# ESMS-Group-Public/FoKL-GPy

Measured on AMD Instinct MI355X. Metric: candidate-terms/sec (basis build + Gibbs + BIC), higher is better.
Workload: dtype f64

## Files before the change

### fokl_gpy_amd/_capi.py

```python
import ctypes
import os

import numpy as np

_HERE = os.path.dirname(os.path.abspath(__file__))
LIB_PATH = os.environ.get('FOKL_HIP_LIBRARY', os.path.join(_HERE, 'libfokl_hip.so'))

UNIQUE_ID_BYTES = 128
K_BASIS, K_GRAM, K_RESID, K_PREDICT, K_RESID_MF, K_GRAM_MFMA, K_GRAM_REDUCE = 0, 1, 2, 3, 4, 5, 6
K_INTEGRATE, K_BAND = 7, 8
K_OPTIMIZE = 9
K_OPTIMIZE_SYSTEM = 10
K_POPULATION = 11
K_RESAMPLE = 12
K_SCORE = 13
K_INFER = 14
K_DESIGN = 15
INTEGRATE_MAX_STATES = 4
RESID_TERMS_MAX_FACTORS = 32
RESID_TERMS_MAX_ORDER = 8
RESID_TERMS_LAYOUTS = ((8, 1), (16, 1), (8, 2), (4, 4), (2, 8), (8, 4), (16, 2), (4, 8))
SLOT_ONES, SLOT_Y, SLOT_FIRST_FREE = 0, 1, 2
PREDICT_NONE, PREDICT_VALU_LDS, PREDICT_VALU_GLOBAL, PREDICT_MFMA = 0, 1, 2, 3
POPULATION_COEFFICIENTS = ('none', 'registers', 'table')
# ... 1396 lines not shown
        a = self._area[3 * self.p1 + self.p1 * self.p1 + 2:]
        return dict(sweeps=int(a[0]), rotations=int(a[1]), seconds=float(a[2]), not_converged=bool(a[3]))

    def release(self):
        if not self._released and self.engine._h:
            self._released = True
            _check(self.engine._lib.fokl_dspectral_release(self.engine._h, self.ticket))


class DeviceSpectralEngine:

    def __init__(self, device=0):
        self._lib = load()
        self._h = None
        h = c_vp(0)
        _check(self._lib.fokl_dspectral_create(int(device), ctypes.byref(h)))
        self._h = h
        self.device = int(device)
        self.max_columns = int(self._lib.fokl_dspectral_max_columns())

    def close(self):
        if self._h:
            self._lib.fokl_dspectral_destroy(self._h)
            self._h = None

    __del__ = close

    def set_signs(self, canonical=True):
        _check(self._lib.fokl_dspectral_set_signs(self._h, 1 if canonical else 0))

    def submit(self, gram, idx, launch=True):
        gram = np.ascontiguousarray(gram, dtype=np.float64)
        idx = np.ascontiguousarray(idx, dtype=np.int32)
        ticket, result = c_i64(0), c_vp(0)
        _check(self._lib.fokl_dspectral_submit(self._h, _ptr(gram), int(gram.shape[0]), _ptr(idx), int(idx.size),
                                               int(gram.shape[0]) - 1, 1 if launch else 0, ctypes.byref(ticket),
                                               ctypes.byref(result)))
        return DeviceSpectralJob(self, ticket.value, result.value, idx.size)

    def flush(self):
        _check(self._lib.fokl_dspectral_flush(self._h))

    def stats(self):
        submitted, launches = c_i64(0), c_i64(0)
        _check(self._lib.fokl_dspectral_stats(self._h, ctypes.byref(submitted), ctypes.byref(launches)))
        return dict(submitted=submitted.value, launches=launches.value)


def gibbs_chain_device(engine, lamb, qty, b, btau, dtd, sigsqd0, tausqd0, tape, stat_first=0):
    job = engine.submit(lamb, qty, b, btau, dtd, sigsqd0, tausqd0, tape, stat_first, follow=False)
    try:
        mean_w, flag = job.wait()
        return job.fetch_w(), np.array(mean_w), bool(flag[0])
    finally:
        job.release()



_OPS_SIGS = (('reserve_slots', [c_vp, c_int]),
             ('build_terms', [c_vp, c_vp, c_int, c_vp]),
             ('gram', [c_vp, c_vp, c_int, c_vp, c_int, c_vp, c_int, c_int]),
             ('gram_launch', [c_vp, c_vp, c_int, c_vp, c_int, c_int]),
             ('gram_fetch', [c_vp, c_vp, c_i64]),
             ('gram_ready', [c_vp]),
             ('bic_resid', [c_vp, c_vp, c_int, c_vp, c_vp, c_int]),
             ('bic_resid_launch', [c_vp, c_vp, c_int, c_vp]),
             ('bic_resid_fetch', [c_vp, c_vp, c_int]),
             ('bic_resid_terms_launch', [c_vp, c_vp, c_int, c_vp]))
_OPS_TYPES = {name: ctypes.CFUNCTYPE(c_int, *args) for name, args in _OPS_SIGS}


class _BackendOps(ctypes.Structure):
    _fields_ = [('ctx', c_vp)] + [(name, c_vp) for name, _ in _OPS_SIGS] + [('kernel_id', c_i32)]


class _RunParams(ctypes.Structure):
    _fields_ = [(name, c_i32) for name in (
        'm', 'n_phis', 'way3', 'tolerance', 'gimmie', 'draws', 'half0', 'lookahead', 'lookahead_native', 'foresight',
        'speculate_across', 'forecast_early', 'forecast_polls', 'matrix_free', 'update_from', 'update_depth',
        'update_lookahead', 'head_start', 'slot_capacity')]


RUN_STATS = ('terms_physical', 'substages', 'forecasts_used', 'forecasts_early', 'resid_matrix_free', 't_resid',
             'phase_prepare', 'phase_model', 'phase_statistics', 'phase_tests', 'phase_wrap_up')


def backend_ops(backend, kernel_id):
    lib = load()
    ops = _BackendOps()
    ops.kernel_id = int(kernel_id)
    ctx = getattr(backend, 'ctx', None)
    if isinstance(ctx, DeviceContext):
        ops.ctx = ctx._h
        for name, _ in _OPS_SIGS:
            setattr(ops, name, ctypes.cast(getattr(lib, 'fokl_' + name), c_vp).value)
        return ops, (ctx,)
    pending, raised = {}, []

    def arr(ptr, count, ctype, dtype):
        return np.array(np.ctypeslib.as_array(ctypes.cast(ptr, ctypes.POINTER(ctype * count)).contents), dtype=dtype)

    def guard(fn):
        def call(*args):
            try:
                fn(*args)
                return 0
            except BaseException as exc:
                raised.append(exc)
                return -3
        return call

    def out(ptr, values):
        values = np.ascontiguousarray(values, dtype=np.float64).reshape(-1)
        ctypes.memmove(ptr, values.ctypes.data, values.nbytes)

    def reserve_slots(_c, n):
        backend.reserve_slots(int(n))

    def build_terms(_c, terms, T, slots):
        sl = arr(slots, T, ctypes.c_int32, np.int32)
        m = pending['m']
        backend.build_terms(arr(terms, T * m, ctypes.c_int32, np.int32).reshape(T, m), [int(v) for v in sl])

    def gram(_c, rows, nr, cols, nc, dst, _path, allreduce):
        out(dst, backend.gram([int(v) for v in arr(rows, nr, ctypes.c_int32, np.int32)],
                              [int(v) for v in arr(cols, nc, ctypes.c_int32, np.int32)], bool(allreduce)))

    def gram_launch(_c, rows, nr, cols, nc, allreduce):
        pending['gram'] = backend.gram([int(v) for v in arr(rows, nr, ctypes.c_int32, np.int32)],
                                       [int(v) for v in arr(cols, nc, ctypes.c_int32, np.int32)], bool(allreduce))

    def gram_fetch(_c, dst, count):
        block = pending.pop('gram')
        assert block.size == count
        out(dst, block)

    def bic_resid(_c, slots, nc, betahat, dst, allreduce):
        out(dst, backend.bic_resid([int(v) for v in arr(slots, nc, ctypes.c_int32, np.int32)],
                                   arr(betahat, nc, ctypes.c_double, np.float64), bool(allreduce)))

    def bic_resid_launch(_c, slots, nc, betahat):
        pending['resid'] = backend.bic_resid([int(v) for v in arr(slots, nc, ctypes.c_int32, np.int32)],
                                             arr(betahat, nc, ctypes.c_double, np.float64), False)

    def bic_resid_fetch(_c, dst, _allreduce):
        out(dst, pending.pop('resid'))

    table = dict(reserve_slots=reserve_slots, build_terms=build_terms, gram=gram, gram_launch=gram_launch,
                 gram_fetch=gram_fetch, bic_resid=bic_resid, bic_resid_launch=bic_resid_launch,
                 bic_resid_fetch=bic_resid_fetch)
    keep = [pending, raised]
    for name, fn in table.items():
        cb = _OPS_TYPES[name](guard(fn))
        keep.append(cb)
        setattr(ops, name, ctypes.cast(cb, c_vp).value)
    return ops, tuple(keep)


class NativeRun:

    def __init__(self, backend, kernel_id, **params):
        self._lib = load()
        self._h = None
        self._ops, self._keep = backend_ops(backend, kernel_id)
        if isinstance(self._keep[0], dict):
            self._keep[0]['m'] = int(params['m'])
        self._prm = _RunParams(**{k: int(v) for k, v in params.items()})
# ... 349 lines not shown
    def design_select(self, slots, C0, CMC0=None, picks=1, replicates=False, refresh_every=64, keep=False, grid_cap=0):
        s = np.ascontiguousarray(slots, dtype=np.int32)
        nc = s.shape[0]
        C0 = np.ascontiguousarray(C0, dtype=np.float64)
        if C0.shape != (nc, nc):
            raise ValueError("design_select: C0 must be [columns, columns] of the slot list")
        if CMC0 is not None:
            CMC0 = np.ascontiguousarray(CMC0, dtype=np.float64)
            if CMC0.shape != (nc, nc):
                raise ValueError("design_select: CMC0 must be [columns, columns] of the slot list")
        picks = int(picks)
        rows = max(picks, 0)
        index = np.empty(rows, dtype=np.int64)
        gain, vstar, x = np.empty(rows), np.empty(rows), np.empty((rows, nc))
        v = np.empty(self.n, dtype=np.float64) if keep else None
        w = np.empty(self.n, dtype=np.float64) if keep and CMC0 is not None else None
        self._ck(self._lib.fokl_design_select(self._h, _ptr(s), nc, _ptr(C0), _ptr(CMC0), picks, int(bool(replicates)),
                                              int(refresh_every), int(grid_cap), _ptr(index), _ptr(gain), _ptr(vstar), _ptr(x),
                                              _ptr(v), _ptr(w)))
        return dict(index=index, gain=gain, vstar=vstar, x=x, v=v, w=w)

    def design_report(self):
        out = np.zeros(12, dtype=np.int64)
        self._ck(self._lib.fokl_design_report(self._h, _ptr(out)))
        v = [int(x) for x in out]
        return dict(instance=DESIGN_INSTANCES[v[0]], grid=v[1], step_grid=v[2], row_tiles=v[3], lds_bytes=v[4], picks=v[5],
                    refreshes=v[6], launches=v[7], kernel_us=v[8], quadform_us=v[9], step_us=v[10], pivot_us=v[11])

    def infer_inputs(self, mtx_u, betas, h, table, lo, hi, prior_mean, prior_prec, y, known_prod, starts, burnin, draws,
                     thin, jump_every, seed, draw_ids=None, rows=True, term_cap=0):
        f64 = lambda a: np.ascontiguousarray(a, dtype=np.float64)
        mtx_u = np.ascontiguousarray(mtx_u, dtype=np.int32)
        betas, h, table, lo, hi, prior_mean, prior_prec, y, known_prod, starts = (
            f64(a) for a in (betas, h, table, lo, hi, prior_mean, prior_prec, y, known_prod, starts))
        if mtx_u.ndim != 2 or betas.ndim != 2 or table.ndim != 2 or y.ndim != 1 or starts.ndim != 2 or lo.ndim != 1:
            raise ValueError("infer_inputs: array shapes disagree")
        n_terms, d = mtx_u.shape
        E, K = betas.shape[0], y.shape[0]
        if betas.shape[1] != n_terms + 1 or h.shape != (E,) or known_prod.shape != (K, n_terms + 1) or \
                starts.shape != (INFER_WALKERS, d) or any(a.shape != (d,) for a in (lo, hi, prior_mean, prior_prec)):
            raise ValueError("infer_inputs: array shapes disagree")
        ids = None
        if draw_ids is not None:
            ids = np.ascontiguousarray(draw_ids, dtype=np.uint32)
            if ids.shape != (E,):
                raise ValueError("infer_inputs: one draw id per row of betas")
        kept = -(-int(draws) // int(thin)) if int(thin) >= 1 and int(draws) >= 1 else 0
        x = np.empty((E, kept, INFER_WALKERS, d), dtype=np.float64) if rows else None
        lp = np.empty((E, kept, INFER_WALKERS), dtype=np.float64) if rows else None
        sums = np.empty((E, INFER_WALKERS, 2, 2, d), dtype=np.float64)
        accepted = np.empty((E, INFER_WALKERS, 2), dtype=np.int32)
        evaluations = np.empty(E, dtype=np.int64)
        self._ck(self._lib.fokl_infer_inputs(
            self._h, int(d), int(n_terms), _ptr(mtx_u), int(E), _ptr(betas), _ptr(h), _ptr(ids), _ptr(table),
            int(table.shape[0]), int(table.shape[1]), _ptr(lo), _ptr(hi), _ptr(prior_mean), _ptr(prior_prec), int(K), _ptr(y),
            _ptr(known_prod), _ptr(starts), int(burnin), int(draws), int(thin), int(jump_every), int(seed) & 0xFFFFFFFF,
            int(term_cap), _ptr(x), _ptr(lp), _ptr(sums), _ptr(accepted), _ptr(evaluations)))
        return x, lp, sums, accepted, evaluations

    def infer_report(self):
        out = np.zeros(9, dtype=np.int64)
        self._ck(self._lib.fokl_infer_report(self._h, _ptr(out)))
        v = [int(x) for x in out]
        return dict(mapping=INFER_MAPPINGS[v[0]], lds_rows=v[1], grid=v[2], launches=v[3], kernel_us=v[4], iterations=v[5],
                    evaluations=v[6], draws_per_launch=v[7], lds_bytes=v[8])

    def _fit_report(self, which, count):
        out = np.zeros(count, dtype=np.int64)
        self._ck(self._lib.fokl_fit_report(self._h, which, _ptr(out), count))
        return [int(v) for v in out]

    def gram_report(self):
        keys = ('kernel', 'nt8', 'half', 'loaders', 'lds_buffers', 'ks', 'depth', 'rows_per_chunk', 'groups', 'ct', 'nt',
                'pieces', 'lds_bytes', 'S', 'chunks_per_workgroup', 'nr_pad', 'nc_pad', 'slabs', 'reduce_epb', 'row_tiles',
                'col_tiles', 'lanes')
        ran = dict(zip(keys, self._fit_report(0, len(keys))))
        ran['kernel'], ran['half'] = GRAM_KERNELS[ran['kernel']], bool(ran['half'])
        return ran

    def resid_report(self):
        v = self._fit_report(1, 9)
        return dict(kernel=RESID_KERNELS[v[0]], columns=v[1], batches=v[2], grid=v[3], row_tiles=v[4], layout=(v[5], v[6]),
                    order_class=v[7], inputs=v[8])

    def basis_report(self):
        v = self._fit_report(2, 23)
        keys = ('kernel', 'splines', 'lanes', 'factors', 'slabs', 'grid', 'row_tiles')

        def one(rec):
            d = dict(zip(keys, rec))
            d['kernel'], d['splines'] = BASIS_KERNELS[d['kernel']], bool(d['splines'])
            return d
        return dict(launches=v[0], lds_table=v[1], first=one(v[2:9]), last=one(v[9:16]), last_lds=one(v[16:23]))

    def gp_integrate_ensemble(self, n_members, n_states, n_other, n_steps, betas, per_member, mtx, rows, cols, sources,
                              n_src, forcing, norms, table, n_basis, width, h, y0, cut=None, want_members=False):
        mean = np.empty((n_states, n_steps + 1), dtype=np.float64)
        bounds = np.empty((n_states, n_steps + 1, 2), dtype=np.float64) if cut is not None else None
        members = np.empty((n_members, n_states, n_steps + 1), dtype=np.float64) if want_members else None
        self._ck(self._lib.fokl_gp_integrate_ensemble(
            self._h, int(n_members), int(n_states), int(n_other), int(n_steps), betas, _ptr(per_member), mtx, _ptr(rows),
            _ptr(cols), sources, _ptr(n_src), _ptr(forcing), _ptr(norms), _ptr(table), int(n_basis), int(width), float(h),
            _ptr(y0), int(y0.ndim == 2), int(cut or 0), _ptr(mean), _ptr(bounds), _ptr(members)))
        return mean, bounds, members

    def simulate_ensemble(self, p):
        K, E, P = int(p['K']), int(p['E']), int(p['n_steps']) + 1
        mean = np.empty((K, P), dtype=np.float64)
        bounds = np.empty((K, P, 2), dtype=np.float64) if p['want_bounds'] else None
        members = np.empty((E, K, P), dtype=np.float64) if p['want_members'] else None
        first = np.empty(E, dtype=np.int32)
        i32 = lambda a: np.ascontiguousarray(a, dtype=np.int32)
        f64 = lambda a: np.ascontiguousarray(a, dtype=np.float64)
        forcing, norm_src, norm_lo, norm_span = f64(p['forcing']), i32(p['norm_src']), f64(p['norm_lo']), f64(p['norm_span'])
        fac_norm, fac_kind, fac_row, fac_degree = (i32(p[key]) for key in ('fac_norm', 'fac_kind', 'fac_row', 'fac_degree'))
        spline, bern, entries = f64(p['spline_table']), f64(p['bern_table']), i32(p['entries']).reshape(-1, 4)
        begin, count, constant = i32(p['entry_begin']), i32(p['entry_count']), i32(p['constant'])
        coef, y0, box = f64(p['coef']), f64(p['y0']), f64(p['box'])
        if coef.ndim != 2 or coef.shape[1] != E or y0.shape != (K, E) or box.shape != (K, 2) or begin.shape != (K,) or \
                count.shape != (K,) or constant.shape != (K,) or forcing.ndim != 2 or forcing.shape[0] != P - 1 or \
                not (norm_src.shape == norm_lo.shape == norm_span.shape) or \
                not (fac_norm.shape == fac_kind.shape == fac_row.shape == fac_degree.shape) or \
                spline.shape[1:] != (499, 4) or bern.ndim != 2 or bern.shape[1] != 21:
            raise ValueError("simulate_ensemble: array shapes disagree")
        self._ck(self._lib.fokl_simulate_ensemble(
            self._h, E, K, P - 1, float(p['h']), forcing.shape[1], _ptr(forcing), int(p['n_norm_forcing']), norm_src.shape[0],
            _ptr(norm_src), _ptr(norm_lo), _ptr(norm_span), int(p['n_forcing_factors']), fac_norm.shape[0], _ptr(fac_norm),
            _ptr(fac_kind), _ptr(fac_row), _ptr(fac_degree), spline.shape[0], _ptr(spline), bern.shape[0], _ptr(bern),
            entries.shape[0], _ptr(entries), _ptr(begin), _ptr(count), _ptr(constant), coef.shape[0], _ptr(coef), _ptr(y0),
            _ptr(box), int(p['cut']) if p['want_bounds'] else 0, _ptr(mean), _ptr(bounds), _ptr(members), _ptr(first)))
        return mean, bounds, members, first

    def simulate_report(self):
        out = np.zeros(8, dtype=np.int64)
        self._ck(self._lib.fokl_simulate_report(self._h, _ptr(out)))
        keys = ('NS', 'members', 'workgroups', 'lds_bytes', 'launches', 'spline_factors', 'bernoulli_factors',
                'steps_per_launch')
        return dict(zip(keys, (int(v) for v in out)))

    def assimilate_ensemble(self, p):
        K, E, P = int(p['K']), int(p['E']), int(p['n_steps']) + 1
        i32 = lambda a: np.ascontiguousarray(a, dtype=np.int32)
        f64 = lambda a: np.ascontiguousarray(a, dtype=np.float64)
        forcing, norm_src, norm_lo, norm_span = f64(p['forcing']), i32(p['norm_src']), f64(p['norm_lo']), f64(p['norm_span'])
        fac_norm, fac_kind, fac_row, fac_degree = (i32(p[key]) for key in ('fac_norm', 'fac_kind', 'fac_row', 'fac_degree'))
        spline, bern, entries = f64(p['spline_table']), f64(p['bern_table']), i32(p['entries']).reshape(-1, 4)
        begin, count, constant = i32(p['entry_begin']), i32(p['entry_count']), i32(p['constant'])
        coef, y0, box = f64(np.asarray(p['coef']).T), f64(p['y0']), f64(p['box'])
        ids = np.ascontiguousarray(p['draw_ids'], dtype=np.uint32)
        obs_state, obs_sd, obs_row = i32(p['obs_state']), f64(p['obs_sd']), i32(p['obs_row'])
        data, obs_const, q, y0_sd = f64(p['data']), f64(p['obs_const']), f64(p['process_q']), f64(p['y0_sd'])
        n_obs = data.shape[0] if data.ndim == 2 else -1
        if coef.ndim != 2 or coef.shape[0] != E or y0.shape != (K, E) or box.shape != (K, 2) or begin.shape != (K,) or \
                count.shape != (K,) or constant.shape != (K,) or forcing.ndim != 2 or forcing.shape[0] != P - 1 or \
                not (norm_src.shape == norm_lo.shape == norm_span.shape) or \
                not (fac_norm.shape == fac_kind.shape == fac_row.shape == fac_degree.shape) or \
                spline.shape[1:] != (499, 4) or bern.ndim != 2 or bern.shape[1] != 21 or ids.shape != (E,) or \
                obs_state.ndim != 1 or obs_sd.shape != obs_state.shape or data.ndim != 2 or \
                data.shape[1] != obs_state.shape[0] or obs_row.shape != (P,) or obs_const.shape != (n_obs,) or \
                q.shape != (K,) or y0_sd.shape != (K,):
            raise ValueError("assimilate_ensemble: array shapes disagree")
        stats = np.empty((E, n_obs, 2 * K + 3), dtype=np.float64)
        keep = bool(p['want_particles'])
        particles = np.empty((E, n_obs, ASSIMILATE_PARTICLES, K), dtype=np.float64) if keep else None
        weights = np.empty((E, n_obs, ASSIMILATE_PARTICLES), dtype=np.float64) if keep else None
        first, collapsed = np.empty(E, dtype=np.int32), np.empty(E, dtype=np.int32)
# ... 396 lines not shown
```

### fokl_gpy_amd/csrc/fokl_gram_dev.inc

```

namespace fokl {


constexpr int GM_THREADS = 256;
constexpr int GM_R = 32;
constexpr int GM_PITCH = GM_R + 2;

template <int TI, int TJ, bool ISPLIT>
__global__ __launch_bounds__(GM_THREADS) void gram_mfma_kernel(double *const *__restrict__ slot_ptr,
                                                               const int *__restrict__ row_slots, int nr,
                                                               const int *__restrict__ col_slots, int nc, int64_t n,
                                                               double *__restrict__ slab, int nr_pad, int nc_pad,
                                                               const double *__restrict__ zero_col)
{
    static_assert(!ISPLIT || TI == 4, "i-split needs one i-tile per wavefront");
    constexpr int BI = 16 * TI;
    constexpr int BJ = ISPLIT ? 16 * TJ : 64 * TJ;
    constexpr int NCOL = BI + BJ;
    constexpr int PASSES = (NCOL + 15) / 16;
    constexpr int MI = ISPLIT ? 1 : TI;
    __shared__ __attribute__((aligned(16))) double tile[NCOL * GM_PITCH];

    const int tid = threadIdx.x, wave = tid / WAVE, lane = tid % WAVE;
    const int i0 = blockIdx.z * BI, j0 = blockIdx.y * BJ;
// ... 302 lines not shown

template <int NT>
static gram_tiles_fn tiles_kernel_n(int passes, int depth, int ks)
{
    if (passes <= 4) return tiles_kernel_np<NT, 4>(depth, ks);
    if (passes <= 8) return tiles_kernel_np<NT, 8>(depth, ks);
    return tiles_kernel_np<NT, 16>(depth, ks);
}

static gram_tiles_fn tiles_kernel(int nt, int passes, int depth, int ks)
{
    switch (nt) {
        case 1: return tiles_kernel_n<1>(passes, depth, ks);
        case 2: return tiles_kernel_n<2>(passes, depth, ks);
        case 3: return tiles_kernel_n<3>(passes, depth, ks);
        case 4: return tiles_kernel_n<4>(passes, depth, ks);
        case 5: return gram_tiles_kernel<5, 16, 1, 1>;
        case 6: return gram_tiles_kernel<6, 16, 1, 1>;
        case 7: return gram_tiles_kernel<7, 16, 1, 1>;
        case 8: return gram_tiles_kernel<8, 16, 1, 1>;
        case 9: return gram_tiles_kernel<9, 16, 1, 1>;
        default: return gram_tiles_kernel<10, 16, 1, 1>;
    }
}

typedef void (*gram_tiles4_fn)(double *const *, const int *, int, const GramGroup *, int, int64_t, double *, int, int,
                               const double *, const double *);

template <int NT>
static gram_tiles4_fn tiles4s_kernel_n(int passes)
{
    if (passes <= 2) return gram_tiles4s_kernel<NT, 2>;
    if (passes <= 4) return gram_tiles4s_kernel<NT, 4>;
    if (passes <= 6) return gram_tiles4s_kernel<NT, 6>;
    return gram_tiles4s_kernel<NT, 8>;
}

static gram_tiles4_fn tiles4s_kernel(int nt, int passes)
{
    switch (nt) {
        case 1: return tiles4s_kernel_n<1>(passes);
        case 2: return tiles4s_kernel_n<2>(passes);
        case 3: return tiles4s_kernel_n<3>(passes);
        default: return tiles4s_kernel_n<4>(passes);
    }
}


static gram_dma_fn tiles_dma_kernel_ab(int nt8, bool half, int nbuf, int loaders)
{
    if (nbuf == 3) return loaders == 0 ? tiles_dma_kernel_b<3, 0>(nt8, half) : nullptr;
    if (nbuf == 2 && loaders == 2) return tiles_dma_kernel_b<2, 2>(nt8, half);
    return tiles_dma_kernel(nt8, half, nbuf, loaders);
}

static int launch_gram_panel(fokl_ctx *ctx, const GramCall &c, GramLaunch &run)
{
    const int *d_rows, *d_cols;
    int rc = push_slot_lists(ctx, c, d_rows, d_cols);
    if (rc) return rc;
    const int nr = c.nr, nc = c.nc;
    gram_mfma_fn mfma_fn = nullptr;
    int BI, BJ;
    const int j_tiles = (nc + 15) / 16;
    if (nr > 32) {
        const int panels = (j_tiles + 11) / 12;
        const int tj = (j_tiles + panels - 1) / panels;
        mfma_fn = isplit_kernel(tj);
        BI = 64;
        BJ = 16 * tj;
    } else {
        const int ti = nr > 16 ? 2 : 1;
        const int per_wave = (j_tiles + 3) / 4;
        const int panels = (per_wave + 2) / 3;
        const int tj = (per_wave + panels - 1) / panels;
        mfma_fn = jsplit_kernel(ti, tj);
        BI = 16 * ti;
        BJ = 64 * tj;
    }
    const int gz = (nr + BI - 1) / BI, gy = (nc + BJ - 1) / BJ;
    run.nr_pad = gz * BI;
    run.nc_pad = gy * BJ;
    const int64_t n_chunks = (ctx->n + GM_R - 1) / GM_R;
    const int per_cu = blocks_per_cu(mfma_fn, GM_THREADS, 0);
    const int target = std::max(1, (per_cu * cu_count(ctx)) / (gz * gy));
    rc = size_slabs(ctx, run, (int)std::max<int64_t>(1, std::min<int64_t>(n_chunks, target)), 1, n_chunks);
    if (rc) return rc;
    run.rep[0] = FOKL_GRAM_PANEL, run.rep[5] = run.rep[6] = 1, run.rep[7] = GM_R, run.rep[8] = gy * gz;
    run.rep[21] = GM_THREADS;
    TimedRegion timed(ctx, c.slot, c.bytes, c.flops);
    hipLaunchKernelGGL(mfma_fn, dim3(run.S, gy, gz), dim3(GM_THREADS), 0, ctx->stream, ctx->d_slot_ptr, d_rows, nr, d_cols,
                       nc, ctx->n, ctx->d_slab, run.nr_pad, run.nc_pad, ctx->d_zero);
    return FOKL_OK;
}

static int launch_gram_tiles4(fokl_ctx *ctx, const GramCall &c, GramLaunch &run, int wgs_cap)
{
    const GramPlan &pl = run.plan;
    const int P = pl.ct <= 2 ? 2 : pl.ct <= 4 ? 4 : pl.ct <= 6 ? 6 : 8;
    gram_tiles4_fn fn = tiles4s_kernel(pl.nt, pl.ct);
    const size_t lds = (size_t)P * 16 * G4_PITCH * sizeof(double);
    int rc = raise_lds_limit(ctx, reinterpret_cast<const void *>(fn), lds);
    if (rc) return rc;
    const int64_t n_chunks = (ctx->n + 31) / 32;
    const int per_cu = std::min(wgs_cap, blocks_per_cu(fn, G4S_THREADS, lds));
    const int target = std::max(1, (per_cu * cu_count(ctx)) / (int)pl.groups.size());
    rc = size_slabs(ctx, run, (int)std::max<int64_t>(1, std::min<int64_t>(n_chunks, target)), 1, n_chunks);
    if (rc) return rc;
    run.rep[0] = FOKL_GRAM_TILES4, run.rep[1] = pl.nt, run.rep[7] = 32, run.rep[12] = (int64_t)lds, run.rep[21] = G4S_THREADS;
    TimedRegion timed(ctx, c.slot, c.bytes, c.flops);
    hipLaunchKernelGGL(fn, dim3(run.S, (unsigned)pl.groups.size()), dim3(G4S_THREADS), lds, ctx->stream, ctx->d_slot_ptr,
                       run.d_icols, pl.nci, run.d_groups, pl.ct, ctx->n, ctx->d_slab, run.nr_pad, run.nc_pad, ctx->d_zero,
                       run.grid_base);
    return FOKL_OK;
}

static int launch_gram_dev(fokl_ctx *ctx, const GramCall &c, const LaunchKnobs &k, int path, GramLaunch &run, bool &taken)
{
    const GramPlan &pl = run.plan;
    taken = true;
    if (path == 3) return launch_gram_panel(ctx, c, run);
    if (pl.kind == 1) return launch_gram_tiles4(ctx, c, run, k.wgs);
    if (pl.ks == 1 && k.dma != 2 && !(k.dma == 1 && c.slot == FOKL_K_GRAM_MFMA)) {
        gram_tiles_fn fn = tiles_kernel(pl.nt, pl.ct << pl.rb_shift, pl.depth, 1);
        const size_t lds = (size_t)pl.ct * 16 * ((32 << pl.rb_shift) + 2) * sizeof(double);
        return launch_gram_tiles(ctx, c, run, fn, k.wgs, blocks_per_cu(fn, GT_THREADS, lds), cu_count(ctx));
    }
    if (pl.ks > 1 && (pl.rb_shift != 0 || pl.depth != 1)) {
        const int passes = pl.ct << pl.rb_shift;
        return launch_gram_tiles(ctx, c, run, tiles_kernel(pl.nt, passes, pl.depth, pl.ks), k.wgs, passes > 8 && pl.depth == 2 ? 2 : 3);
    }
    const size_t pieces = (pl.ct * 16 * 34 * 8 + 1023) / 1024;
    const int nbuf = k.bufs == 3 && 3 * pieces * 1024 <= 160 * 1024 ? 3 : 2;
    if (pl.ks == 1 && (nbuf == 3 || k.loaders == 2))
        return launch_gram_dma(ctx, c, run, tiles_dma_kernel_ab, k.wgs, nbuf, nbuf == 2 ? k.loaders : 0);
    taken = false;
    return FOKL_OK;
}
```

### fokl_gpy_amd/csrc/fokl_hip.hip

```cpp
#include <hip/hip_runtime.h>

#include <algorithm>
#include <climits>
#include <cmath>
#include <cstdint>
#include <cstdio>
#include <cstdlib>
#include <cstring>
#include <map>
#include <mutex>
#include <string>
#include <utility>
#include <vector>

#include "../../include/fokl_hip_internal.h"
#include "fokl_kernels.hip.h"

using namespace fokl;


static std::mutex g_err_mutex;
static std::string g_err;

void fokl_set_global_error(const std::string &msg)
{
    std::lock_guard<std::mutex> lock(g_err_mutex);
    g_err = msg;
}

struct TimingSlot {
    double ms = 0.0;
    int64_t launches = 0;
    double bytes = 0.0;
    double flops = 0.0;
    double ideal_ms = 0.0;
};

struct PendingEvent {
    int kernel_id;
    hipEvent_t start, stop;
};

struct fokl_ctx {
    int device = 0;
    int cus = 0;
    hipStream_t stream = nullptr;
    std::string err;

    bool have_data = false;
    int64_t n = 0, ld = 0;
    int m = 0, kernel = 0, n_basis = 0, width = 0;
    double *d_x = nullptr;
    double *d_zero = nullptr;
    double *d_staged = nullptr;
    int64_t staged_n = 0;
    int staged_m = 0;
    double *d_phis = nullptr;
    std::vector<double> h_phis;
    size_t phis_doubles = 0;

    static constexpr int CHUNK_SLOTS = 16;
    std::vector<double *> chunks;
    std::vector<double *> slot_ptr;
    double **d_slot_ptr = nullptr;
    int table_cap = 0;

    char *d_args = nullptr;
    char *h_args = nullptr;
    size_t args_cap = 0;
    double *d_slab = nullptr;
    size_t slab_doubles = 0;
    double *d_out = nullptr;
    double *h_out = nullptr;
    size_t out_doubles = 0;
    hipEvent_t args_free = nullptr;
    bool resid_pending = false;
    double *d_rout = nullptr;
    double *h_rout = nullptr;
    double *d_gout = nullptr;
    double *h_gout = nullptr;
    size_t gout_doubles = 0;
    size_t gram_pending = 0;
    hipEvent_t gram_done = nullptr;
    hipEvent_t resid_done = nullptr;
    int64_t predict_report[6] = {0, 0, 0, 0, 0, 0};
    int64_t population_report[FOKL_POPULATION_REPORT_LEN] = {};
    int64_t resample_report[FOKL_RESAMPLE_REPORT_LEN] = {};
    int64_t score_report[FOKL_SCORE_REPORT_LEN] = {};
    int64_t infer_report[FOKL_INFER_REPORT_LEN] = {};
    int64_t design_report[FOKL_DESIGN_REPORT_LEN] = {};
    int64_t simulate_report[FOKL_SIMULATE_REPORT_LEN] = {};
    int64_t assimilate_report[FOKL_ASSIMILATE_REPORT_LEN] = {};
    int64_t control_report[FOKL_CONTROL_REPORT_LEN] = {};
    int64_t control_pooled_report[FOKL_CONTROL_POOLED_REPORT_LEN] = {};
    int64_t control_cvar_report[FOKL_CONTROL_CVAR_REPORT_LEN] = {};
    int64_t gram_report[FOKL_GRAM_REPORT_LEN] = {};
    int64_t resid_report[FOKL_RESID_REPORT_LEN] = {};
    int64_t basis_report[FOKL_BASIS_REPORT_LEN] = {};

    bool timing = false;
    TimingSlot tslot[FOKL_K_COUNT];
    std::vector<PendingEvent> pending;
    std::vector<hipEvent_t> event_pool;

    void *comm = nullptr;
    int rank = 0, world = 1;
    double *d_comm = nullptr;
    size_t comm_doubles = 0;

    int64_t optimize_report[FOKL_OPTIMIZE_REPORT_LEN] = {};
    int64_t system_optimize_report[FOKL_OPTIMIZE_REPORT_LEN] = {};
};

static int fail(fokl_ctx *ctx, int code, const std::string &msg)
{
    if (ctx) ctx->err = msg;
    fokl_set_global_error(msg);
    return code;
}

#define HIP_TRY(ctx, call)                                                                                     \
    do {                                                                                                       \
        hipError_t e__ = (call);                                                                               \
        if (e__ != hipSuccess)                                                                                 \
            return fail(ctx, FOKL_ERR_HIP, std::string(#call) + ": " + hipGetErrorString(e__));                \
    } while (0)

struct DeviceBuffers {
    std::vector<void *> owned;
    ~DeviceBuffers()
    {
        for (void *p : owned) (void)hipFree(p);
    }
    template <typename T>
    hipError_t get(T **out, size_t count)
    {
        void *p = nullptr;
        hipError_t e = hipMalloc(&p, std::max<size_t>(count, 1) * sizeof(T));
        if (e == hipSuccess) owned.push_back(p);
        *out = static_cast<T *>(p);
        return e;
    }
    template <typename T>
    hipError_t upload(T **out, const void *host, size_t count)
    {
        hipError_t e = get(out, count);
        if (e == hipSuccess && count) e = hipMemcpy(*out, host, count * sizeof(T), hipMemcpyHostToDevice);
        return e;
    }
};


static hipEvent_t take_event(fokl_ctx *ctx)
{
    if (!ctx->event_pool.empty()) {
        hipEvent_t e = ctx->event_pool.back();
        ctx->event_pool.pop_back();
        return e;
    }
    hipEvent_t e = nullptr;
    if (hipEventCreate(&e) != hipSuccess) return nullptr;
    return e;
}

struct TimedRegion {
    fokl_ctx *ctx;
    int id;
    hipEvent_t start = nullptr, stop = nullptr;
    TimedRegion(fokl_ctx *c, int kernel_id, double bytes, double flops) : ctx(c), id(kernel_id)
    {
        if (!ctx->timing) return;
        ctx->tslot[id].launches += 1;
        ctx->tslot[id].bytes += bytes;
        ctx->tslot[id].flops += flops;
        ctx->tslot[id].ideal_ms += 1e3 * std::max(bytes / FOKL_PEAK_HBM_BYTES_PER_S, flops / FOKL_PEAK_F64_FLOPS);
        start = take_event(ctx);
        stop = take_event(ctx);
        if (start && stop) (void)hipEventRecord(start, ctx->stream);
    }
    ~TimedRegion()
    {
        if (!ctx->timing || !start || !stop) return;
        (void)hipEventRecord(stop, ctx->stream);
        ctx->pending.push_back({id, start, stop});
    }
};

static void drain_events(fokl_ctx *ctx)
{
    for (auto &p : ctx->pending) {
        float ms = 0.f;
        if (hipEventSynchronize(p.stop) == hipSuccess && hipEventElapsedTime(&ms, p.start, p.stop) == hipSuccess)
            ctx->tslot[p.kernel_id].ms += ms;
        ctx->event_pool.push_back(p.start);
        ctx->event_pool.push_back(p.stop);
    }
    ctx->pending.clear();
}


static int ensure_args(fokl_ctx *ctx, size_t bytes)
{
    if (bytes <= ctx->args_cap) return FOKL_OK;
    size_t cap = std::max<size_t>(bytes * 2, 1 << 16);
    HIP_TRY(ctx, hipStreamSynchronize(ctx->stream));
    if (ctx->d_args) HIP_TRY(ctx, hipFree(ctx->d_args));
    if (ctx->h_args) HIP_TRY(ctx, hipHostFree(ctx->h_args));
    ctx->d_args = nullptr;
    ctx->h_args = nullptr;
    ctx->args_cap = 0;
    HIP_TRY(ctx, hipMalloc((void **)&ctx->d_args, cap));
    HIP_TRY(ctx, hipHostMalloc((void **)&ctx->h_args, cap, hipHostMallocDefault));
    ctx->args_cap = cap;
    return FOKL_OK;
}

static int ensure_slab(fokl_ctx *ctx, size_t doubles)
{
    if (doubles <= ctx->slab_doubles) return FOKL_OK;
    size_t cap = std::max<size_t>(doubles + doubles / 2, 1 << 16);
    HIP_TRY(ctx, hipStreamSynchronize(ctx->stream));
    if (ctx->d_slab) HIP_TRY(ctx, hipFree(ctx->d_slab));
    ctx->d_slab = nullptr;
    ctx->slab_doubles = 0;
    HIP_TRY(ctx, hipMalloc((void **)&ctx->d_slab, cap * sizeof(double)));
    ctx->slab_doubles = cap;
    return FOKL_OK;
}

static int ensure_out(fokl_ctx *ctx, size_t doubles)
{
    if (doubles <= ctx->out_doubles) return FOKL_OK;
    size_t cap = std::max<size_t>(doubles * 2, 1 << 12);
    HIP_TRY(ctx, hipStreamSynchronize(ctx->stream));
    if (ctx->d_out) HIP_TRY(ctx, hipFree(ctx->d_out));
    if (ctx->h_out) HIP_TRY(ctx, hipHostFree(ctx->h_out));
    ctx->d_out = nullptr;
    ctx->h_out = nullptr;
    ctx->out_doubles = 0;
    HIP_TRY(ctx, hipMalloc((void **)&ctx->d_out, cap * sizeof(double)));
    HIP_TRY(ctx, hipHostMalloc((void **)&ctx->h_out, cap * sizeof(double), hipHostMallocDefault));
    ctx->out_doubles = cap;
    return FOKL_OK;
}

static int ensure_rout(fokl_ctx *ctx)
{
    if (ctx->d_rout) return FOKL_OK;
    HIP_TRY(ctx, hipMalloc((void **)&ctx->d_rout, 2 * sizeof(double)));
    HIP_TRY(ctx, hipHostMalloc((void **)&ctx->h_rout, 2 * sizeof(double), hipHostMallocDefault));
    return FOKL_OK;
}

static int ensure_gout(fokl_ctx *ctx, size_t doubles)
{
    if (doubles <= ctx->gout_doubles) return FOKL_OK;
    size_t cap = std::max<size_t>(doubles * 2, 1 << 12);
    HIP_TRY(ctx, hipStreamSynchronize(ctx->stream));
    if (ctx->d_gout) HIP_TRY(ctx, hipFree(ctx->d_gout));
    if (ctx->h_gout) HIP_TRY(ctx, hipHostFree(ctx->h_gout));
    ctx->d_gout = nullptr;
    ctx->h_gout = nullptr;
    ctx->gout_doubles = 0;
    HIP_TRY(ctx, hipMalloc((void **)&ctx->d_gout, cap * sizeof(double)));
    HIP_TRY(ctx, hipHostMalloc((void **)&ctx->h_gout, cap * sizeof(double), hipHostMallocDefault));
    ctx->gout_doubles = cap;
    return FOKL_OK;
}

static int begin_args(fokl_ctx *ctx, size_t bytes)
{
    int rc = ensure_args(ctx, bytes);
    if (rc) return rc;
    HIP_TRY(ctx, hipEventSynchronize(ctx->args_free));
    return FOKL_OK;
}

static int push_args(fokl_ctx *ctx, size_t bytes)
{
    HIP_TRY(ctx, hipMemcpyAsync(ctx->d_args, ctx->h_args, bytes, hipMemcpyHostToDevice, ctx->stream));
    HIP_TRY(ctx, hipEventRecord(ctx->args_free, ctx->stream));
    return FOKL_OK;
}

static void free_slots(fokl_ctx *ctx)
{
    for (double *c : ctx->chunks) (void)hipFree(c);
    ctx->chunks.clear();
    ctx->slot_ptr.clear();
}

static int check_slots(fokl_ctx *ctx, const int32_t *slots, int count, const char *who)
{
    if (!slots && count > 0) return fail(ctx, FOKL_ERR_ARG, std::string(who) + ": null slot list");
    const int cap = (int)ctx->slot_ptr.size();
    for (int i = 0; i < count; ++i)
        if (slots[i] < 0 || slots[i] >= cap)
            return fail(ctx, FOKL_ERR_ARG, std::string(who) + ": slot " + std::to_string(slots[i]) +
                                               " outside [0, " + std::to_string(cap) + ")");
    return FOKL_OK;
}


extern "C" int fokl_version(void) { return 100; }

extern "C" int fokl_device_count(int *count)
{
    if (!count) return fail(nullptr, FOKL_ERR_ARG, "fokl_device_count: null pointer");
    int n = 0;
    hipError_t e = hipGetDeviceCount(&n);
    if (e != hipSuccess) {
        *count = 0;
        return fail(nullptr, FOKL_ERR_HIP, std::string("hipGetDeviceCount: ") + hipGetErrorString(e));
    }
    *count = n;
    return FOKL_OK;
}

extern "C" const char *fokl_last_error(const fokl_ctx *ctx)
{
    if (ctx) return ctx->err.c_str();
    std::lock_guard<std::mutex> lock(g_err_mutex);
    static thread_local std::string copy;
    copy = g_err;
    return copy.c_str();
}

extern "C" int fokl_ctx_create(int device, fokl_ctx **out)
{
    if (!out) return fail(nullptr, FOKL_ERR_ARG, "fokl_ctx_create: null output pointer");
    *out = nullptr;
    int n = 0;
    hipError_t e = hipGetDeviceCount(&n);
    if (e != hipSuccess || n <= 0)
        return fail(nullptr, FOKL_ERR_HIP, "fokl_ctx_create: no HIP device available (" +
                                               std::string(hipGetErrorString(e)) + ")");
    if (device < 0 || device >= n)
        return fail(nullptr, FOKL_ERR_ARG, "fokl_ctx_create: device index out of range");
    fokl_ctx *ctx = new fokl_ctx();
    ctx->device = device;
    if (const char *mode = std::getenv("FOKL_SYNC"))
        if (std::strcmp(mode, "blocking") == 0) {
            (void)hipSetDeviceFlags(hipDeviceScheduleBlockingSync);
            (void)hipGetLastError();
        }
    HIP_TRY(nullptr, hipSetDevice(device));
    hipDeviceProp_t prop;
    HIP_TRY(nullptr, hipGetDeviceProperties(&prop, device));
    if (std::string(prop.gcnArchName).rfind("gfx950", 0) != 0) {
        std::string arch = prop.gcnArchName;
        delete ctx;
        return fail(nullptr, FOKL_ERR_HIP, "fokl_ctx_create: device is " + arch + ", this library is built for gfx950 only");
    }
    const int total_cus = prop.multiProcessorCount;
    ctx->cus = total_cus;
    const hipError_t made = hipStreamCreateWithFlags(&ctx->stream, hipStreamNonBlocking);
    if (made != hipSuccess ||
        hipEventCreateWithFlags(&ctx->args_free, hipEventDisableTiming) != hipSuccess ||
        hipEventCreateWithFlags(&ctx->gram_done, hipEventDisableTiming) != hipSuccess ||
        hipEventCreateWithFlags(&ctx->resid_done, hipEventDisableTiming) != hipSuccess) {
        delete ctx;
        return fail(nullptr, FOKL_ERR_HIP, "fokl_ctx_create: cannot create stream / event");
    }
    (void)hipEventRecord(ctx->args_free, ctx->stream);
    *out = ctx;
    return FOKL_OK;
}

extern "C" int fokl_comm_destroy(fokl_ctx *ctx);

extern "C" void fokl_ctx_destroy(fokl_ctx *ctx)
{
    if (!ctx) return;
    (void)hipSetDevice(ctx->device);
    if (ctx->stream) (void)hipStreamSynchronize(ctx->stream);
    (void)fokl_comm_destroy(ctx);
    drain_events(ctx);
    for (hipEvent_t e : ctx->event_pool) (void)hipEventDestroy(e);
    free_slots(ctx);
    if (ctx->d_slot_ptr) (void)hipFree(ctx->d_slot_ptr);
    if (ctx->d_x) (void)hipFree(ctx->d_x);
    if (ctx->d_phis) (void)hipFree(ctx->d_phis);
    if (ctx->d_zero) (void)hipFree(ctx->d_zero);
    if (ctx->d_staged) (void)hipFree(ctx->d_staged);
    if (ctx->d_args) (void)hipFree(ctx->d_args);
    if (ctx->h_args) (void)hipHostFree(ctx->h_args);
    if (ctx->d_slab) (void)hipFree(ctx->d_slab);
    if (ctx->d_out) (void)hipFree(ctx->d_out);
    if (ctx->h_out) (void)hipHostFree(ctx->h_out);
    if (ctx->d_gout) (void)hipFree(ctx->d_gout);
    if (ctx->h_gout) (void)hipHostFree(ctx->h_gout);
    if (ctx->d_rout) (void)hipFree(ctx->d_rout);
    if (ctx->h_rout) (void)hipHostFree(ctx->h_rout);
    if (ctx->d_comm) (void)hipFree(ctx->d_comm);
    if (ctx->args_free) (void)hipEventDestroy(ctx->args_free);
    if (ctx->gram_done) (void)hipEventDestroy(ctx->gram_done);
    if (ctx->resid_done) (void)hipEventDestroy(ctx->resid_done);
    if (ctx->stream) (void)hipStreamDestroy(ctx->stream);
    delete ctx;
}

extern "C" int fokl_sync(fokl_ctx *ctx)
{
    if (!ctx) return fail(nullptr, FOKL_ERR_ARG, "fokl_sync: null context");
    HIP_TRY(ctx, hipStreamSynchronize(ctx->stream));
    drain_events(ctx);
    return FOKL_OK;
}

extern "C" int fokl_slot_capacity(const fokl_ctx *ctx) { return ctx ? (int)ctx->slot_ptr.size() : 0; }
extern "C" int64_t fokl_rows(const fokl_ctx *ctx) { return ctx ? ctx->n : 0; }


extern "C" int fokl_reserve_slots(fokl_ctx *ctx, int n_slots)
{
    if (!ctx) return fail(nullptr, FOKL_ERR_ARG, "fokl_reserve_slots: null context");
    if (!ctx->have_data) return fail(ctx, FOKL_ERR_STATE, "fokl_reserve_slots: call fokl_upload first");
    HIP_TRY(ctx, hipSetDevice(ctx->device));
    bool grew = false;
    while ((int)ctx->slot_ptr.size() < n_slots) {
        double *chunk = nullptr;
        const size_t bytes = (size_t)fokl_ctx::CHUNK_SLOTS * ctx->ld * sizeof(double);
        HIP_TRY(ctx, hipMalloc((void **)&chunk, bytes));
        ctx->chunks.push_back(chunk);
        for (int i = 0; i < fokl_ctx::CHUNK_SLOTS; ++i) ctx->slot_ptr.push_back(chunk + (size_t)i * ctx->ld);
        grew = true;
    }
    if (grew) {
        const int cap = (int)ctx->slot_ptr.size();
        if (cap > ctx->table_cap) {
            HIP_TRY(ctx, hipStreamSynchronize(ctx->stream));
            if (ctx->d_slot_ptr) HIP_TRY(ctx, hipFree(ctx->d_slot_ptr));
            ctx->d_slot_ptr = nullptr;
            ctx->table_cap = 0;
            const int new_cap = std::max(cap * 2, 256);
            HIP_TRY(ctx, hipMalloc((void **)&ctx->d_slot_ptr, (size_t)new_cap * sizeof(double *)));
            ctx->table_cap = new_cap;
        }
        HIP_TRY(ctx, hipStreamSynchronize(ctx->stream));
        HIP_TRY(ctx, hipMemcpy(ctx->d_slot_ptr, ctx->slot_ptr.data(), (size_t)cap * sizeof(double *),
                               hipMemcpyHostToDevice));
    }
    return FOKL_OK;
}


static int upload_dataset(fokl_ctx *ctx, const double *x, const double *y, int64_t n, int m, int kernel, const double *phis,
                          int n_basis, int width, const double *lows, const double *spans, const char *who)
{
    if (!ctx) return fail(nullptr, FOKL_ERR_ARG, std::string(who) + ": null context");
    if (!y || !phis) return fail(ctx, FOKL_ERR_ARG, std::string(who) + ": null pointer");
    if (n <= 0 || m <= 0 || m > 4096) return fail(ctx, FOKL_ERR_ARG, std::string(who) + ": need n > 0 and 0 < m <= 4096");
    if (kernel != FOKL_KERNEL_SPLINES && kernel != FOKL_KERNEL_BERNOULLI)
        return fail(ctx, FOKL_ERR_ARG, std::string(who) + ": unknown kernel id");
    if (n_basis <= 0 || width <= 0) return fail(ctx, FOKL_ERR_ARG, std::string(who) + ": empty coefficient table");
    if (kernel == FOKL_KERNEL_BERNOULLI && width < n_basis + 1)
        return fail(ctx, FOKL_ERR_ARG, std::string(who) + ": Bernoulli table needs width >= n_basis + 1");
    HIP_TRY(ctx, hipSetDevice(ctx->device));
    HIP_TRY(ctx, hipStreamSynchronize(ctx->stream));
    drain_events(ctx);

    free_slots(ctx);
    if (ctx->d_x) HIP_TRY(ctx, hipFree(ctx->d_x));
    if (ctx->d_phis) HIP_TRY(ctx, hipFree(ctx->d_phis));
    if (ctx->d_zero) HIP_TRY(ctx, hipFree(ctx->d_zero));
    ctx->d_x = nullptr;
    ctx->d_phis = nullptr;
    ctx->d_zero = nullptr;
    ctx->have_data = false;

    ctx->n = n;
    ctx->m = m;
    ctx->ld = (n + 63) / 64 * 64;
    ctx->kernel = kernel;
    ctx->n_basis = n_basis;
    ctx->width = width;
    ctx->phis_doubles = (kernel == FOKL_KERNEL_SPLINES) ? (size_t)n_basis * 4 * width : (size_t)n_basis * width;

// ... 41 lines not shown

extern "C" int fokl_stage_inputs(fokl_ctx *ctx, const double *x, int64_t n, int m, double *lows_out, double *highs_out)
{
    if (!ctx) return fail(nullptr, FOKL_ERR_ARG, "fokl_stage_inputs: null context");
    if (!x || !lows_out || !highs_out) return fail(ctx, FOKL_ERR_ARG, "fokl_stage_inputs: null pointer");
    if (n <= 0 || m <= 0 || m > 4096) return fail(ctx, FOKL_ERR_ARG, "fokl_stage_inputs: need n > 0 and 0 < m <= 4096");
    HIP_TRY(ctx, hipSetDevice(ctx->device));
    if (ctx->d_staged) HIP_TRY(ctx, hipFree(ctx->d_staged));
    ctx->d_staged = nullptr;
    HIP_TRY(ctx, hipMalloc((void **)&ctx->d_staged, (size_t)n * m * sizeof(double)));
    ctx->staged_n = n;
    ctx->staged_m = m;
    HIP_TRY(ctx, hipMemcpy(ctx->d_staged, x, (size_t)n * m * sizeof(double), hipMemcpyHostToDevice));
    const int64_t total = n * (int64_t)m;
    int64_t lanes = std::min<int64_t>((int64_t)1024 * 256, (total + 7) / 8);
    lanes = std::max<int64_t>(m, lanes / m * m);
    const int blocks = (int)((lanes + 255) / 256);
    double *d_part = nullptr;
    HIP_TRY(ctx, hipMalloc((void **)&d_part, (size_t)(2 * lanes + 2 * m) * sizeof(double)));
    hipLaunchKernelGGL(column_bounds_kernel, dim3(blocks), dim3(256), 0, ctx->stream, ctx->d_staged, total, m, lanes, d_part);
    hipLaunchKernelGGL(column_bounds_finish_kernel, dim3(m), dim3(256), 0, ctx->stream, d_part, lanes, m, d_part + 2 * lanes);
    HIP_TRY(ctx, hipGetLastError());
    std::vector<double> h((size_t)2 * m);
    HIP_TRY(ctx, hipMemcpyAsync(h.data(), d_part + 2 * lanes, (size_t)2 * m * sizeof(double), hipMemcpyDeviceToHost, ctx->stream));
    HIP_TRY(ctx, hipStreamSynchronize(ctx->stream));
    HIP_TRY(ctx, hipFree(d_part));
    for (int k = 0; k < m; ++k) {
        lows_out[k] = h[(size_t)k];
        highs_out[k] = h[(size_t)m + k];
    }
    return FOKL_OK;
}

extern "C" int fokl_upload_staged(fokl_ctx *ctx, const double *y, int64_t n, int m, int kernel, const double *phis,
                                  int n_basis, int width, const double *lows, const double *spans)
{
    if (!ctx) return fail(nullptr, FOKL_ERR_ARG, "fokl_upload_staged: null context");
    if (!lows || !spans) return fail(ctx, FOKL_ERR_ARG, "fokl_upload_staged: null pointer");
    if (!ctx->d_staged || ctx->staged_n != n || ctx->staged_m != m)
        return fail(ctx, FOKL_ERR_STATE, "fokl_upload_staged: no staged inputs of this shape (fokl_stage_inputs first)");
    return upload_dataset(ctx, nullptr, y, n, m, kernel, phis, n_basis, width, lows, spans, "fokl_upload_staged");
}

extern "C" int fokl_download_inputs(fokl_ctx *ctx, double *x_out)
{
    if (!ctx) return fail(nullptr, FOKL_ERR_ARG, "fokl_download_inputs: null context");
    if (!x_out) return fail(ctx, FOKL_ERR_ARG, "fokl_download_inputs: null pointer");
    if (!ctx->have_data) return fail(ctx, FOKL_ERR_STATE, "fokl_download_inputs: call fokl_upload first");
    HIP_TRY(ctx, hipSetDevice(ctx->device));
    double *d_rows = nullptr;
    HIP_TRY(ctx, hipMalloc((void **)&d_rows, (size_t)ctx->n * ctx->m * sizeof(double)));
    const int blocks = (int)std::min<int64_t>((ctx->n + 255) / 256, 4096);
    hipLaunchKernelGGL(rows_from_columns_kernel, dim3(blocks), dim3(256), 0, ctx->stream, ctx->d_x, ctx->n, ctx->m, ctx->ld, d_rows);
    HIP_TRY(ctx, hipGetLastError());
    HIP_TRY(ctx, hipMemcpyAsync(x_out, d_rows, (size_t)ctx->n * ctx->m * sizeof(double), hipMemcpyDeviceToHost, ctx->stream));
    HIP_TRY(ctx, hipStreamSynchronize(ctx->stream));
    HIP_TRY(ctx, hipFree(d_rows));
    return FOKL_OK;
}


static int cu_count(fokl_ctx *ctx) { return ctx->cus > 0 ? ctx->cus : 256; }

static int env_int(const char *name, int fallback)
{
    const char *v = std::getenv(name);
    return v && *v ? std::atoi(v) : fallback;
}

struct LaunchKnobs {
    int path = 2, mfma4 = 0, dma = 2, half = 1, bufs = 2, loaders = 4, rb = 1, depth = 1, wgs = 3;
    int k1_wgs = INT_MAX;
    int tiles4_nt = 0, tiles4_ct = 0;
    bool half_slots() const { return mfma4 != 2 && dma == 2 && half != 0; }
};
#ifdef FOKL_DEV_KERNELS
static LaunchKnobs launch_knobs();
#else
static LaunchKnobs launch_knobs() { return LaunchKnobs(); }
#endif

static constexpr size_t K1_LDS_BUDGET = 144 * 1024;

static int launch_basis(fokl_ctx *ctx, const int32_t *terms, const int32_t *slots, int t_begin, int t_end,
                        const DerivSpec &deriv)
{
    const int m = ctx->m;
    const bool splines = ctx->kernel == FOKL_KERNEL_SPLINES;
    std::map<std::pair<int, int>, int> fac_id;
    for (int j = t_begin; j < t_end; ++j)
        for (int k = 0; k < m; ++k) {
            const int o = terms[(size_t)j * m + k];
            if (o != 0) fac_id.emplace(std::make_pair(k, o), 0);
        }
    int U = 0;
    for (auto &kv : fac_id) kv.second = U++;
    const int T = t_end - t_begin;

    std::vector<int> slab_orders;
    if (splines) {
        for (auto &kv : fac_id) {
            const int o = kv.first.second;
            if (std::find(slab_orders.begin(), slab_orders.end(), o) == slab_orders.end() &&
                (int)slab_orders.size() < K1_MAX_LDS_SLABS)
                slab_orders.push_back(o);
        }
    }
    const int NS = (int)slab_orders.size();
    size_t slab_doubles = splines ? (((size_t)NS * 4 * ctx->width + 1) & ~(size_t)1) : 0;
    int threads = K1_THREADS;
    {
        int best_waves = -1;
        for (int t : {256, 128, 64}) {
            const size_t need = slab_doubles * sizeof(double) + (size_t)std::max(U, 1) * t * sizeof(d2);
            const int blocks = (int)std::min<size_t>(16, (160 * 1024) / std::max<size_t>(need, 1));
            const int waves = std::min(32, blocks * (t / 64));
            if (waves > best_waves) {
                best_waves = waves;
                threads = t;
            }
        }
        if (const char *env = getenv("FOKL_K1_THREADS")) {
            const int t = atoi(env);
            if (t == 64 || t == 128 || t == 256) threads = t;
        }
    }
    const bool reg_table = U <= K1_REG_FACTORS;
    if (reg_table) threads = K1_THREADS;
    size_t lds_bytes = slab_doubles * sizeof(double) +
                       (reg_table ? 0 : (size_t)std::max(U, 1) * threads * sizeof(d2));

    size_t n_fac_entries = 0;
    for (int j = t_begin; j < t_end; ++j)
        for (int k = 0; k < m; ++k) n_fac_entries += terms[(size_t)j * m + k] != 0;

    const size_t n_ints = (size_t)3 * U + K1_MAX_LDS_SLABS + (T + 1) + n_fac_entries + T;
    const size_t plan_bytes = sizeof(BasisPlan);
    const size_t bytes = plan_bytes + n_ints * sizeof(int);
    int rc = begin_args(ctx, bytes);
    if (rc) return rc;
    BasisPlan *plan = reinterpret_cast<BasisPlan *>(ctx->h_args);
    plan->n_fac = U;
    plan->n_terms = T;
    plan->n_slabs = NS;
    plan->pad = 0;
    int *arr = reinterpret_cast<int *>(ctx->h_args + plan_bytes);
    int *fac_input = arr, *fac_order = arr + U, *fac_slab = arr + 2 * U, *slab_order = arr + 3 * U;
    int *term_off = slab_order + K1_MAX_LDS_SLABS, *term_fac = term_off + (T + 1);
    int *term_slot = term_fac + n_fac_entries;
    for (auto &kv : fac_id) {
        const int u = kv.second;
        fac_input[u] = kv.first.first;
        fac_order[u] = kv.first.second;
        int s = -1;
        for (int q = 0; q < NS; ++q)
            if (slab_orders[q] == kv.first.second) s = q;
        fac_slab[u] = s;
    }
    for (int q = 0; q < K1_MAX_LDS_SLABS; ++q) slab_order[q] = q < NS ? slab_orders[q] : 1;
    int off = 0;
    for (int j = t_begin; j < t_end; ++j) {
        term_off[j - t_begin] = off;
        for (int k = 0; k < m; ++k) {
            const int o = terms[(size_t)j * m + k];
            if (o != 0) term_fac[off++] = fac_id[std::make_pair(k, o)];
        }
        term_slot[j - t_begin] = slots[j];
    }
    term_off[T] = off;
    rc = push_args(ctx, bytes);
    if (rc) return rc;

    const int64_t tile_rows = (int64_t)threads * K1_ROWS_PER_THREAD;
    const int64_t n_tiles = (ctx->n + tile_rows - 1) / tile_rows;
    int per_cu = (int)std::max<size_t>(1, std::min<size_t>(reg_table ? 5 : 16, (160 * 1024) / std::max<size_t>(lds_bytes, 1)));
    per_cu = std::min(per_cu, launch_knobs().k1_wgs);
    const int grid = (int)std::min<int64_t>(n_tiles, (int64_t)cu_count(ctx) * per_cu);
    const BasisPlan *d_plan = reinterpret_cast<const BasisPlan *>(ctx->d_args);
    const int *d_arr = reinterpret_cast<const int *>(ctx->d_args + plan_bytes);

    int m_used = 0;
    {
        int last = -1;
        for (auto &kv : fac_id)
            if (kv.first.first != last) {
                last = kv.first.first;
                ++m_used;
            }
    }
    const double alg_bytes = 8.0 * (double)ctx->n * (double)(m_used + T);
    TimedRegion timed(ctx, FOKL_K_BASIS, alg_bytes, 0.0);
    typedef void (*basis_fn)(const double *, int64_t, int64_t, const double *, int, const BasisPlan *, const int *,
                             double *const *, DerivSpec);
    basis_fn fn = splines ? (reg_table ? basis_build_reg_kernel<true> : basis_build_kernel<true>)
                          : (reg_table ? basis_build_reg_kernel<false> : basis_build_kernel<false>);
    if (lds_bytes > 64 * 1024)
        HIP_TRY(ctx, hipFuncSetAttribute(reinterpret_cast<const void *>(fn), hipFuncAttributeMaxDynamicSharedMemorySize,
                                         (int)K1_LDS_BUDGET + 4096));
    hipLaunchKernelGGL(fn, dim3(grid), dim3(threads), lds_bytes, ctx->stream, ctx->d_x, ctx->ld, ctx->n, ctx->d_phis,
                       ctx->width, d_plan, d_arr, ctx->d_slot_ptr, deriv);
    HIP_TRY(ctx, hipGetLastError());
    {
        const int64_t rec[7] = {reg_table ? FOKL_BASIS_REG_TABLE : FOKL_BASIS_LDS_TABLE, splines ? 1 : 0, threads, U, NS,
                                grid, n_tiles};
        int64_t *rep = ctx->basis_report;
        if (rep[0]++ == 0) std::memcpy(rep + 2, rec, sizeof rec);
        std::memcpy(rep + 9, rec, sizeof rec);
        if (!reg_table) {
            rep[1] += 1;
            std::memcpy(rep + 16, rec, sizeof rec);
        }
    }
    return FOKL_OK;
}

static int build_terms_impl(fokl_ctx *ctx, const int32_t *terms, int T, const int32_t *slots, const DerivSpec &deriv);

extern "C" int fokl_build_terms(fokl_ctx *ctx, const int32_t *terms, int T, const int32_t *slots)
{
    const DerivSpec plain = {-1, 0, 1.0, 0};
    return build_terms_impl(ctx, terms, T, slots, plain);
}

extern "C" int fokl_build_terms_deriv(fokl_ctx *ctx, const int32_t *terms, int T, const int32_t *slots, int wrt_input,
                                      int order, double divisor)
{
    if (!ctx) return fail(nullptr, FOKL_ERR_ARG, "fokl_build_terms_deriv: null context");
    if (!ctx->have_data) return fail(ctx, FOKL_ERR_STATE, "fokl_build_terms_deriv: call fokl_upload first");
    if (wrt_input < 0 || wrt_input >= ctx->m || (order != 1 && order != 2) || !(divisor != 0.0))
        return fail(ctx, FOKL_ERR_ARG, "fokl_build_terms_deriv: need 0 <= wrt_input < m, order 1 or 2, divisor != 0");
    for (int j = 0; j < T; ++j)
        if (terms && terms[(size_t)j * ctx->m + wrt_input] == 0)
            return fail(ctx, FOKL_ERR_ARG, "fokl_build_terms_deriv: a term does not contain the differentiated input "
                                           "(its derivative is the zero column; leave it out)");
    const DerivSpec spec = {wrt_input, order, divisor, 1};
    return build_terms_impl(ctx, terms, T, slots, spec);
}

static int build_terms_impl(fokl_ctx *ctx, const int32_t *terms, int T, const int32_t *slots, const DerivSpec &deriv)
{
    if (!ctx) return fail(nullptr, FOKL_ERR_ARG, "fokl_build_terms: null context");
    std::memset(ctx->basis_report, 0, sizeof ctx->basis_report);
    if (!ctx->have_data) return fail(ctx, FOKL_ERR_STATE, "fokl_build_terms: call fokl_upload first");
    if (T < 0 || (T > 0 && (!terms || !slots))) return fail(ctx, FOKL_ERR_ARG, "fokl_build_terms: null pointer");
    if (T == 0) return FOKL_OK;
    HIP_TRY(ctx, hipSetDevice(ctx->device));
    int rc = check_slots(ctx, slots, T, "fokl_build_terms");
    if (rc) return rc;
    const int m = ctx->m;
    for (int j = 0; j < T; ++j) {
        if (slots[j] < FOKL_SLOT_FIRST_FREE)
            return fail(ctx, FOKL_ERR_ARG, "fokl_build_terms: slots 0 and 1 are reserved (ones, y)");
        int nz = 0;
        for (int k = 0; k < m; ++k) {
            const int o = terms[(size_t)j * m + k];
            if (o < 0 || o > ctx->n_basis)
                return fail(ctx, FOKL_ERR_ARG, "fokl_build_terms: basis order " + std::to_string(o) +
                                                   " outside [0, " + std::to_string(ctx->n_basis) + "]");
            nz += o != 0;
        }
        if (nz == 0) return fail(ctx, FOKL_ERR_ARG, "fokl_build_terms: term with no input (all-zero row)");
    }
    const bool splines = ctx->kernel == FOKL_KERNEL_SPLINES;
    const size_t slab_bytes = splines ? (size_t)K1_MAX_LDS_SLABS * 4 * ctx->width * sizeof(double) + 16 : 0;
    const int lds_fac = (int)((K1_LDS_BUDGET - slab_bytes) / (K1_THREADS * sizeof(d2)));
    int max_fac = K1_REG_FACTORS;
    for (int j = 0; j < T; ++j) {
        int nz = 0;
        for (int k = 0; k < m; ++k) nz += terms[(size_t)j * m + k] != 0;
        if (nz > lds_fac) return fail(ctx, FOKL_ERR_ARG, "fokl_build_terms: a single term has more factors than fit in LDS");
        if (nz > max_fac) max_fac = nz;
    }
    int begin = 0;
    while (begin < T) {
        std::map<std::pair<int, int>, int> seen;
        int end = begin;
        while (end < T) {
            std::vector<std::pair<int, int>> add;
            for (int k = 0; k < m; ++k) {
                const int o = terms[(size_t)end * m + k];
                if (o != 0 && !seen.count({k, o})) add.push_back({k, o});
            }
            if ((int)(seen.size() + add.size()) > max_fac) break;
            for (auto &p : add) seen[p] = 1;
            ++end;
        }
        if (end == begin) rc = fail(ctx, FOKL_ERR_ARG, "fokl_build_terms: a single term has more factors than fit in LDS");
        if (!rc) rc = launch_basis(ctx, terms, slots, begin, end, deriv);
        if (rc) {
            std::memset(ctx->basis_report, 0, sizeof ctx->basis_report);
            return rc;
        }
        begin = end;
    }
    return FOKL_OK;
}


extern "C" int fokl_comm_allreduce_sum_f64(fokl_ctx *ctx, double *buf, int count);
static int comm_allreduce_device(fokl_ctx *ctx, double *d_buf, size_t count);

static int reduce_elements_per_block(int total)
{
    int epb = 1;
    while (epb < 16 && epb * 64 < total) epb *= 2;
    while (epb < 64 && (total + epb - 1) / epb > 4096) epb *= 2;
    return epb;
}

template <typename F>
static int blocks_per_cu(F fn, int threads, size_t dyn_lds)
{
    int nb = 0;
    if (hipOccupancyMaxActiveBlocksPerMultiprocessor(&nb, fn, threads, dyn_lds) != hipSuccess || nb < 1) nb = 1;
    return std::min(nb, 8);
}


struct GramPlan {
    int nci = 0, it = 0, jt = 0;
    int nt = 1, ct = 1, ks = 1, rb_shift = 0, depth = 1;
    int kind = 0, waves = 4;
    bool half = false;
    std::vector<int32_t> icols;
    std::vector<int32_t> perm;
    std::vector<GramGroup> groups;
};

static void plan_gram(const int32_t *row_slots, int nr, const int32_t *col_slots, int nc, int kind, const LaunchKnobs &knobs,
                      GramPlan &pl)
{
    pl.kind = kind;
    pl.waves = 4;
    const int nt_max = kind == 1 ? knobs.tiles4_nt : GT_MAX_NT;
    const int ct_max = kind == 1 ? knobs.tiles4_ct : GT_MAX_CT;
    pl.icols.assign(row_slots, row_slots + nr);
    pl.perm.resize(nc);
    {
        std::map<int32_t, int> where;
        for (int i = 0; i < nr; ++i) where.emplace(row_slots[i], i);
        for (int j = 0; j < nc; ++j) {
            auto f = where.find(col_slots[j]);
            if (f != where.end()) {
                pl.perm[j] = f->second;
            } else {
                pl.perm[j] = (int)pl.icols.size();
                where.emplace(col_slots[j], (int)pl.icols.size());
                pl.icols.push_back(col_slots[j]);
            }
        }
    }
    pl.nci = (int)pl.icols.size();
    pl.it = (nr + 15) / 16;
    pl.jt = (pl.nci + 15) / 16;

    struct Cut {
        std::vector<std::pair<int, int>> tiles;
        std::vector<int> staged;
    };
    std::vector<Cut> cuts;
    const int max_tiles = pl.waves * nt_max;
    for (int b0 = 0; b0 < pl.it; b0 += 4) {
        const int i_hi = std::min(pl.it, b0 + 4);
        std::vector<std::pair<int, int>> seq;
        for (int jt = b0; jt < pl.jt; ++jt)
            for (int it = b0; it < std::min(i_hi, jt + 1); ++it) seq.emplace_back(it, jt);
        const int T = (int)seq.size();
        for (int G = std::max(1, (T + max_tiles - 1) / max_tiles);; ++G) {
            std::vector<Cut> trial;
            bool fits = true;
            int at = 0;
            for (int gi = 0; gi < G && fits; ++gi) {
                const int size = T / G + (gi < T % G ? 1 : 0);
                Cut c;
                c.tiles.assign(seq.begin() + at, seq.begin() + at + size);
                at += size;
                for (auto &t : c.tiles) {
                    c.staged.push_back(t.first);
                    c.staged.push_back(t.second);
                }
                std::sort(c.staged.begin(), c.staged.end());
                c.staged.erase(std::unique(c.staged.begin(), c.staged.end()), c.staged.end());
                fits = (int)c.staged.size() <= ct_max && size <= max_tiles;
                if (size > 0) trial.push_back(std::move(c));
            }
            if (fits) {
                for (auto &c : trial) cuts.push_back(std::move(c));
                break;
            }
        }
    }

    int most_tiles = 1, most_staged = 1;
    for (auto &c : cuts) {
        most_tiles = std::max(most_tiles, (int)c.tiles.size());
        most_staged = std::max(most_staged, (int)c.staged.size());
    }
    pl.ks = kind != 0 ? 1 : most_tiles == 1 ? 4 : most_tiles == 2 ? 2 : 1;
// ... 82 lines not shown
static int no_instance(fokl_ctx *ctx, const char *kernel, const GramPlan &pl)
{
    return fail(ctx, FOKL_ERR_ARG, std::string("fokl_gram: this library holds no ") + kernel + " for nt " + std::to_string(pl.nt) +
                                       ", ct " + std::to_string(pl.ct << pl.rb_shift) + ", depth " + std::to_string(pl.depth));
}

static gram_tiles_fn ksplit_kernel(const GramPlan &pl)
{
    if (pl.nt != 1 || pl.ct > 4 || pl.rb_shift != 0 || pl.depth != 1) return nullptr;
    return pl.ks == 4 ? gram_tiles_kernel<1, 4, 1, 4> : pl.ks == 2 ? gram_tiles_kernel<1, 4, 1, 2> : nullptr;
}

typedef void (*gram_dma_fn)(const GramGroup *, int, int, int64_t, double *, int, int, const double *, uint32_t);
typedef gram_dma_fn (*gram_dma_picker)(int nt8, bool half, int nbuf, int loaders);

template <int NBUF, int LW>
static gram_dma_fn tiles_dma_kernel_b(int nt8, bool half)
{
    static const gram_dma_fn plain[5] = {gram_tiles_dma_kernel<1, NBUF, false, LW>, gram_tiles_dma_kernel<2, NBUF, false, LW>,
                                         gram_tiles_dma_kernel<3, NBUF, false, LW>, gram_tiles_dma_kernel<4, NBUF, false, LW>,
                                         gram_tiles_dma_kernel<5, NBUF, false, LW>};
    static const gram_dma_fn slots[4] = {gram_tiles_dma_kernel<1, NBUF, true, LW>, gram_tiles_dma_kernel<2, NBUF, true, LW>,
                                         gram_tiles_dma_kernel<3, NBUF, true, LW>, gram_tiles_dma_kernel<4, NBUF, true, LW>};
    return nt8 < 1 || nt8 > (half ? 4 : 5) ? nullptr : half ? slots[nt8 - 1] : plain[nt8 - 1];
}

static gram_dma_fn tiles_dma_kernel(int nt8, bool half, int nbuf, int loaders)
{
    if (nbuf != 2) return nullptr;
    return loaders == 4 ? tiles_dma_kernel_b<2, 4>(nt8, half) : loaders == 0 ? tiles_dma_kernel_b<2, 0>(nt8, half) : nullptr;
}

extern "C" int fokl_gram_plan(const int32_t *row_slots, int nr, const int32_t *col_slots, int nc, int kind, int32_t *info,
                              int32_t *icols, int32_t *perm, int32_t *staged, int32_t *tiles, int cap_groups)
{
    if (!row_slots || !col_slots || !info || nr <= 0 || nc <= 0 || kind < 0 || kind > 1)
        return fail(nullptr, FOKL_ERR_ARG, "fokl_gram_plan: bad argument");
    const LaunchKnobs knobs = launch_knobs();
    if (kind == 1 && !knobs.tiles4_nt)
        return fail(nullptr, FOKL_ERR_ARG, "fokl_gram_plan: kind 1 (4x4x4 tile lists) needs a development build");
    GramPlan pl;
    plan_gram(row_slots, nr, col_slots, nc, kind, knobs, pl);
    const int32_t head[10] = {pl.nci, pl.it, pl.jt, (int32_t)pl.groups.size(), pl.nt, pl.ct, pl.rb_shift, pl.ks, pl.depth,
                              pl.waves};
    std::memcpy(info, head, sizeof(head));
    if ((int)pl.groups.size() > cap_groups) return FOKL_OK;
    if (icols) std::memcpy(icols, pl.icols.data(), pl.icols.size() * sizeof(int32_t));
    if (perm) std::memcpy(perm, pl.perm.data(), pl.perm.size() * sizeof(int32_t));
    for (size_t gi = 0; gi < pl.groups.size(); ++gi) {
        const GramGroup &g = pl.groups[gi];
        if (staged) std::memcpy(staged + gi * GT_MAX_CT, g.ct, sizeof(g.ct));
        if (tiles)
            for (int w = 0; w < GT_MAX_WAVES; ++w)
                for (int k = 0; k < GT_MAX_NT; ++k) {
                    int32_t *t = tiles + ((gi * GT_MAX_WAVES + w) * GT_MAX_NT + k) * 4;
                    t[0] = g.a[w][k] | (pl.half && k < 2 && g.oi[w][k] != 0xFFFF ? 256 : 0);
                    t[1] = g.b[w][k];
                    t[2] = g.oi[w][k] == 0xFFFF ? -1 : g.oi[w][k];
                    t[3] = g.oj[w][k] == 0xFFFF ? -1 : g.oj[w][k];
                }
    }
    return FOKL_OK;
}


struct GramCall {
    const int32_t *row_slots, *col_slots;
    int nr, nc;
    int slot;
    double bytes, flops;
};

struct GramLaunch {
    GramPlan plan;
    const int *d_icols = nullptr;
    const GramGroup *d_groups = nullptr;
    const double *grid_base = nullptr;
    const int *d_perm = nullptr;
    int S = 0, slabs = 0;
    int nr_pad = 0, nc_pad = 0;
    int64_t rep[FOKL_GRAM_REPORT_LEN] = {};
};

static std::mutex lds_limit_mutex;
static std::map<const void *, size_t> lds_limit_set;

static int raise_lds_limit(fokl_ctx *ctx, const void *fn, size_t lds)
{
    std::lock_guard<std::mutex> lock(lds_limit_mutex);
    size_t &have = lds_limit_set[fn];
    if (have < lds) {
        HIP_TRY(ctx, hipFuncSetAttribute(fn, hipFuncAttributeMaxDynamicSharedMemorySize, 160 * 1024));
        have = 160 * 1024;
    }
    return FOKL_OK;
}

static int pinned_row_cut(int wgs_cap, int by_registers, size_t lds, size_t groups, int64_t n_chunks, int cus = 256)
{
    const int lds_fit = (int)std::max<size_t>(1, (size_t)(160 * 1024) / std::max<size_t>(lds, 1));
    const int target = std::max(1, (std::min({wgs_cap, by_registers, lds_fit}) * cus) / (int)groups);
    return (int)std::max<int64_t>(1, std::min<int64_t>(n_chunks, target));
}

static int size_slabs(fokl_ctx *ctx, GramLaunch &run, int S, int ks, int64_t n_chunks)
{
    run.S = S;
    run.slabs = S * ks;
    run.rep[14] = (n_chunks + S - 1) / S;
    return ensure_slab(ctx, (size_t)run.slabs * run.nr_pad * run.nc_pad);
}

static int push_slot_lists(fokl_ctx *ctx, const GramCall &c, const int *&d_rows, const int *&d_cols)
{
    const size_t arg_bytes = (size_t)(c.nr + c.nc) * sizeof(int);
    int rc = begin_args(ctx, arg_bytes);
    if (rc) return rc;
    int *h = reinterpret_cast<int *>(ctx->h_args);
    std::memcpy(h, c.row_slots, (size_t)c.nr * sizeof(int));
    std::memcpy(h + c.nr, c.col_slots, (size_t)c.nc * sizeof(int));
    d_rows = reinterpret_cast<const int *>(ctx->d_args);
    d_cols = d_rows + c.nr;
    return push_args(ctx, arg_bytes);
}

static int launch_gram_valu(fokl_ctx *ctx, const GramCall &c, GramLaunch &run)
{
    const int *d_rows, *d_cols;
    int rc = push_slot_lists(ctx, c, d_rows, d_cols);
    if (rc) return rc;
    const int gz = (c.nr + GV_TI - 1) / GV_TI, gy = (c.nc + GV_TJ - 1) / GV_TJ;
    run.nr_pad = gz * GV_TI;
    run.nc_pad = gy * GV_TJ;
    const int64_t n_row_blocks = (ctx->n + GV_THREADS * 2 - 1) / (GV_THREADS * 2);
    const int target = std::max(1, (8 * cu_count(ctx)) / (gz * gy));
    rc = size_slabs(ctx, run, (int)std::max<int64_t>(1, std::min<int64_t>(n_row_blocks, target)), 1, n_row_blocks);
    if (rc) return rc;
    run.rep[0] = FOKL_GRAM_VALU, run.rep[5] = run.rep[6] = 1, run.rep[7] = GV_THREADS * 2, run.rep[8] = gy * gz;
    run.rep[21] = GV_THREADS;
    TimedRegion timed(ctx, c.slot, c.bytes, c.flops);
    hipLaunchKernelGGL(gram_valu_kernel, dim3(run.S, gy, gz), dim3(GV_THREADS), 0, ctx->stream, ctx->d_slot_ptr, d_rows, c.nr,
                       d_cols, c.nc, ctx->n, ctx->d_slab, run.nr_pad, run.nc_pad);
    return FOKL_OK;
}

static int stage_gram_tiles(fokl_ctx *ctx, const GramCall &c, int kind, const LaunchKnobs &knobs, GramLaunch &run)
{
    GramPlan &pl = run.plan;
    plan_gram(c.row_slots, c.nr, c.col_slots, c.nc, kind, knobs, pl);
    const uintptr_t lo = reinterpret_cast<uintptr_t>(run.grid_base);
    const uint32_t zero_units = (uint32_t)((reinterpret_cast<uintptr_t>(ctx->d_zero) - lo) >> 8) | 0x80000000u;
    for (GramGroup &g : pl.groups)
        for (int p = 0; p < GT_MAX_CT; ++p)
            for (int k = 0; k < 16; ++k) {
                const int col = g.ct[p] >= 0 ? 16 * g.ct[p] + k : -1;
                g.col_units[p][k] = col >= 0 && col < pl.nci
                                        ? (uint32_t)((reinterpret_cast<uintptr_t>(ctx->slot_ptr[pl.icols[col]]) - lo) >> 8)
                                        : zero_units;
            }
    const size_t ints = (size_t)pl.nci + (size_t)c.nc;
    const size_t group_off = (ints * sizeof(int32_t) + 15) / 16 * 16;
    const size_t arg_bytes = group_off + pl.groups.size() * sizeof(GramGroup);
    int rc = begin_args(ctx, arg_bytes);
    if (rc) return rc;
    std::memcpy(ctx->h_args, pl.icols.data(), (size_t)pl.nci * sizeof(int32_t));
    std::memcpy(ctx->h_args + (size_t)pl.nci * sizeof(int32_t), pl.perm.data(), (size_t)c.nc * sizeof(int32_t));
    std::memcpy(ctx->h_args + group_off, pl.groups.data(), pl.groups.size() * sizeof(GramGroup));
    run.d_icols = reinterpret_cast<const int *>(ctx->d_args);
    run.d_perm = run.d_icols + pl.nci;
    run.d_groups = reinterpret_cast<const GramGroup *>(ctx->d_args + group_off);
    run.nr_pad = 16 * pl.it;
    run.nc_pad = 16 * pl.jt;
    run.rep[2] = pl.half ? 1 : 0, run.rep[5] = pl.ks, run.rep[6] = pl.depth, run.rep[8] = (int64_t)pl.groups.size();
    run.rep[9] = pl.ct, run.rep[10] = pl.nt, run.rep[19] = pl.it, run.rep[20] = pl.jt;
    return push_args(ctx, arg_bytes);
}

static int launch_gram_tiles(fokl_ctx *ctx, const GramCall &c, GramLaunch &run, gram_tiles_fn fn, int wgs_cap,
                             int by_registers = 3, int cut_cus = 256)
{
    const GramPlan &pl = run.plan;
    if (!fn) return no_instance(ctx, "gram_tiles_kernel", pl);
    const int R = 32 << pl.rb_shift;
    const size_t lds = (size_t)pl.ct * 16 * (R + 2) * sizeof(double);
    int rc = raise_lds_limit(ctx, reinterpret_cast<const void *>(fn), lds);
    if (rc) return rc;
    const int64_t n_chunks = (ctx->n + R - 1) / R;
    rc = size_slabs(ctx, run, pinned_row_cut(wgs_cap, by_registers, lds, pl.groups.size(), n_chunks, cut_cus), pl.ks, n_chunks);
    if (rc) return rc;
    run.rep[0] = FOKL_GRAM_TILES, run.rep[1] = pl.nt, run.rep[7] = R, run.rep[12] = (int64_t)lds, run.rep[21] = GT_THREADS;
    TimedRegion timed(ctx, c.slot, c.bytes, c.flops);
    hipLaunchKernelGGL(fn, dim3(run.S, (unsigned)pl.groups.size()), dim3(GT_THREADS), lds, ctx->stream, ctx->d_slot_ptr,
                       run.d_icols, pl.nci, run.d_groups, pl.ct, pl.rb_shift, ctx->n, ctx->d_slab, run.nr_pad, run.nc_pad,
                       ctx->d_zero, run.grid_base);
    return FOKL_OK;
}

static int launch_gram_dma(fokl_ctx *ctx, const GramCall &c, GramLaunch &run, gram_dma_picker pick, int wgs_cap, int nbuf,
                           int loaders)
{
    const GramPlan &pl = run.plan;
    const int nt8 = (pl.nt + 1) / 2, pieces = (pl.ct * 16 * 34 * 8 + 1023) / 1024;
    const size_t lds = (size_t)nbuf * pieces * 1024;
    gram_dma_fn fn = pick(nt8, pl.half, nbuf, 0);
    if (!fn) return no_instance(ctx, "gram_tiles_dma_kernel", pl);
    int rc = raise_lds_limit(ctx, reinterpret_cast<const void *>(fn), lds);
    if (rc) return rc;
    const int by_registers = nt8 == 1 ? 3 : 2;
    if (loaders) {
        gram_dma_fn with = pick(nt8, pl.half, nbuf, loaders);
        if (!with) return no_instance(ctx, "gram_tiles_dma_kernel with loader wavefronts", pl);
        rc = raise_lds_limit(ctx, reinterpret_cast<const void *>(with), lds);
        if (rc) return rc;
        const int per_cu = std::min({wgs_cap, blocks_per_cu(fn, GD_THREADS, lds), by_registers});
        if (blocks_per_cu(with, GD_THREADS + 64 * loaders, lds) >= per_cu)
            fn = with;
        else
            loaders = 0;
    }
    const int64_t n_chunks = (ctx->n + 31) / 32;
    rc = size_slabs(ctx, run, pinned_row_cut(wgs_cap, by_registers, lds, pl.groups.size(), n_chunks), 1, n_chunks);
    if (rc) return rc;
    const uint32_t zero_units =
        (uint32_t)((reinterpret_cast<uintptr_t>(ctx->d_zero) - reinterpret_cast<uintptr_t>(run.grid_base)) >> 8);
    run.rep[0] = FOKL_GRAM_DMA, run.rep[1] = nt8, run.rep[3] = loaders, run.rep[4] = nbuf, run.rep[7] = 32, run.rep[11] = pieces;
    run.rep[12] = (int64_t)lds, run.rep[21] = GD_THREADS + 64 * loaders;
    TimedRegion timed(ctx, c.slot, c.bytes, c.flops);
    hipLaunchKernelGGL(fn, dim3(run.S, (unsigned)pl.groups.size()), dim3(GD_THREADS + 64 * loaders), lds, ctx->stream,
                       run.d_groups, pl.ct, pieces, ctx->n, ctx->d_slab, run.nr_pad, run.nc_pad, run.grid_base, zero_units);
    return FOKL_OK;
}

#ifdef FOKL_DEV_KERNELS
#include "fokl_gram_dev.inc"
#endif

static int launch_gram(fokl_ctx *ctx, const GramCall &c, const LaunchKnobs &knobs, int path, GramLaunch &run)
{
    if (path == 1) return launch_gram_valu(ctx, c, run);
    if (path == 2) {
        const int rc = stage_gram_tiles(ctx, c, knobs.mfma4 == 2 ? 1 : 0, knobs, run);
        if (rc) return rc;
    }
#ifdef FOKL_DEV_KERNELS
    bool taken = false;
    const int rc = launch_gram_dev(ctx, c, knobs, path, run, taken);
    if (taken) return rc;
#endif
    if (path == 3) return fail(ctx, FOKL_ERR_ARG, "fokl_gram: path 3 (round-1 panel kernel) needs a development build");
    if (run.plan.ks > 1) return launch_gram_tiles(ctx, c, run, ksplit_kernel(run.plan), knobs.wgs);
    return launch_gram_dma(ctx, c, run, tiles_dma_kernel, knobs.wgs, 2, knobs.loaders);
}

static int gram_enqueue(fokl_ctx *ctx, const int32_t *row_slots, int nr, const int32_t *col_slots, int nc, int path,
                        int allreduce, bool aside)
{
    std::memset(ctx->gram_report, 0, sizeof ctx->gram_report);
    if (!ctx->have_data) return fail(ctx, FOKL_ERR_STATE, "fokl_gram: call fokl_upload first");
    if (nr <= 0 || nc <= 0) return fail(ctx, FOKL_ERR_ARG, "fokl_gram: empty block");
    if (path < 0 || path > 3) return fail(ctx, FOKL_ERR_ARG, "fokl_gram: path must be 0, 1, 2 or 3");
    HIP_TRY(ctx, hipSetDevice(ctx->device));
    int rc = check_slots(ctx, row_slots, nr, "fokl_gram");
    if (rc) return rc;
    rc = check_slots(ctx, col_slots, nc, "fokl_gram");
    if (rc) return rc;

    const LaunchKnobs knobs = launch_knobs();
    if (path == 0) path = (int64_t)nr * nc > 64 ? knobs.path : 1;
    if (path < 1 || path > 3) path = 2;
    const double *grid_base = path == 2 ? slot_grid_base(ctx) : nullptr;
    if (path == 2 && !grid_base) path = 3;
    rc = aside ? ensure_gout(ctx, (size_t)nr * nc) : ensure_out(ctx, (size_t)nr * nc);
    if (rc) return rc;
    double *d_dst = aside ? ctx->d_gout : ctx->d_out;
    double *h_dst = aside ? ctx->h_gout : ctx->h_out;

    std::vector<int32_t> uniq(row_slots, row_slots + nr);
    uniq.insert(uniq.end(), col_slots, col_slots + nc);
    std::sort(uniq.begin(), uniq.end());
    const double distinct = (double)(std::unique(uniq.begin(), uniq.end()) - uniq.begin());
    GramCall call = {row_slots, col_slots, nr, nc, FOKL_K_GRAM, 8.0 * (double)ctx->n * distinct,
                     2.0 * (double)ctx->n * (double)nr * (double)nc};
    if (call.flops / FOKL_PEAK_F64_FLOPS > call.bytes / FOKL_PEAK_HBM_BYTES_PER_S) call.slot = FOKL_K_GRAM_MFMA;
    if (const char *trace = std::getenv("FOKL_GRAM_TRACE")) {
        if (FILE *fh = std::fopen(trace, "a")) {
            std::fprintf(fh, "%d %d %d %s\n", nr, nc, (int)distinct, call.slot == FOKL_K_GRAM_MFMA ? "gram_mfma" : "gram");
            std::fclose(fh);
        }
    }

    GramLaunch run;
    run.grid_base = grid_base;
    rc = launch_gram(ctx, call, knobs, path, run);
    if (rc) return rc;
    HIP_TRY(ctx, hipGetLastError());

    const int total = nr * nc, epb = reduce_elements_per_block(total);
    {
        TimedRegion timed(ctx, FOKL_K_GRAM_REDUCE, 8.0 * ((double)run.slabs + 1.0) * total, 0.0);
        if (run.d_perm)
            hipLaunchKernelGGL(reduce_slabs_sym_kernel, dim3((total + epb - 1) / epb), dim3(RD_THREADS), 0, ctx->stream,
                               ctx->d_slab, run.slabs, nr, nc, run.nr_pad, run.nc_pad, epb, run.d_perm, d_dst);
        else
            hipLaunchKernelGGL(reduce_slabs_kernel, dim3((total + epb - 1) / epb), dim3(RD_THREADS), 0, ctx->stream,
                               ctx->d_slab, run.slabs, nr, nc, run.nr_pad, run.nc_pad, epb, d_dst);
    }
    HIP_TRY(ctx, hipGetLastError());
    if (allreduce && ctx->comm) {
        rc = comm_allreduce_device(ctx, d_dst, (size_t)nr * nc);
        if (rc) return rc;
    }
    HIP_TRY(ctx, hipMemcpyAsync(h_dst, d_dst, (size_t)nr * nc * sizeof(double), hipMemcpyDeviceToHost, ctx->stream));
    run.rep[13] = run.S, run.rep[15] = run.nr_pad, run.rep[16] = run.nc_pad, run.rep[17] = run.slabs, run.rep[18] = epb;
    std::memcpy(ctx->gram_report, run.rep, sizeof run.rep);
    return FOKL_OK;
}

extern "C" int fokl_gram(fokl_ctx *ctx, const int32_t *row_slots, int nr, const int32_t *col_slots, int nc,
                         double *out, int path, int allreduce)
{
    if (!ctx) return fail(nullptr, FOKL_ERR_ARG, "fokl_gram: null context");
    if (!out) return fail(ctx, FOKL_ERR_ARG, "fokl_gram: null output");
    int rc = gram_enqueue(ctx, row_slots, nr, col_slots, nc, path, allreduce, false);
    if (rc) return rc;
    HIP_TRY(ctx, hipStreamSynchronize(ctx->stream));
    std::memcpy(out, ctx->h_out, (size_t)nr * nc * sizeof(double));
    return FOKL_OK;
}

extern "C" int fokl_gram_launch(fokl_ctx *ctx, const int32_t *row_slots, int nr, const int32_t *col_slots, int nc,
                                int allreduce)
{
    if (!ctx) return fail(nullptr, FOKL_ERR_ARG, "fokl_gram_launch: null context");
    ctx->gram_pending = 0;
    int rc = gram_enqueue(ctx, row_slots, nr, col_slots, nc, 0, allreduce, true);
    if (rc) return rc;
    HIP_TRY(ctx, hipEventRecord(ctx->gram_done, ctx->stream));
    ctx->gram_pending = (size_t)nr * nc;
    return FOKL_OK;
}

extern "C" int fokl_gram_ready(fokl_ctx *ctx)
{
    if (!ctx) return fail(nullptr, FOKL_ERR_ARG, "fokl_gram_ready: null context");
    if (!ctx->gram_pending) return fail(ctx, FOKL_ERR_STATE, "fokl_gram_ready: nothing launched");
    const hipError_t st = hipEventQuery(ctx->gram_done);
    if (st == hipSuccess) return 1;
    if (st == hipErrorNotReady) return 0;
    return fail(ctx, FOKL_ERR_HIP, std::string("hipEventQuery: ") + hipGetErrorString(st));
}

extern "C" int fokl_gram_fetch(fokl_ctx *ctx, double *out, int64_t count)
{
    if (!ctx || !out) return fail(ctx, FOKL_ERR_ARG, "fokl_gram_fetch: null pointer");
    if (!ctx->gram_pending) return fail(ctx, FOKL_ERR_STATE, "fokl_gram_fetch: nothing launched");
    if (count != (int64_t)ctx->gram_pending)
        return fail(ctx, FOKL_ERR_ARG, "fokl_gram_fetch: the launched block has a different size");
    HIP_TRY(ctx, hipSetDevice(ctx->device));
    HIP_TRY(ctx, hipEventSynchronize(ctx->gram_done));
    std::memcpy(out, ctx->h_gout, ctx->gram_pending * sizeof(double));
    ctx->gram_pending = 0;
    return FOKL_OK;
}


extern "C" int fokl_bic_resid_launch(fokl_ctx *ctx, const int32_t *slots, int nc, const double *betahat)
{
    if (!ctx) return fail(nullptr, FOKL_ERR_ARG, "fokl_bic_resid_launch: null context");
    std::memset(ctx->resid_report, 0, sizeof ctx->resid_report);
    if (!ctx->have_data) return fail(ctx, FOKL_ERR_STATE, "fokl_bic_resid_launch: call fokl_upload first");
    if (nc <= 0 || !betahat) return fail(ctx, FOKL_ERR_ARG, "fokl_bic_resid_launch: empty model or null pointer");
    if (ctx->resid_pending) return fail(ctx, FOKL_ERR_STATE, "fokl_bic_resid_launch: previous launch not fetched");
    HIP_TRY(ctx, hipSetDevice(ctx->device));
    int rc = check_slots(ctx, slots, nc, "fokl_bic_resid_launch");
    if (rc) return rc;

    const size_t beta_off = ((size_t)nc * sizeof(int) + 7) & ~(size_t)7;
    const size_t arg_bytes = beta_off + (size_t)nc * sizeof(double);
    rc = begin_args(ctx, arg_bytes);
    if (rc) return rc;
    std::memcpy(ctx->h_args, slots, (size_t)nc * sizeof(int));
    std::memcpy(ctx->h_args + beta_off, betahat, (size_t)nc * sizeof(double));
    rc = push_args(ctx, arg_bytes);
    if (rc) return rc;

    const int64_t n_row_blocks = (ctx->n + RS_THREADS * 2 - 1) / (RS_THREADS * 2);
    const int S = (int)std::max<int64_t>(1, std::min<int64_t>(n_row_blocks, (int64_t)cu_count(ctx) * 8));
    rc = ensure_slab(ctx, (size_t)S * 2);
    if (rc) return rc;
    rc = ensure_rout(ctx);
    if (rc) return rc;
    {
        {
            TimedRegion timed(ctx, FOKL_K_RESID, 8.0 * (double)ctx->n * (double)(nc + 1), 2.0 * (double)ctx->n * nc);
            hipLaunchKernelGGL(resid_kernel, dim3(S), dim3(RS_THREADS), 0, ctx->stream, ctx->d_slot_ptr,
                               reinterpret_cast<const int *>(ctx->d_args),
                               nc, reinterpret_cast<const double *>(ctx->d_args + beta_off),
                               ctx->slot_ptr[FOKL_SLOT_Y], ctx->n, ctx->d_slab);
        }
        HIP_TRY(ctx, hipGetLastError());
        hipLaunchKernelGGL(reduce_slabs_kernel, dim3(1), dim3(RD_THREADS), 0, ctx->stream, ctx->d_slab, S, 1, 2, 1, 2,
                           2, ctx->d_rout);
        HIP_TRY(ctx, hipGetLastError());
    }
    HIP_TRY(ctx, hipMemcpyAsync(ctx->h_rout, ctx->d_rout, 2 * sizeof(double), hipMemcpyDeviceToHost, ctx->stream));
    HIP_TRY(ctx, hipEventRecord(ctx->resid_done, ctx->stream));
    ctx->resid_pending = true;
    {
        const int64_t rep[FOKL_RESID_REPORT_LEN] = {FOKL_RESID_COLUMNS, nc, (nc + RS_BATCH - 1) / RS_BATCH, S, n_row_blocks};
        std::memcpy(ctx->resid_report, rep, sizeof rep);
    }
    return FOKL_OK;
}

typedef void (*resid_quad_fn)(const double *, int64_t, int64_t, const double *, int, const ResidQuadTable *, const double *,
                              double *);

struct ResidQuadLayout {
    int gm, km;
    resid_quad_fn bernoulli2, bernoulli4, bernoulli8, splines;
};
#define FOKL_RQ_LAYOUT(GM, KM)                                                                          \
    {GM, KM, resid_quadratic_kernel<false, GM, KM, 2>, resid_quadratic_kernel<false, GM, KM, 4>,        \
     resid_quadratic_kernel<false, GM, KM, RT_MAX_ORDER>, resid_quadratic_kernel<true, GM, KM, 2>}
static const ResidQuadLayout kResidQuadLayouts[] = {FOKL_RQ_LAYOUT(8, 1), FOKL_RQ_LAYOUT(16, 1), FOKL_RQ_LAYOUT(8, 2),
                                                    FOKL_RQ_LAYOUT(4, 4), FOKL_RQ_LAYOUT(2, 8), FOKL_RQ_LAYOUT(8, 4),
                                                    FOKL_RQ_LAYOUT(16, 2), FOKL_RQ_LAYOUT(4, 8)};
#undef FOKL_RQ_LAYOUT

extern "C" int fokl_bic_resid_terms_launch(fokl_ctx *ctx, const int32_t *terms, int n_terms, const double *betahat)
{
    if (!ctx) return fail(nullptr, FOKL_ERR_ARG, "fokl_bic_resid_terms_launch: null context");
    std::memset(ctx->resid_report, 0, sizeof ctx->resid_report);
    if (!ctx->have_data) return fail(ctx, FOKL_ERR_STATE, "fokl_bic_resid_terms_launch: call fokl_upload first");
    if (n_terms < 0 || !betahat || (n_terms > 0 && !terms))
        return fail(ctx, FOKL_ERR_ARG, "fokl_bic_resid_terms_launch: null pointer");
    if (ctx->resid_pending) return fail(ctx, FOKL_ERR_STATE, "fokl_bic_resid_terms_launch: previous launch not fetched");
    HIP_TRY(ctx, hipSetDevice(ctx->device));
    const int m = ctx->m;
    const bool splines = ctx->kernel == FOKL_KERNEL_SPLINES;

    std::map<int, std::vector<int>> orders_of;
    for (int j = 0; j < n_terms; ++j) {
        int nz = 0;
        for (int k = 0; k < m; ++k) {
            const int o = terms[(size_t)j * m + k];
            if (o < 0 || o > ctx->n_basis)
                return fail(ctx, FOKL_ERR_ARG, "fokl_bic_resid_terms_launch: basis order " + std::to_string(o) +
                                                   " outside [0, " + std::to_string(ctx->n_basis) + "]");
            if (o != 0) {
                if (!splines && o > RT_MAX_ORDER)
                    return fail(ctx, FOKL_ERR_ARG, "fokl_bic_resid_terms_launch: Bernoulli order " + std::to_string(o) +
                                                       " beyond " + std::to_string(RT_MAX_ORDER) +
                                                       " (FOKL_RESID_TERMS_MAX_ORDER)");
                std::vector<int> &os = orders_of[k];
                auto at = std::lower_bound(os.begin(), os.end(), o);
                if (at == os.end() || *at != o) os.insert(at, o);
                ++nz;
            }
        }
        if (nz == 0) return fail(ctx, FOKL_ERR_ARG, "fokl_bic_resid_terms_launch: term with no input (all-zero row)");
        if (nz > 2)
            return fail(ctx, FOKL_ERR_ARG, "fokl_bic_resid_terms_launch: a term has more than two factors (the stored-column "
                                           "pass, fokl_bic_resid_launch, takes such models)");
    }
    const int G = (int)orders_of.size();
    int K = 1, top_order = 1;
    for (const auto &kv : orders_of) {
        K = std::max(K, (int)kv.second.size());
        top_order = std::max(top_order, kv.second.back());
    }
    const ResidQuadLayout *layout = nullptr;
    for (const ResidQuadLayout &l : kResidQuadLayouts)
        if (G <= l.gm && K <= l.km) {
            layout = &l;
            break;
        }
    if (!layout)
        return fail(ctx, FOKL_ERR_ARG, "fokl_bic_resid_terms_launch: " + std::to_string(G) + " inputs with up to " +
                                           std::to_string(K) + " orders each fit none of the factor layouts (8 x 1, 16 x 1, "
                                           "8 x 2, 4 x 4, 2 x 8, 8 x 4, 16 x 2, 4 x 8: FOKL_RESID_TERMS_MAX_FACTORS slots)");
    const int GM = layout->gm, KM = layout->km, UM = GM * KM;

    int rc = begin_args(ctx, sizeof(ResidQuadTable));
    if (rc) return rc;
    ResidQuadTable *tab = reinterpret_cast<ResidQuadTable *>(ctx->h_args);
    std::memset(tab, 0, sizeof(ResidQuadTable));
    tab->n_groups = G;
    std::map<std::pair<int, int>, int> slot_of;
    double flops_per_row = 5.0;
    {
        int g = 0;
        for (const auto &kv : orders_of) {
            tab->input[g] = kv.first;
            tab->omax[g] = kv.second.back();
            flops_per_row += 8.0 * std::max(0, kv.second.back() - 1);
            for (size_t k = 0; k < kv.second.size(); ++k) {
                const int o = kv.second[k], u = g * KM + (int)k;
                slot_of[std::make_pair(kv.first, o)] = u;
                if (!splines)
                    for (int q = 0; q <= o; ++q) tab->coef[u][q] = ctx->h_phis[(size_t)(o - 1) * ctx->width + q];
                tab->coef[u][9] = (double)o;
                flops_per_row += splines ? 14.0 : 2.0 * o;
            }
            ++g;
        }
    }
    tab->c0 = betahat[0];
    for (int j = 0; j < n_terms; ++j) {
        int fa = -1, fb = -1;
        for (int k = 0; k < m; ++k) {
            const int o = terms[(size_t)j * m + k];
            if (o != 0) (fa < 0 ? fa : fb) = slot_of[std::make_pair(k, o)];
        }
        if (fb < 0)
            tab->lin[fa] += betahat[j + 1];
        else
            tab->quad[resid_quad_index(fa, fb, UM, KM)] += betahat[j + 1];
    }
    flops_per_row += 2.0 * 2.0 * (UM + UM * (UM - 1) / 2 - GM * (KM * (KM - 1) / 2));
    rc = push_args(ctx, sizeof(ResidQuadTable));
    if (rc) return rc;

    const int64_t n_row_blocks = (ctx->n + RS_THREADS * 2 - 1) / (RS_THREADS * 2);
    const int S = (int)std::max<int64_t>(1, std::min<int64_t>(n_row_blocks, (int64_t)cu_count(ctx) * 8));
    rc = ensure_slab(ctx, (size_t)S * 2);
    if (rc) return rc;
    rc = ensure_rout(ctx);
    if (rc) return rc;
    resid_quad_fn fn = splines ? layout->splines : top_order <= 2 ? layout->bernoulli2 : top_order <= 4 ? layout->bernoulli4 : layout->bernoulli8;
    {
        {
            TimedRegion timed(ctx, FOKL_K_RESID_MF, 8.0 * (double)ctx->n * (double)(G + 1),
                              (double)ctx->n * flops_per_row);
            hipLaunchKernelGGL(fn, dim3(S), dim3(RS_THREADS), 0, ctx->stream, ctx->d_x, ctx->ld, ctx->n, ctx->d_phis,
                               ctx->width, reinterpret_cast<const ResidQuadTable *>(ctx->d_args), ctx->slot_ptr[FOKL_SLOT_Y],
                               ctx->d_slab);
        }
        HIP_TRY(ctx, hipGetLastError());
        hipLaunchKernelGGL(reduce_slabs_kernel, dim3(1), dim3(RD_THREADS), 0, ctx->stream, ctx->d_slab, S, 1, 2, 1, 2,
                           2, ctx->d_rout);
        HIP_TRY(ctx, hipGetLastError());
    }
    HIP_TRY(ctx, hipMemcpyAsync(ctx->h_rout, ctx->d_rout, 2 * sizeof(double), hipMemcpyDeviceToHost, ctx->stream));
    HIP_TRY(ctx, hipEventRecord(ctx->resid_done, ctx->stream));
    ctx->resid_pending = true;
    {
        const int64_t rep[FOKL_RESID_REPORT_LEN] = {FOKL_RESID_MATRIX_FREE, n_terms, 0, S, n_row_blocks, GM, KM,
                                                    splines ? 0 : top_order <= 2 ? 2 : top_order <= 4 ? 4 : RT_MAX_ORDER, G};
        std::memcpy(ctx->resid_report, rep, sizeof rep);
    }
    return FOKL_OK;
}

extern "C" int fokl_bic_resid_fetch(fokl_ctx *ctx, double *out, int allreduce)
{
    if (!ctx || !out) return fail(ctx, FOKL_ERR_ARG, "fokl_bic_resid_fetch: null pointer");
    if (!ctx->resid_pending) return fail(ctx, FOKL_ERR_STATE, "fokl_bic_resid_fetch: nothing was launched");
    HIP_TRY(ctx, hipSetDevice(ctx->device));
    ctx->resid_pending = false;
    if (allreduce && ctx->comm) {
        int rc = comm_allreduce_device(ctx, ctx->d_rout, 2);
        if (rc) return rc;
        HIP_TRY(ctx, hipMemcpyAsync(ctx->h_rout, ctx->d_rout, 2 * sizeof(double), hipMemcpyDeviceToHost, ctx->stream));
        HIP_TRY(ctx, hipEventRecord(ctx->resid_done, ctx->stream));
    }
    HIP_TRY(ctx, hipEventSynchronize(ctx->resid_done));
    out[0] = ctx->h_rout[0];
    out[1] = ctx->h_rout[1];
    return FOKL_OK;
}

extern "C" int fokl_bic_resid(fokl_ctx *ctx, const int32_t *slots, int nc, const double *betahat, double *out,
                              int allreduce)
{
    if (!out) return fail(ctx, FOKL_ERR_ARG, "fokl_bic_resid: null output");
    int rc = fokl_bic_resid_launch(ctx, slots, nc, betahat);
    if (rc) return rc;
    return fokl_bic_resid_fetch(ctx, out, allreduce);
}

extern "C" int fokl_fit_report(const fokl_ctx *ctx, int which, int64_t *out, int count)
{
    if (!ctx || !out || count < 0) return fail(nullptr, FOKL_ERR_ARG, "fokl_fit_report: null argument");
    const int64_t *src = which == FOKL_REPORT_GRAM ? ctx->gram_report : which == FOKL_REPORT_RESID ? ctx->resid_report
                         : which == FOKL_REPORT_BASIS ? ctx->basis_report : nullptr;
    const int len = which == FOKL_REPORT_GRAM ? FOKL_GRAM_REPORT_LEN : which == FOKL_REPORT_RESID ? FOKL_RESID_REPORT_LEN
                                                                                                  : FOKL_BASIS_REPORT_LEN;
    if (!src) return fail(nullptr, FOKL_ERR_ARG, "fokl_fit_report: which must be FOKL_REPORT_GRAM, _RESID or _BASIS");
    std::memcpy(out, src, (size_t)std::min(count, len) * sizeof(int64_t));
    return FOKL_OK;
}


extern "C" int fokl_read_slot(fokl_ctx *ctx, int slot, int64_t row0, int64_t nrows, double *host)
{
    if (!ctx) return fail(nullptr, FOKL_ERR_ARG, "fokl_read_slot: null context");
    if (!ctx->have_data) return fail(ctx, FOKL_ERR_STATE, "fokl_read_slot: call fokl_upload first");
    int32_t s = slot;
    int rc = check_slots(ctx, &s, 1, "fokl_read_slot");
    if (rc) return rc;
    if (row0 < 0 || nrows < 0 || row0 + nrows > ctx->n || (nrows > 0 && !host))
        return fail(ctx, FOKL_ERR_ARG, "fokl_read_slot: row range outside the dataset");
    HIP_TRY(ctx, hipSetDevice(ctx->device));
    HIP_TRY(ctx, hipStreamSynchronize(ctx->stream));
    HIP_TRY(ctx, hipMemcpy(host, ctx->slot_ptr[slot] + row0, (size_t)nrows * sizeof(double), hipMemcpyDeviceToHost));
    return FOKL_OK;
}

extern "C" int fokl_write_slot(fokl_ctx *ctx, int slot, int64_t row0, int64_t nrows, const double *host)
{
    if (!ctx) return fail(nullptr, FOKL_ERR_ARG, "fokl_write_slot: null context");
    if (!ctx->have_data) return fail(ctx, FOKL_ERR_STATE, "fokl_write_slot: call fokl_upload first");
    int32_t s = slot;
    int rc = check_slots(ctx, &s, 1, "fokl_write_slot");
    if (rc) return rc;
    if (row0 < 0 || nrows < 0 || row0 + nrows > ctx->n || (nrows > 0 && !host))
        return fail(ctx, FOKL_ERR_ARG, "fokl_write_slot: row range outside the dataset");
    HIP_TRY(ctx, hipSetDevice(ctx->device));
    HIP_TRY(ctx, hipStreamSynchronize(ctx->stream));
    HIP_TRY(ctx, hipMemcpy(ctx->slot_ptr[slot] + row0, host, (size_t)nrows * sizeof(double), hipMemcpyHostToDevice));
    return FOKL_OK;
}


extern "C" int fokl_timing_enable(fokl_ctx *ctx, int on)
{
    if (!ctx) return fail(nullptr, FOKL_ERR_ARG, "fokl_timing_enable: null context");
    ctx->timing = on != 0;
    return FOKL_OK;
}

extern "C" int fokl_timing_reset(fokl_ctx *ctx)
{
    if (!ctx) return fail(nullptr, FOKL_ERR_ARG, "fokl_timing_reset: null context");
    (void)hipStreamSynchronize(ctx->stream);
    drain_events(ctx);
    for (auto &t : ctx->tslot) t = TimingSlot();
    return FOKL_OK;
}

extern "C" int fokl_timing_get(fokl_ctx *ctx, int kernel_id, double *total_ms, int64_t *launches, double *bytes,
                               double *flops, double *ideal_ms)
{
    if (!ctx) return fail(nullptr, FOKL_ERR_ARG, "fokl_timing_get: null context");
    if (kernel_id < 0 || kernel_id >= FOKL_K_COUNT) return fail(ctx, FOKL_ERR_ARG, "fokl_timing_get: bad kernel id");
    HIP_TRY(ctx, hipStreamSynchronize(ctx->stream));
    drain_events(ctx);
    if (total_ms) *total_ms = ctx->tslot[kernel_id].ms;
    if (launches) *launches = ctx->tslot[kernel_id].launches;
    if (bytes) *bytes = ctx->tslot[kernel_id].bytes;
    if (flops) *flops = ctx->tslot[kernel_id].flops;
    if (ideal_ms) *ideal_ms = ctx->tslot[kernel_id].ideal_ms;
    return FOKL_OK;
}

#include "fokl_comm.inc"
#include "fokl_chain_device.inc"
#include "fokl_spectral_device.inc"
#include "fokl_predict.inc"
#include "fokl_population.inc"
#include "fokl_integrate_device.inc"
#include "fokl_simulate_device.inc"
#include "fokl_assimilate_device.inc"
#include "fokl_control_device.inc"
#include "fokl_control_pooled_device.inc"
#include "fokl_control_cvar_device.inc"
#include "fokl_probe.inc"
#include "fokl_dgemm_device.inc"
#include "fokl_optimize_core.inc"
#include "fokl_optimize_device.inc"
#include "fokl_optimize_system_device.inc"
#include "fokl_infer_device.inc"
#include "fokl_embedded_device.inc"
#include "fokl_resample_device.inc"
#include "fokl_score_device.inc"
#include "fokl_design_device.inc"

#if defined(FOKL_GT_STAMP) || defined(FOKL_GD_STAMP)
extern "C" int fokl_debug_stamps_read(unsigned long long *out, int count)
{
    return hipMemcpyFromSymbol(out, HIP_SYMBOL(fokl::fokl_debug_stamps), sizeof(unsigned long long) * count) == hipSuccess ? 0 : -1;
}

extern "C" int fokl_debug_stamps_clear()
{
    static const unsigned long long zeros[8192] = {};
    return hipMemcpyToSymbol(HIP_SYMBOL(fokl::fokl_debug_stamps), zeros, sizeof(zeros)) == hipSuccess ? 0 : -1;
}
#endif
```

### fokl_gpy_amd/csrc/fokl_kernels.hip.h

```cpp
#pragma once
#include <hip/hip_runtime.h>
#include <stdint.h>

namespace fokl {

constexpr int WAVE = 64;
constexpr int K1_THREADS = 256;
constexpr int K1_ROWS_PER_THREAD = 2;
constexpr int K1_MAX_LDS_SLABS = 4;

typedef double d2 __attribute__((ext_vector_type(2)));
typedef double d4 __attribute__((ext_vector_type(4)));

typedef __attribute__((address_space(1))) const d2 *global_cd2_ptr;
typedef __attribute__((address_space(1))) d2 *global_d2_ptr;
typedef __attribute__((address_space(1))) double *global_d_ptr;
typedef __attribute__((address_space(1))) const double *global_cd_ptr;

__device__ __forceinline__ d2 load_d2(const double *p) { return *(global_cd2_ptr)(p); }
#ifndef FOKL_STREAM_NT
#define FOKL_STREAM_NT 1
#endif
__device__ __forceinline__ d2 load_d2_stream(const double *p)
{
// ... 50 lines not shown

__device__ __forceinline__ double bernoulli_basis_d1(const double *__restrict__ c, int order, double x)
{
    double s = 0.0;
    double ph = 1.0, pl = 0.0;
    for (int k = 2; k <= order; ++k) {
        dd_mul_d(ph, pl, x);
        s = s + ((double)k * c[k]) * ph;
    }
    return c[1] + s;
}

__device__ __forceinline__ double bernoulli_basis_d2(const double *__restrict__ c, int order, double x)
{
    double s = 0.0;
    double ph = 1.0, pl = 0.0;
    for (int k = 2; k <= order; ++k) {
        if (k > 2) dd_mul_d(ph, pl, x);
        s = s + ((double)((k - 1) * k) * c[k]) * ph;
    }
    return s;
}

__device__ __forceinline__ double cubic_basis_d1(double c1, double c2, double c3, double t)
{
    double r = c1 + (2.0 * c2) * t;
    return r + (3.0 * c3) * (t * t);
}

__device__ __forceinline__ double cubic_basis_d2(double c2, double c3, double t) { return 2.0 * c2 + (6.0 * c3) * t; }

__device__ __forceinline__ void spline_locate(double x, int width, bool twice_normalised, int &piece, double &t)
{
    double xl = x * (double)width;
    int p = (int)ceil(xl);
    if (p == 0) p = 1;
    p -= 1;
    if (twice_normalised) {
        const double r = 1.0 / (double)width;
        t = (x - (double)p * r) / r;
    } else {
        t = xl - (double)p;
    }
    piece = min(max(p, 0), width - 1);
}

struct DerivSpec {
    int input;
    int order;
    double div;
    int twice_normalised;
};

template <bool SPLINES, typename SlabPtr>
__device__ __forceinline__ void evaluate_factor(SlabPtr sl, const double *__restrict__ bern, int order,
                                                int width, d2 x, int p0, int p1, double t0, double t1, int deriv,
                                                double div, double &vx, double &vy)
{
    if (SPLINES) {
        if (deriv == 0) {
            vx = cubic_basis(sl[p0], sl[width + p0], sl[2 * width + p0], sl[3 * width + p0], t0);
            vy = cubic_basis(sl[p1], sl[width + p1], sl[2 * width + p1], sl[3 * width + p1], t1);
        } else if (deriv == 1) {
            vx = cubic_basis_d1(sl[width + p0], sl[2 * width + p0], sl[3 * width + p0], t0) / div;
            vy = cubic_basis_d1(sl[width + p1], sl[2 * width + p1], sl[3 * width + p1], t1) / div;
        } else {
            vx = cubic_basis_d2(sl[2 * width + p0], sl[3 * width + p0], t0) / div;
            vy = cubic_basis_d2(sl[2 * width + p1], sl[3 * width + p1], t1) / div;
        }
    } else {
        if (deriv == 0) {
            vx = bernoulli_basis(bern, order, x.x);
            vy = bernoulli_basis(bern, order, x.y);
        } else if (deriv == 1) {
            vx = bernoulli_basis_d1(bern, order, x.x) / div;
            vy = bernoulli_basis_d1(bern, order, x.y) / div;
        } else {
            vx = bernoulli_basis_d2(bern, order, x.x) / div;
            vy = bernoulli_basis_d2(bern, order, x.y) / div;
        }
    }
}

template <bool SPLINES>
__global__ __launch_bounds__(K1_THREADS) void basis_build_kernel(
    const double *__restrict__ xT, int64_t ld, int64_t n, const double *__restrict__ phis, int width,
    const BasisPlan *__restrict__ plan, const int *__restrict__ arr, double *const *__restrict__ slot_ptr,
    DerivSpec deriv)
{
    __builtin_amdgcn_s_setprio(3);
    extern __shared__ __attribute__((aligned(16))) double lds[];
    const int U = plan->n_fac, T = plan->n_terms, NS = plan->n_slabs;
    const int *fac_input = arr;
    const int *fac_order = arr + U;
    const int *fac_slab = arr + 2 * U;
    const int *slab_order = arr + 3 * U;
    const int *term_off = arr + 3 * U + K1_MAX_LDS_SLABS;
    const int *term_fac = term_off + (T + 1);
    const int *term_slot = term_fac + term_off[T];

    const int tid = threadIdx.x;
    const int nthr = blockDim.x;
    double *slabs = lds;
    const int slab_doubles = SPLINES ? ((NS * 4 * width + 1) & ~1) : 0;
    d2 *fac = reinterpret_cast<d2 *>(lds + slab_doubles);

    if (SPLINES) {
        for (int s = 0; s < NS; ++s) {
            const double *src = phis + (size_t)(slab_order[s] - 1) * 4 * width;
            for (int i = tid; i < 4 * width; i += nthr) slabs[s * 4 * width + i] = src[i];
        }
        __syncthreads();
    }

    const int tile_rows = nthr * K1_ROWS_PER_THREAD;
    const int64_t n_tiles = (n + tile_rows - 1) / tile_rows;
    for (int64_t tile = blockIdx.x; tile < n_tiles; tile += gridDim.x) {
        const int64_t r0 = tile * tile_rows + (int64_t)tid * K1_ROWS_PER_THREAD;
        const bool in0 = r0 < n, in1 = r0 + 1 < n;

        int cur_input = -1;
        d2 x = {0.0, 0.0};
        int p0 = 0, p1 = 0;
        double t0 = 0.0, t1 = 0.0;
        for (int u = 0; u < U; ++u) {
            const int k = fac_input[u], order = fac_order[u];
            if (k != cur_input) {
                cur_input = k;
                if (in0) x = *reinterpret_cast<const d2 *>(xT + (size_t)k * ld + r0);
                if (SPLINES) {
                    spline_locate(x.x, width, deriv.twice_normalised != 0, p0, t0);
                    spline_locate(x.y, width, deriv.twice_normalised != 0, p1, t1);
                }
            }
            d2 v;
            {
                const int s = SPLINES ? fac_slab[u] : -1;
                const double *bern = SPLINES ? nullptr : phis + (size_t)(order - 1) * width;
                const int dv = k == deriv.input ? deriv.order : 0;
                double vx, vy;
                if (SPLINES && s < 0)
                    evaluate_factor<SPLINES>((global_cd_ptr)(phis + (size_t)(order - 1) * 4 * width), bern, order, width,
                                             x, p0, p1, t0, t1, dv, deriv.div, vx, vy);
                else
                    evaluate_factor<SPLINES>((const double *)(slabs + (SPLINES ? s : 0) * 4 * width), bern, order, width,
                                             x, p0, p1, t0, t1, dv, deriv.div, vx, vy);
                v.x = vx;
                v.y = vy;
            }
            fac[u * nthr + tid] = v;
        }

        for (int j = 0; j < T; ++j) {
            const int b = term_off[j], e = term_off[j + 1];
            d2 phi = fac[term_fac[b] * nthr + tid];
            for (int f = b + 1; f < e; ++f) {
                const d2 g = fac[term_fac[f] * nthr + tid];
                phi.x = phi.x * g.x;
                phi.y = phi.y * g.y;
            }
            double *col = slot_ptr[term_slot[j]];
            if (in1) {
                store_d2(col + r0, phi);
            } else if (in0) {
                store_d1(col + r0, phi.x);
            }
        }
    }
}

constexpr int K1_REG_FACTORS = 16;

template <bool SPLINES>
__global__ __launch_bounds__(K1_THREADS) void basis_build_reg_kernel(
    const double *__restrict__ xT, int64_t ld, int64_t n, const double *__restrict__ phis, int width,
    const BasisPlan *__restrict__ plan, const int *__restrict__ arr, double *const *__restrict__ slot_ptr,
    DerivSpec deriv)
{
    __builtin_amdgcn_s_setprio(3);
    extern __shared__ __attribute__((aligned(16))) double lds[];
    const int U = plan->n_fac, T = plan->n_terms, NS = plan->n_slabs;
    const int *fac_input = arr;
    const int *fac_order = arr + U;
    const int *fac_slab = arr + 2 * U;
    const int *slab_order = arr + 3 * U;
    const int *term_off = arr + 3 * U + K1_MAX_LDS_SLABS;
    const int *term_fac = term_off + (T + 1);
    const int *term_slot = term_fac + term_off[T];

    const int tid = threadIdx.x;
    const int nthr = blockDim.x;
    double *slabs = lds;
    if (SPLINES) {
        for (int s = 0; s < NS; ++s) {
            const double *src = phis + (size_t)(slab_order[s] - 1) * 4 * width;
            for (int i = tid; i < 4 * width; i += nthr) slabs[s * 4 * width + i] = src[i];
        }
        __syncthreads();
    }

    const int tile_rows = nthr * K1_ROWS_PER_THREAD;
    const int64_t n_tiles = (n + tile_rows - 1) / tile_rows;
    for (int64_t tile = blockIdx.x; tile < n_tiles; tile += gridDim.x) {
        const int64_t r0 = tile * tile_rows + (int64_t)tid * K1_ROWS_PER_THREAD;
        const bool in0 = r0 < n, in1 = r0 + 1 < n;
        double fx[K1_REG_FACTORS], fy[K1_REG_FACTORS];

        int cur_input = -1;
        d2 x = {0.0, 0.0};
        int p0 = 0, p1 = 0;
        double t0 = 0.0, t1 = 0.0;
        for (int u = 0; u < U; ++u) {
            const int k = fac_input[u], order = fac_order[u];
            if (k != cur_input) {
                cur_input = k;
                if (in0) x = *reinterpret_cast<const d2 *>(xT + (size_t)k * ld + r0);
                if (SPLINES) {
                    spline_locate(x.x, width, deriv.twice_normalised != 0, p0, t0);
                    spline_locate(x.y, width, deriv.twice_normalised != 0, p1, t1);
                }
            }
            double vx, vy;
            {
                const int s = SPLINES ? fac_slab[u] : -1;
                const double *bern = SPLINES ? nullptr : phis + (size_t)(order - 1) * width;
                const int dv = k == deriv.input ? deriv.order : 0;
                if (SPLINES && s < 0)
                    evaluate_factor<SPLINES>((global_cd_ptr)(phis + (size_t)(order - 1) * 4 * width), bern, order, width,
                                             x, p0, p1, t0, t1, dv, deriv.div, vx, vy);
                else
                    evaluate_factor<SPLINES>((const double *)(slabs + (SPLINES ? s : 0) * 4 * width), bern, order, width,
                                             x, p0, p1, t0, t1, dv, deriv.div, vx, vy);
            }
            fx[u] = vx;
            fy[u] = vy;
        }

        for (int j = 0; j < T; ++j) {
            const int b = term_off[j], e = term_off[j + 1];
            const int a0 = term_fac[b];
            d2 phi = {fx[a0], fy[a0]};
            for (int f = b + 1; f < e; ++f) {
                const int g = term_fac[f];
                phi.x = phi.x * fx[g];
                phi.y = phi.y * fy[g];
            }
            double *col = slot_ptr[term_slot[j]];
            if (in1) {
                store_d2(col + r0, phi);
            } else if (in0) {
                store_d1(col + r0, phi.x);
            }
        }
    }
}


__global__ void transpose_inputs_kernel(const double *__restrict__ x, const double *__restrict__ y, int64_t n, int m,
                                        int64_t ld, double *__restrict__ xT, double *__restrict__ ones,
                                        double *__restrict__ ycol, const double *__restrict__ bounds)
{
    for (int64_t i = (int64_t)blockIdx.x * blockDim.x + threadIdx.x; i < ld; i += (int64_t)gridDim.x * blockDim.x) {
        const bool in = i < n;
        for (int k = 0; k < m; ++k) {
            double v = in ? x[(size_t)i * m + k] : 0.0;
            if (bounds && in) v = (v - bounds[k]) / bounds[m + k];
            xT[(size_t)k * ld + i] = v;
        }
        ones[i] = in ? 1.0 : 0.0;
        ycol[i] = in ? y[i] : 0.0;
    }
}

__global__ void rows_from_columns_kernel(const double *__restrict__ xT, int64_t n, int m, int64_t ld, double *__restrict__ rows)
{
    for (int64_t i = (int64_t)blockIdx.x * blockDim.x + threadIdx.x; i < n; i += (int64_t)gridDim.x * blockDim.x)
        for (int k = 0; k < m; ++k) rows[(size_t)i * m + k] = xT[(size_t)k * ld + i];
}

__device__ __forceinline__ double nan_min(double a, double b) { return (b < a || b != b) ? b : a; }
__device__ __forceinline__ double nan_max(double a, double b) { return (b > a || b != b) ? b : a; }

__global__ void column_bounds_kernel(const double *__restrict__ x, int64_t total, int m, int64_t lanes, double *__restrict__ part)
{
    const int64_t t = (int64_t)blockIdx.x * blockDim.x + threadIdx.x;
    if (t >= lanes) return;
    double lo = x[t < total ? t : t % m], hi = lo;
    for (int64_t at = t + lanes; at < total; at += lanes) {
        const double v = x[at];
        lo = nan_min(lo, v);
        hi = nan_max(hi, v);
    }
    part[t] = lo;
    part[lanes + t] = hi;
}

__global__ void column_bounds_finish_kernel(const double *__restrict__ part, int64_t lanes, int m, double *__restrict__ out)
{
    __shared__ double lo_s[256], hi_s[256];
    const int k = blockIdx.x, tid = threadIdx.x;
    double lo = part[k], hi = part[lanes + k];
    for (int64_t t = k + (int64_t)tid * m; t < lanes; t += (int64_t)256 * m) {
        lo = nan_min(lo, part[t]);
        hi = nan_max(hi, part[lanes + t]);
    }
    lo_s[tid] = lo;
    hi_s[tid] = hi;
    __syncthreads();
    for (int w = 128; w > 0; w >>= 1) {
        if (tid < w) {
            lo_s[tid] = nan_min(lo_s[tid], lo_s[tid + w]);
            hi_s[tid] = nan_max(hi_s[tid], hi_s[tid + w]);
        }
        __syncthreads();
    }
    if (tid == 0) {
        out[k] = lo_s[0];
        out[m + k] = hi_s[0];
    }
}


__device__ __forceinline__ double wave_sum(double v)
{
#pragma unroll
    for (int off = WAVE / 2; off > 0; off >>= 1) v += __shfl_down(v, off, WAVE);
    return v;
}


constexpr int GV_THREADS = 256;
constexpr int GV_TI = 4, GV_TJ = 4;

__global__ __launch_bounds__(GV_THREADS) void gram_valu_kernel(double *const *__restrict__ slot_ptr,
                                                               const int *__restrict__ row_slots, int nr,
                                                               const int *__restrict__ col_slots, int nc, int64_t n,
                                                               double *__restrict__ slab, int nr_pad, int nc_pad)
// ... 544 lines not shown
        fokl_debug_stamps[2 * blockIdx.x] = __builtin_amdgcn_s_memtime() - stamp_c0;
        fokl_debug_stamps[2 * blockIdx.x + 1] = __builtin_amdgcn_s_memrealtime() - stamp_r0;
    }
#endif
#ifdef FOKL_GD_STAMP
    if (lane == 0 && (wave == 0 || wave == 7) && blockIdx.y == 0 && blockIdx.x < 512) {
        unsigned long long *st = fokl_debug_stamps + 8 * blockIdx.x + (wave == 7 ? 4 : 0);
        st[0] = ph_issue;
        st[1] = ph_mult;
        st[2] = ph_wait;
        st[3] = ph_bar;
    }
#endif
    double *out = slab + (size_t)blockIdx.x * nr_pad * nc_pad;
    asm volatile("" ::: "memory");
    if (half_real) {
        const int oi = g.oi[row][first], oj = g.oj[row][first];
#pragma unroll
        for (int q = 0; q < 2; ++q) out[(size_t)(16 * oi + 4 * q + fk) * nc_pad + 16 * oj + fm] = hacc[q];
    }
#pragma unroll
    for (int k = 0; k < NT; ++k) {
        const int j = E0 + 2 * k + first;
        if (j < GT_MAX_NT) {
            const int oi = g.oi[row][j], oj = g.oj[row][j];
            if (oi != 0xFFFF) {
#pragma unroll
                for (int v = 0; v < 4; ++v) out[(size_t)(16 * oi + fk + 4 * v) * nc_pad + 16 * oj + fm] = acc[k][v];
            }
        }
    }
}

__global__ __launch_bounds__(RD_THREADS) void reduce_slabs_sym_kernel(const double *__restrict__ slab, int S, int nr,
                                                                      int nc, int nr_pad, int nc_pad, int epb,
                                                                      const int *__restrict__ perm,
                                                                      double *__restrict__ out)
{
    __shared__ double part_sum[RD_THREADS];
    const int parts = RD_THREADS / epb;
    const int el = threadIdx.x % epb, part = threadIdx.x / epb;
    const int e = blockIdx.x * epb + el;
    const int total = nr * nc;
    double acc = 0.0;
    if (e < total) {
        int i = e / nc, c = perm[e % nc];
        if ((c >> 4) < (i >> 4)) {
            const int t = i;
            i = c;
            c = t;
        }
        const size_t plane = (size_t)nr_pad * nc_pad;
        const double *p = slab + (size_t)i * nc_pad + c;
        double a[8] = {0.0, 0.0, 0.0, 0.0, 0.0, 0.0, 0.0, 0.0};
        int k = part;
        for (; k + 7 * parts < S; k += 8 * parts) {
            double v[8];
#pragma unroll
            for (int u = 0; u < 8; ++u) v[u] = p[(size_t)(k + u * parts) * plane];
#pragma unroll
            for (int u = 0; u < 8; ++u) a[u] += v[u];
        }
        for (int u = 0; k < S; k += parts, ++u) a[u & 7] += p[(size_t)k * plane];
        acc = ((a[0] + a[1]) + (a[2] + a[3])) + ((a[4] + a[5]) + (a[6] + a[7]));
    }
    part_sum[threadIdx.x] = acc;
    __syncthreads();
    if (part == 0 && e < total) {
        double s = part_sum[el];
        for (int q = 1; q < parts; ++q) s += part_sum[q * epb + el];
        out[e] = s;
    }
}


constexpr int RS_THREADS = 256;
constexpr int RS_BATCH = 256;

struct ResidCol {
    const double *ptr;
    double beta;
};

__global__ __launch_bounds__(RS_THREADS) void resid_kernel(double *const *__restrict__ slot_ptr,
                                                           const int *__restrict__ slots, int nc,
                                                           const double *__restrict__ beta,
                                                           const double *__restrict__ y, int64_t n,
                                                           double *__restrict__ slab)
{
    __builtin_amdgcn_s_setprio(3);
    __shared__ __attribute__((aligned(16))) ResidCol cols[RS_BATCH];
    __shared__ double red[RS_THREADS / WAVE][2];
    const int tid = threadIdx.x;
    double s1 = 0.0, s2 = 0.0;
    const int64_t n_tiles = (n + RS_THREADS * 2 - 1) / (RS_THREADS * 2);
    const bool single_batch = nc <= RS_BATCH;
    if (single_batch) {
        for (int j = tid; j < nc; j += RS_THREADS) cols[j] = ResidCol{slot_ptr[slots[j]], beta[j]};
        __syncthreads();
    }
    for (int64_t tile = blockIdx.x; tile < n_tiles; tile += gridDim.x) {
        const int64_t r = (tile * RS_THREADS + tid) * 2;
        const bool in0 = r < n, in1 = r + 1 < n;
        d2 fit = {0.0, 0.0};
        for (int c0 = 0; c0 < nc; c0 += RS_BATCH) {
            const int cnt = min(RS_BATCH, nc - c0);
            if (!single_batch) {
                __syncthreads();
                for (int j = tid; j < cnt; j += RS_THREADS) cols[j] = ResidCol{slot_ptr[slots[c0 + j]], beta[c0 + j]};
                __syncthreads();
            }
            if (in0) {
#pragma unroll 8
                for (int j = 0; j < cnt; ++j) {
                    const ResidCol c = cols[j];
                    const d2 xv = load_d2_stream(c.ptr + r);
                    fit.x = __builtin_fma(c.beta, xv.x, fit.x);
                    fit.y = __builtin_fma(c.beta, xv.y, fit.y);
                }
            }
        }
        if (in0) {
            const d2 yv = *reinterpret_cast<const d2 *>(y + r);
            const double r0 = yv.x - fit.x;
            const double r1 = in1 ? yv.y - fit.y : 0.0;
            s1 += r0 + r1;
            s2 += r0 * r0 + r1 * r1;
        }
    }
    const int wave = tid / WAVE, lane = tid % WAVE;
    s1 = wave_sum(s1);
    s2 = wave_sum(s2);
    if (lane == 0) {
        red[wave][0] = s1;
        red[wave][1] = s2;
    }
    __syncthreads();
    if (tid < 2) {
        double s = red[0][tid];
#pragma unroll
        for (int w = 1; w < RS_THREADS / WAVE; ++w) s += red[w][tid];
        slab[(size_t)blockIdx.x * 2 + tid] = s;
    }
}



constexpr int RT_MAX_ORDER = 8;
constexpr int RT_COEF_STRIDE = 10;
constexpr int RQ_MAX_SLOTS = 32;

struct ResidQuadTable {
    int32_t n_groups;
    int32_t pad;
    int32_t input[RQ_MAX_SLOTS];
    int32_t omax[RQ_MAX_SLOTS];
    double c0;
    double coef[RQ_MAX_SLOTS][RT_COEF_STRIDE];
    double lin[RQ_MAX_SLOTS];
    double quad[RQ_MAX_SLOTS * (RQ_MAX_SLOTS - 1) / 2];
};

__host__ __device__ constexpr int resid_quad_index(int a, int b, int UM, int KM)
{
    int q = 0;
    for (int i = 0; i < UM; ++i)
        for (int j = i + 1; j < UM; ++j) {
            if (i / KM == j / KM) continue;
            if (i == a && j == b) return q;
            ++q;
        }
    return -1;
}

typedef __attribute__((address_space(4))) const ResidQuadTable *const_quad_ptr;

template <bool SPLINES, int GM, int KM, int OT>
__global__ __launch_bounds__(RS_THREADS) void resid_quadratic_kernel(
    const double *__restrict__ xT, int64_t ld, int64_t n, const double *__restrict__ phis, int width,
    const ResidQuadTable *__restrict__ table, const double *__restrict__ y, double *__restrict__ slab)
{
    constexpr int UM = GM * KM;
    static_assert(UM <= RQ_MAX_SLOTS && OT >= 2 && OT <= RT_MAX_ORDER, "slot layout");
    __builtin_amdgcn_s_setprio(3);
    __shared__ double red[RS_THREADS / WAVE][2];
    const const_quad_ptr tab = (const_quad_ptr)(uintptr_t)table;
    const int tid = threadIdx.x;
    const int G = tab->n_groups;

    double s1 = 0.0, s2 = 0.0;
    const int64_t n_tiles = (n + RS_THREADS * 2 - 1) / (RS_THREADS * 2);
    for (int64_t tile = blockIdx.x; tile < n_tiles; tile += gridDim.x) {
        const int64_t r = (tile * RS_THREADS + tid) * 2;
        const bool in0 = r < n, in1 = r + 1 < n;
        if (!in0) continue;
        d2 xv[GM];
#pragma unroll
        for (int g = 0; g < GM; ++g) xv[g] = load_d2(xT + (size_t)tab->input[g < G ? g : 0] * ld + r);
        const d2 yv = load_d2(y + r);

        double f[UM][2];
#pragma unroll
        for (int g = 0; g < GM; ++g) {
            const double x[2] = {xv[g].x, xv[g].y};
            if (SPLINES) {
                int piece[2];
                double t[2];
#pragma unroll
                for (int q = 0; q < 2; ++q) spline_locate(x[q], width, false, piece[q], t[q]);
#pragma unroll
                for (int k = 0; k < KM; ++k) {
                    const int order = (int)tab->coef[g * KM + k][9];
                    const global_cd_ptr sl = (global_cd_ptr)(phis + (size_t)((order > 0 ? order : 1) - 1) * 4 * width);
#pragma unroll
                    for (int q = 0; q < 2; ++q) {
                        const double v = cubic_basis(sl[piece[q]], sl[width + piece[q]], sl[2 * width + piece[q]],
                                                     sl[3 * width + piece[q]], t[q]);
                        f[g * KM + k][q] = order > 0 ? v : 0.0;
                    }
                }
            } else {
                double pw[OT + 1][2];
                {
                    double ph[2], pl[2];
#pragma unroll
                    for (int q = 0; q < 2; ++q) {
                        pw[1][q] = ph[q] = x[q];
                        pl[q] = 0.0;
// ... 64 lines not shown
```

### fokl_gpy_amd/csrc/fokl_run.cpp

```cpp
#include <algorithm>
#include <chrono>
#include <cmath>
#include <cstdint>
#include <cstring>
#include <map>
#include <memory>
#include <string>
#include <vector>

#include "../../include/fokl_hip_internal.h"

extern void fokl_set_global_error(const std::string &msg);

namespace {

inline double now_s()
{
    return 1e-9 * (double)std::chrono::duration_cast<std::chrono::nanoseconds>(
                      std::chrono::steady_clock::now().time_since_epoch())
                      .count();
}

using Gram = std::shared_ptr<std::vector<double>>;

// ... 98 lines not shown

    void give(std::vector<int32_t> slots)
    {
        std::sort(slots.begin(), slots.end(), [](int32_t x, int32_t y) { return x > y; });
        free_list.insert(free_list.end(), slots.begin(), slots.end());
    }
};

struct Ahead {
    bool valid = false;
    std::vector<int32_t> vecs;
    int T = 0;
    std::vector<int32_t> slots;
    int over = 0;
    bool pending = false;
    bool built = false;
    std::vector<double> block;
};

struct SpectrumRef {
    fokl_spectrum *h = nullptr;
    Gram gram;
};

Gram extend_gram(const std::vector<double> &gram, int A, const std::vector<int> &keep, const std::vector<double> &block, int vm,
                 int block_ld, const std::vector<int> &block_kept, int over)
{
    const int n_prev = (int)keep.size(), A2 = n_prev + vm, L = A2 + 1, old = A + 1;
    auto out = std::make_shared<std::vector<double>>((size_t)L * L);
    double *o = out->data();
    for (int i = 0; i < n_prev; ++i) {
        const double *src = gram.data() + (size_t)keep[(size_t)i] * old;
        for (int j = 0; j < n_prev; ++j) o[(size_t)i * L + j] = src[keep[(size_t)j]];
        o[(size_t)i * L + A2] = o[(size_t)A2 * L + i] = src[A];
    }
    o[(size_t)A2 * L + A2] = gram[(size_t)A * old + A];
    for (int r = 0; r < vm; ++r) {
        const double *b = block.data() + (size_t)r * block_ld;
        double *row = o + (size_t)(n_prev + r) * L;
        for (int j = 0; j < n_prev; ++j) {
            const double v = b[block_kept[(size_t)j]];
            row[j] = v;
            o[(size_t)j * L + n_prev + r] = v;
        }
        for (int c = 0; c < vm; ++c) row[n_prev + c] = b[over + c];
        row[A2] = o[(size_t)A2 * L + n_prev + r] = b[over + vm];
    }
    return out;
}

}

struct fokl_run {
    fokl_backend_ops ops{};
    fokl_run_params prm{};
    Slots pool;
    Patterns patterns;
    std::vector<double> base;
    Ahead ahead;
    bool have_next = false;
    int next_stage = 0;
    std::vector<int32_t> next_indvec;
    std::vector<int32_t> mtx;
    int mtx_rows = 0;
    std::vector<double> evs;
    fokl_outcome *best_model = nullptr, *last_model = nullptr;
    std::vector<double> stat_mean_abs, stat_rel_std;
    std::vector<int32_t> stat_sizes;
    double stats[FOKL_RUN_STATS] = {};
    std::string error;
};

namespace {

int run_fail(fokl_run *r, int code, const std::string &msg)
{
    if (r) r->error = msg;
    fokl_set_global_error(msg);
    return code;
}

enum RunStat {
    R_TERMS_PHYSICAL, R_SUBSTAGES, R_FORECASTS_USED, R_FORECASTS_EARLY, R_RESID_MATRIX_FREE, R_T_RESID, R_PHASE_PREPARE,
    R_PHASE_MODEL, R_PHASE_STATISTICS, R_PHASE_TESTS, R_PHASE_WRAP_UP, R_COUNT
};
static_assert(R_COUNT <= FOKL_RUN_STATS, "fokl_run_stats: grow FOKL_RUN_STATS");

int matrix_free_pay_from(const fokl_backend_ops &ops, const std::vector<int32_t> &terms, int rows, int m)
{
    static const int layouts[8][2] = {{8, 1}, {16, 1}, {8, 2}, {4, 4}, {2, 8}, {8, 4}, {16, 2}, {4, 8}};
    if (!ops.bic_resid_terms_launch || rows < 1) return -1;
    int max_order = 0;
    for (int t = 0; t < rows; ++t) {
        int nz = 0;
        for (int j = 0; j < m; ++j) {
            const int v = terms[(size_t)t * m + j];
            nz += v != 0;
            max_order = std::max(max_order, v);
        }
        if (nz > 2) return -1;
    }
    if (max_order == 0) return -1;
    if (ops.kernel_id != 0 && max_order > 8) return -1;
    int inputs = 0, deepest = 0;
    for (int j = 0; j < m; ++j) {
        std::vector<int32_t> seen;
        for (int t = 0; t < rows; ++t) {
            const int v = terms[(size_t)t * m + j];
            if (v != 0 && std::find(seen.begin(), seen.end(), v) == seen.end()) seen.push_back(v);
        }
        inputs += !seen.empty();
        deepest = std::max(deepest, (int)seen.size());
    }
    int best = -1;
    for (auto &l : layouts)
        if (inputs <= l[0] && deepest <= l[1] && (best < 0 || l[0] * l[1] < best)) best = l[0] * l[1];
    if (best < 0) return -1;
    return ops.kernel_id != 0 ? 0 : (int)(3.5 * best);
}

static const bool g_build_at_start = !(std::getenv("FOKL_BUILD_AHEAD_AT") && std::strcmp(std::getenv("FOKL_BUILD_AHEAD_AT"), "model") == 0);

struct Loop {
    fokl_run *r;
    fokl_search *s;
    const fokl_backend_ops &ops;
    const fokl_run_params &prm;
    int m;
    std::vector<int32_t> damtx;
    std::vector<int32_t> model_slots;
    std::vector<int> keep;
    Gram gram;
    int gram_A = 0;
    std::vector<int32_t> active_slots;
    int A = 0, vm = 0, n_prev = 0, vm_next = -1;
    Gram cur;
    std::vector<int32_t> terms_arr;
    int terms_pay_from = 0;
    std::map<std::vector<int64_t>, int64_t> term_ids;
    std::vector<SpectrumRef> early;
    std::vector<std::vector<int32_t>> early_keys;
    std::vector<int32_t> predicted_kills;
    bool have_predicted = false;
    Ahead ahead;
    bool have_coming = false;
    int coming_stage = 0;
    std::vector<int32_t> coming_indvec;
    struct Forecast {
        std::vector<int32_t> key;
        SpectrumRef sp;
    };
    std::vector<Forecast> forecasts;
    std::vector<fokl_outcome *> outcomes, retiring;
    int rc_cb = FOKL_OK;

    Loop(fokl_run *run, fokl_search *search) : r(run), s(search), ops(run->ops), prm(run->prm), m(run->prm.m) {}

    void release(SpectrumRef &sp)
    {
        if (sp.h) fokl_spectrum_release(s, sp.h);
        sp.h = nullptr;
        sp.gram.reset();
    }

    std::vector<int32_t> columns_without(int count, const std::vector<int32_t> &removed) const
    {
        std::vector<int32_t> out;
        for (int c = 0; c < count; ++c)
            if (std::find(removed.begin(), removed.end(), c) == removed.end()) out.push_back(c);
        return out;
    }

    int fetch_block(Ahead &a)
    {
        if (a.pending) {
            const int nc = a.over + a.T + 1;
            a.block.resize((size_t)a.T * nc);
            const int rc = ops.gram_fetch(ops.ctx, a.block.data(), (int64_t)a.T * nc);
            if (rc != FOKL_OK) return rc;
            a.pending = false;
        }
        return FOKL_OK;
    }

    int build_ahead(const std::vector<int32_t> &indvec, const std::vector<int32_t> &active, Ahead *out)
    {
        Ahead a;
        int rc = build_ahead_columns(indvec, &a);
        if (rc == FOKL_OK) rc = launch_ahead_gram(active, &a);
        if (rc != FOKL_OK) return rc;
        *out = std::move(a);
        return FOKL_OK;
    }

    int build_ahead_columns(const std::vector<int32_t> &indvec, Ahead *a)
    {
        a->vecs = arrangements(indvec);
        a->T = (int)(a->vecs.size() / (size_t)m);
        int rc = r->pool.take(a->T, &a->slots);
        if (rc != FOKL_OK) return rc;
        if ((rc = ops.build_terms(ops.ctx, a->vecs.data(), a->T, a->slots.data())) != FOKL_OK) return rc;
        r->stats[R_TERMS_PHYSICAL] += a->T;
        a->built = true;
        return FOKL_OK;
    }

    int launch_ahead_gram(const std::vector<int32_t> &active, Ahead *a)
    {
        a->over = (int)active.size();
        std::vector<int32_t> cols(active);
        cols.insert(cols.end(), a->slots.begin(), a->slots.end());
        cols.push_back(FOKL_SLOT_Y);
        const int rc = ops.gram_launch(ops.ctx, a->slots.data(), a->T, cols.data(), (int)cols.size(), 0);
        if (rc != FOKL_OK) return rc;
        a->pending = true;
        a->valid = true;
        return FOKL_OK;
    }

    void release_retired()
    {
        for (fokl_outcome *o : retiring) {
            fokl_outcome_release(s, o);
            fokl_outcome_drop(s, o);
        }
        retiring.clear();
    }

    void retire(fokl_outcome *keep_a, fokl_outcome *keep_b)
    {
        std::vector<fokl_outcome *> kept;
        for (fokl_outcome *o : outcomes) {
            if (o == keep_a || o == keep_b) {
                if (std::find(kept.begin(), kept.end(), o) == kept.end()) kept.push_back(o);
            } else {
                retiring.push_back(o);
            }
        }
        outcomes = kept;
    }

    int set_active_terms()
    {
        const int rows = (int)(damtx.size() / (size_t)m);
        std::vector<int64_t> ids((size_t)rows + 1);
        ids[0] = (int64_t)term_ids.emplace(std::vector<int64_t>(), (int64_t)term_ids.size()).first->second;
        for (int t = 0; t < rows; ++t) {
            std::vector<int64_t> key(damtx.begin() + (size_t)t * m, damtx.begin() + (size_t)(t + 1) * m);
            ids[(size_t)t + 1] = term_ids.emplace(std::move(key), (int64_t)term_ids.size()).first->second;
        }
        const int rc = fokl_search_set_substage(s, ids.data(), rows + 1);
        if (rc != FOKL_OK) return rc;
        terms_arr.clear();
        if (prm.matrix_free && rows > 0) {
            const int pay = matrix_free_pay_from(ops, damtx, rows, m);
            if (pay >= 0) {
                terms_arr.assign((size_t)m, 0);
                terms_arr.insert(terms_arr.end(), damtx.begin(), damtx.end());
                terms_pay_from = pay;
            }
        }
        return FOKL_OK;
    }

    int speculate(const std::vector<std::pair<int, bool>> &sizes)
    {
        std::vector<int32_t> sz, mod;
        for (auto &p : sizes) {
            sz.push_back(p.first);
            mod.push_back(p.second ? 1 : 0);
        }
        return fokl_search_speculate(s, sz.data(), mod.data(), (int)sz.size());
    }

    int guess_first_tests(fokl_spectrum *spectrum, int n_new, double siglik, bool before_model,
                          std::vector<std::pair<int, bool>> *tests_out = nullptr)
    {
        std::vector<int32_t> cols((size_t)std::max(1, n_new)), accepted((size_t)std::max(1, n_new));
        int count = 0;
        int rc = fokl_search_likely_first_tests(s, spectrum, n_new, siglik, cols.data(), accepted.data(), &count);
        if (rc != FOKL_OK) return rc;
        std::vector<int32_t> curset;
        std::vector<std::pair<int, bool>> sizes;
        if (before_model) sizes.push_back({A, true});
        fokl_spectrum *against = spectrum;
        (void)fokl_search_hold_spectral(s, 1);
        for (int i = 0; i < count && rc == FOKL_OK; ++i) {
            std::vector<int32_t> trial(curset);
            trial.push_back(cols[(size_t)i]);
            std::sort(trial.begin(), trial.end());
            fokl_spectrum *job = nullptr;
            if ((int)early.size() <= std::min(prm.lookahead_native, 3)) {
                int pos = -1;
                if (against) {
                    const auto without = columns_without(A, curset);
                    pos = (int)(std::lower_bound(without.begin(), without.end(), cols[(size_t)i]) - without.begin());
// ... 43 lines not shown
        fokl_spectrum *job = nullptr;
        if ((rc_cb = fokl_search_spectral_from(s, g->data(), L + 1, idx.data(), L, nullptr, -1, &job)) != FOKL_OK) return;
        rc_cb = fokl_search_register_forecast(s, key.data(), (int)key.size(), job, (*g)[(size_t)L * (L + 1) + L]);
        forecasts.push_back({key, {job, g}});
    }

    static void cb_foresee(void *user, const int32_t *killed, int count) { static_cast<Loop *>(user)->foresee(killed, count); }

    static int cb_residual(void *user, const int32_t *idx, int p1, const double *betahat, double *s1, double *s2)
    {
        Loop *l = static_cast<Loop *>(user);
        std::vector<int32_t> slots((size_t)p1);
        for (int i = 0; i < p1; ++i) slots[(size_t)i] = l->active_slots[(size_t)idx[i]];
        double out[2] = {0, 0};
        const int rc = l->ops.bic_resid(l->ops.ctx, slots.data(), p1, betahat, out, 0);
        *s1 = out[0];
        *s2 = out[1];
        return rc;
    }

    int run();
};

int Loop::run()
{
    fokl_run *R = r;
    double tick = now_s();
    auto lap = [&](int which) {
        const double t = now_s();
        R->stats[which] += t - tick;
        tick = t;
    };
    const int half0 = prm.half0, half1 = (int)std::ceil(prm.draws / 2.0 + 1.0);
    gram = std::make_shared<std::vector<double>>(R->base);
    gram_A = 1;
    keep = {0};
    ahead = std::move(R->ahead);
    R->ahead = Ahead();
    int stage = 0;
    std::vector<int32_t> indvec;
    bool have_pattern = R->have_next;
    if (have_pattern) {
        stage = R->next_stage;
        indvec = R->next_indvec;
    } else {
        have_pattern = R->patterns.next(&stage, &indvec);
    }
    std::vector<double> &evs = R->evs;
    fokl_outcome *betas = nullptr, *last = nullptr;
    std::vector<int32_t> mtx, last_damtx;
    int greater = 0;
    int rc = FOKL_OK;

    while (have_pattern) {
        have_coming = R->patterns.next(&coming_stage, &coming_indvec);
        n_prev = 1 + (int)model_slots.size();
        SpectrumRef spectral_job;
        std::vector<int32_t> vecs, new_slots;
        if (ahead.valid) {
            vecs = ahead.vecs;
            new_slots = ahead.slots;
            bool hit = false;
            for (auto &f : forecasts)
                if (!hit && f.key == model_slots) {
                    spectral_job = f.sp;
                    f.sp = SpectrumRef();
                    hit = true;
                }
            if ((rc = fetch_block(ahead)) != FOKL_OK) return rc;
            if (hit) {
                cur = spectral_job.gram;
                R->stats[R_FORECASTS_USED] += 1;
            } else {
                cur = extend_gram(*gram, gram_A, keep, ahead.block, ahead.T, ahead.over + ahead.T + 1, keep, ahead.over);
            }
            fokl_search_clear_forecasts(s);
            for (auto &f : forecasts) release(f.sp);
            forecasts.clear();
            ahead = Ahead();
        } else {
            vecs = arrangements(indvec);
            const int T = (int)(vecs.size() / (size_t)m);
            if ((rc = R->pool.take(T, &new_slots)) != FOKL_OK) return rc;
            if ((rc = ops.build_terms(ops.ctx, vecs.data(), T, new_slots.data())) != FOKL_OK) return rc;
            R->stats[R_TERMS_PHYSICAL] += T;
            std::vector<int32_t> cols{FOKL_SLOT_ONES};
            cols.insert(cols.end(), model_slots.begin(), model_slots.end());
            cols.insert(cols.end(), new_slots.begin(), new_slots.end());
            cols.push_back(FOKL_SLOT_Y);
            std::vector<double> block((size_t)T * cols.size());
            if ((rc = ops.gram(ops.ctx, new_slots.data(), T, cols.data(), (int)cols.size(), block.data(), 0, 0)) != FOKL_OK)
                return rc;
            std::vector<int> kept((size_t)n_prev);
            for (int i = 0; i < n_prev; ++i) kept[(size_t)i] = i;
            cur = extend_gram(*gram, gram_A, keep, block, T, (int)cols.size(), kept, n_prev);
        }
        vm = (int)(vecs.size() / (size_t)m);
        damtx.insert(damtx.end(), vecs.begin(), vecs.end());
        const int dam = (int)(damtx.size() / (size_t)m);
        if ((rc = set_active_terms()) != FOKL_OK) return rc;
        active_slots.assign(1, FOKL_SLOT_ONES);
        active_slots.insert(active_slots.end(), model_slots.begin(), model_slots.end());
        active_slots.insert(active_slots.end(), new_slots.begin(), new_slots.end());
        A = (int)active_slots.size();
        vm_next = have_coming ? (int)(arrangements(coming_indvec).size() / (size_t)m) : -1;
        early.clear();
        early_keys.clear();
        have_predicted = false;
        bool guessed = false;
        std::vector<std::pair<int, bool>> then;
        if (vm > 0 && A > 1) then.push_back({A - 1, false});
        if (prm.lookahead > 0 && spectral_job.h && fokl_spectrum_done(spectral_job.h)) {
            if ((rc = guess_first_tests(spectral_job.h, vm, NAN, true, &then)) != FOKL_OK) return rc;
            guessed = true;
        }
        lap(R_PHASE_PREPARE);

        std::vector<int32_t> idx((size_t)A);
        for (int i = 0; i < A; ++i) idx[(size_t)i] = i;
        std::vector<int32_t> then_sizes, then_model;
        for (auto &p : then) {
            then_sizes.push_back(p.first);
            then_model.push_back(p.second ? 1 : 0);
        }
        fokl_spectrum *spectrum = nullptr;
        fokl_tape *tape = nullptr;
        if ((rc = fokl_search_model_begin(s, cur->data(), A + 1, idx.data(), A, spectral_job.h, then_sizes.data(),
                                          then_model.data(), (int)then_sizes.size(), &spectrum, &tape)) != FOKL_OK)
            return rc;
        if (g_build_at_start && have_coming && prm.foresight > 0) {
            if ((rc = build_ahead_columns(coming_indvec, &ahead)) != FOKL_OK) {
                fokl_spectrum_release(s, spectrum);
                return rc;
            }
        }
        const double *buffer = nullptr;
        int p1_check = 0;
        if ((rc = fokl_spectrum_wait(s, spectrum, &buffer, &p1_check)) != FOKL_OK) {
            fokl_spectrum_release(s, spectrum);
            return rc;
        }
        const double *betahat = buffer + 2 * (size_t)A;
        if (!terms_arr.empty() && A >= terms_pay_from) {
            rc = ops.bic_resid_terms_launch(ops.ctx, terms_arr.data() + m, A - 1, betahat);
            R->stats[R_RESID_MATRIX_FREE] += 1;
        } else {
            rc = ops.bic_resid_launch(ops.ctx, active_slots.data(), A, betahat);
        }
        if (rc == FOKL_OK && ahead.built && !ahead.valid) rc = launch_ahead_gram(active_slots, &ahead);
        if (rc == FOKL_OK && !guessed && prm.lookahead > 0 && vm > 0) {
            rc = guess_first_tests(spectrum, vm, NAN, false);
            guessed = rc == FOKL_OK;
        }
        fokl_outcome *full = nullptr;
        if (rc == FOKL_OK) rc = fokl_search_model_commit(s, spectrum, tape, (*cur)[(size_t)A * (A + 1) + A], vm, &full);
        if (rc != FOKL_OK) {
            fokl_spectrum_release(s, spectrum);
            return rc;
        }
        release(spectral_job);
        outcomes.push_back(full);
        auto forecast_now = [&]() {
            if (!(g_build_at_start && prm.forecast_early && ahead.valid && ahead.pending && have_predicted && ops.gram_ready &&
                  forecasts.empty()))
                return;
            if (!ops.gram_ready(ops.ctx)) return;
            foresee(predicted_kills.data(), (int)predicted_kills.size());
            if (rc_cb == FOKL_OK) R->stats[R_FORECASTS_EARLY] += 1;
        };
        forecast_now();
        if (rc_cb != FOKL_OK) return rc_cb;
        {
            const double t0 = now_s();
            double mom[2] = {0, 0};
            if ((rc = ops.bic_resid_fetch(ops.ctx, mom, 0)) != FOKL_OK) return rc;
            R->stats[R_T_RESID] += now_s() - t0;
            forecast_now();
            if (rc_cb != FOKL_OK) return rc_cb;
            double ev_model = 0;
            if ((rc = fokl_search_score(s, full, mom[0], mom[1], n_prev, 0, &ev_model)) != FOKL_OK) return rc;
        }
        fokl_outcome *best = full;
        fokl_outcome_view view{};
        if ((rc = fokl_outcome_info(s, full, &view)) != FOKL_OK) return rc;
        double ev = view.ev;
        lap(R_PHASE_MODEL);

        if (!guessed && prm.lookahead > 0) {
            fokl_spectrum *own = nullptr;
            if ((rc = fokl_outcome_spectrum(s, full, &own)) != FOKL_OK) return rc;
            rc = guess_first_tests(own, vm, view.siglik, false);
            fokl_spectrum_release(s, own);
            if (rc != FOKL_OK) return rc;
        }
        release_retired();
        if (have_coming && prm.foresight > 0 && !ahead.valid && !ahead.built) {
            if ((rc = build_ahead(coming_indvec, active_slots, &ahead)) != FOKL_OK) return rc;
        }
        if (prm.forecast_early && ahead.valid && ahead.pending && have_predicted && ops.gram_ready && forecasts.empty()) {
            for (int polls = prm.forecast_polls; polls > 0 && !fokl_outcome_chain_ready(full); --polls)
                if (ops.gram_ready(ops.ctx)) {
                    foresee(predicted_kills.data(), (int)predicted_kills.size());
                    if (rc_cb != FOKL_OK) return rc_cb;
                    R->stats[R_FORECASTS_EARLY] += 1;
                    break;
                }
        }
        have_predicted = false;

        std::vector<int32_t> new_cols((size_t)vm);
        for (int c = 0; c < vm; ++c) new_cols[(size_t)c] = dam - vm + 1 + c;
        std::vector<double> mean_abs((size_t)std::max(1, vm)), rel_std((size_t)std::max(1, vm));
        if (vm > 0 &&
            (rc = fokl_outcome_new_term_stats(s, full, new_cols.data(), vm, half0, half1, mean_abs.data(), rel_std.data())) != FOKL_OK)
            return rc;
        lap(R_PHASE_STATISTICS);
        R->stat_sizes.push_back(vm);
        R->stat_mean_abs.insert(R->stat_mean_abs.end(), mean_abs.begin(), mean_abs.begin() + vm);
        R->stat_rel_std.insert(R->stat_rel_std.end(), rel_std.begin(), rel_std.begin() + vm);
        std::vector<int> order((size_t)vm);
        for (int c = 0; c < vm; ++c) order[(size_t)c] = c;
        std::stable_sort(order.begin(), order.end(), [&](int x, int y) { return mean_abs[(size_t)x] < mean_abs[(size_t)y]; });
        std::vector<int32_t> cand_col((size_t)std::max(1, vm));
        std::vector<double> mean_sorted((size_t)std::max(1, vm)), rel_sorted((size_t)std::max(1, vm));
        for (int c = 0; c < vm; ++c) {
            cand_col[(size_t)c] = new_cols[(size_t)order[(size_t)c]];
            mean_sorted[(size_t)c] = mean_abs[(size_t)order[(size_t)c]];
            rel_sorted[(size_t)c] = rel_std[(size_t)order[(size_t)c]];
        }
// ... 227 lines not shown
```

### fokl_gpy_amd/engine.py

```python
import collections
import itertools
import threading
import math
import os
import time

import numpy as np
from scipy.linalg import eigh as _eigh

from . import _capi

SLOT_ONES, SLOT_Y, SLOT_FIRST_FREE = _capi.SLOT_ONES, _capi.SLOT_Y, _capi.SLOT_FIRST_FREE
from .host_pipeline import (
    HostPipeline, ShardedSpectralJob, GibbsOutcome, EagerOutcome, NativeOutcome, NativeSpectrum, Misprediction, ModelSize,
    chain_engine_for, spectral_engine_for,
    close_chain_engines, drop_spare_buffers, _mark, _flush_marks, _cpu_budget, _thread_plan, _thread_spares,
    _place_host_threads, _SPARES)



def distinct_arrangements(indvec):
    cur = sorted(float(v) for v in indvec)
    n = len(cur)
    rows = [tuple(cur)]
# ... 984 lines not shown
    def _share_of(self, slots):
        world, rank = self.comm.world, self.comm.rank
        share = -(-len(slots) // world)
        mine = list(slots[rank * share:(rank + 1) * share])
        mine += [slots[-1]] * (share - len(mine))
        return mine, share

    def _gather_rows(self, local, total, share):
        t0 = time.perf_counter()
        parts = self.comm.allgather(np.ascontiguousarray(local).reshape(-1)).reshape(self.comm.world, share, -1)
        self.stats['candidate_gathers'] = self.stats.get('candidate_gathers', 0) + 1
        self.stats['t_candidate_gather'] = self.stats.get('t_candidate_gather', 0.0) + time.perf_counter() - t0
        return np.concatenate([parts[r, :max(0, min(share, total - r * share))] for r in range(self.comm.world)], axis=0)

    def _gram_of_new_columns(self, new_slots, col_slots):
        if not self._candidate_split():
            return self.backend.gram(new_slots, col_slots, self.allreduce)
        mine, share = self._share_of(new_slots)
        return self._gather_rows(self.backend.gram(mine, col_slots, False), len(new_slots), share)

    def _arrangements(self, indvec):
        key = tuple(float(v) for v in indvec)
        hit = self._arrangement_memo.get(key)
        if hit is None:
            hit = self._arrangement_memo[key] = distinct_arrangements(indvec)
            hit.setflags(write=False)
        return hit

    def _build_ahead(self, indvec, active_slots):
        vecs = self._arrangements(indvec)
        slots = self.pool.take(vecs.shape[0])
        self.backend.build_terms(vecs.astype(np.int32), slots)
        self.stats['terms_physical'] += vecs.shape[0]
        ahead = dict(indvec=indvec, vecs=vecs, slots=slots, over=len(active_slots))
        if hasattr(self.backend, 'gram_launch'):
            if self._candidate_split():
                mine, share = self._share_of(slots)
                ahead['share'] = share
                ahead['pending'] = self.backend.gram_launch(mine, active_slots + slots + [SLOT_Y], False)
            else:
                ahead['pending'] = self.backend.gram_launch(slots, active_slots + slots + [SLOT_Y], self.allreduce)
        else:
            ahead['block'] = self._gram_of_new_columns(slots, active_slots + slots + [SLOT_Y])
        return ahead

    def _ahead_block(self, ahead):
        if 'block' not in ahead:
            block = self.backend.gram_fetch(ahead.pop('pending'))
            if 'share' in ahead:
                block = self._gather_rows(block, len(ahead['slots']), ahead.pop('share'))
            ahead['block'] = block
        return ahead['block']

    @staticmethod
    def _extend_gram(gram, keep, block, block_kept, over):
        A = gram.shape[0] - 1
        n_prev, vm = len(keep), block.shape[0]
        A2 = n_prev + vm
        out = np.empty((A2 + 1, A2 + 1))
        out[:n_prev, :n_prev] = gram[np.ix_(keep, keep)]
        out[:n_prev, A2] = out[A2, :n_prev] = gram[keep, A]
        out[A2, A2] = gram[A, A]
        cross = block[:, block_kept]
        out[n_prev:A2, :n_prev] = cross
        out[:n_prev, n_prev:A2] = cross.T
        out[n_prev:A2, n_prev:A2] = block[:, over:over + vm]
        out[n_prev:A2, A2] = out[A2, n_prev:A2] = block[:, over + vm]
        return out

    def _run_native(self):
        nrun, self._nrun = self._nrun, None
        if self._update_args is not None:
            nrun.set_update(*self._update_args)
        try:
            nrun.search(self.native)
            mtx, evs, per_substage, best_h, last_h, st = nrun.result()
        finally:
            nrun.close()
        self.substage_stats = per_substage
        for key in ('terms_physical', 'substages', 'forecasts_used', 'resid_matrix_free'):
            self.stats[key] += int(st[key])
        self.stats['forecasts_early'] = self.stats.get('forecasts_early', 0) + int(st['forecasts_early'])
        self.stats['t_resid'] += st['t_resid']
        self.stats['substage_loop'] = 'native'
        phase = self.stats.setdefault('phases', dict(prepare=0.0, model=0.0, statistics=0.0, tests=0.0, wrap_up=0.0))
        for key in phase:
            phase[key] += st['phase_' + key]
        betas = NativeOutcome(self, self.native, best_h)
        last = betas if last_h == best_h else NativeOutcome(self, self.native, last_h)
        self._outcomes = [betas] if last is betas else [betas, last]
        if self.chain_engine is not None and hasattr(self.chain_engine, 'flush'):
            self.chain_engine.flush()
        return self._finish(betas, mtx, evs, last)

    def _run(self):
        if getattr(self, '_nrun', None) is not None:
            if self.native is not None:
                return self._run_native()
            self._nrun.close()
            self._nrun = None
        m, n = self.m, self.n
        draws = self.draws
        half1 = int(math.ceil(draws / 2 + 1))
        half0 = int(math.ceil(draws / 2))

        model_slots = []
        damtx = np.zeros((0, m))
        head = getattr(self, '_head', None)
        self._head = None
        if head is not None:
            base = head[0]
        else:
            base = self.backend.gram([SLOT_ONES, SLOT_Y], [SLOT_ONES, SLOT_Y], self.allreduce)
        gram = np.array(base, dtype=np.float64)
        keep = [0]

        evs = np.array([])
        betas = mtx = None
        last = None
        last_damtx = damtx
        greater = 0
        patterns = self._patterns()
        pattern = next(patterns)
        ahead = head[1] if head is not None else None
        forecasts = {}
        look_ahead = self.host is not None and self.foresight > 0

        phase = self.stats.setdefault('phases', dict(prepare=0.0, model=0.0, statistics=0.0, tests=0.0, wrap_up=0.0))
        tick = time.perf_counter()

        def lap(name):
            nonlocal tick
            now = time.perf_counter()
            phase[name] += now - tick
            tick = now

        while pattern is not None:
            ind, indvec = pattern
            pattern = next(patterns, None)
            n_prev = 1 + len(model_slots)
            spectral_job = None
            if ahead is not None:
                vecs, new_slots = ahead['vecs'], ahead['slots']
                hit = forecasts.pop(tuple(model_slots), None)
                if hit is not None:
                    spectral_job, gram = hit
                    self.stats['forecasts_used'] += 1
                else:
                    gram = self._extend_gram(gram, keep, self._ahead_block(ahead), keep, ahead['over'])
                self._ahead_block(ahead)
                if self.native is not None:
                    self.native.clear_forecasts()
                ahead, forecasts = None, {}
            else:
                vecs = self._arrangements(indvec)
                new_slots = self.pool.take(vecs.shape[0])
                self.backend.build_terms(vecs.astype(np.int32), new_slots)
                self.stats['terms_physical'] += vecs.shape[0]
                block = self._gram_of_new_columns(new_slots, [SLOT_ONES] + model_slots + new_slots + [SLOT_Y])
                gram = self._extend_gram(gram, keep, block, list(range(n_prev)), n_prev)
            _mark('substage', f"{ind} hit={int(spectral_job is not None)}")
            vm = vecs.shape[0]
            damtx = np.append(damtx, vecs, axis=0)
            dam = damtx.shape[0]
            self._set_active_terms(damtx)
            active_slots = [SLOT_ONES] + model_slots + new_slots
# ... 186 lines not shown
```

### include/fokl_hip_internal.h

```cpp
#ifndef FOKL_HIP_INTERNAL_H
#define FOKL_HIP_INTERNAL_H

#include <stddef.h>

#include "fokl_hip.h"

#ifdef __cplusplus
extern "C" {
#endif


#define FOKL_SEGMENT_BLOCKS 256
#define FOKL_SEGMENT_DOUBLES 79872
#define FOKL_ROW_LEAD (1ull << 63)
#define FOKL_SOURCE_X1_HALF (1ull << 63)
#define FOKL_SOURCE_GIVEN ((1ull << 62) - 1)
#define FOKL_GAMMA_FINAL_VALUE (~0ull)
#define FOKL_PRESTATE_WORDS 640
#define FOKL_PRESTATE_BLOCKS 32
typedef struct fokl_stream fokl_stream;
typedef struct fokl_tape_row {
    uint64_t start;
    uint64_t lead_source;
    uint64_t gamma[2];
// ... 438 lines not shown


#define FOKL_CONTROL_REPORT_LEN 8
#define FOKL_CONTROL_MAX_DECISIONS 32
#define FOKL_CONTROL_MAX_STEPS 4096

int fokl_control_solve(fokl_ctx *ctx, int n_draws, int n_states, int64_t n_steps, double h, int n_forcing_cols,
                       const double *forcing, int n_norm_forcing, int n_norm, const int32_t *norm_src, const double *norm_lo,
                       const double *norm_span, int n_forcing_factors, int n_factors, const int32_t *fac_norm,
                       const int32_t *fac_kind, const int32_t *fac_row, const int32_t *fac_degree, int n_spline_rows,
                       const double *spline_table, int n_bern_rows, const double *bern_table, int n_entries,
                       const int32_t *entries, const int32_t *entry_begin, const int32_t *entry_count, const int32_t *constant,
                       int n_coef, const double *coef, const double *y0, const double *box, int n_controls, int n_segments,
                       const int32_t *seg_first, const int32_t *norm_control, const double *ctl_lo, const double *ctl_width,
                       const double *ref, const double *track_weight, const double *terminal_weight, const double *limit_lo,
                       const double *limit_hi, double limit_weight, const double *move_weight, const double *previous,
                       int has_previous, int n_starts, const double *z0, int max_iter, double tol, double *z, double *cost,
                       double *cost_start, int32_t *status, int32_t *iterations, int32_t *descent_steps, int32_t *best_start,
                       double *members, int32_t *first_saturation, double *first_F, double *first_g, double *first_H);

int fokl_control_report(const fokl_ctx *ctx, int64_t *out);


#define FOKL_CONTROL_POOLED_REPORT_LEN 15
#define FOKL_CONTROL_POOL_CHUNK 64

typedef struct fokl_control_first_trial {
    double *trial;
    double *slope;
    int32_t *moved;
    double *pooled;
    double *ft;
    double *ft_sums;
    double *phi_t;
    double *a_t;
    double *z;
    int32_t *status;
    int32_t *descent;
} fokl_control_first_trial;

int fokl_control_pooled_solve(fokl_ctx *ctx, int n_draws, int n_states, int64_t n_steps, double h, int n_forcing_cols,
                              const double *forcing, int n_norm_forcing, int n_norm, const int32_t *norm_src,
                              const double *norm_lo, const double *norm_span, int n_forcing_factors, int n_factors,
                              const int32_t *fac_norm, const int32_t *fac_kind, const int32_t *fac_row,
                              const int32_t *fac_degree, int n_spline_rows, const double *spline_table, int n_bern_rows,
                              const double *bern_table, int n_entries, const int32_t *entries, const int32_t *entry_begin,
                              const int32_t *entry_count, const int32_t *constant, int n_coef, const double *coef,
                              const double *y0, const double *box, int n_controls, int n_segments, const int32_t *seg_first,
                              const int32_t *norm_control, const double *ctl_lo, const double *ctl_width, const double *ref,
                              const double *track_weight, const double *terminal_weight, const double *limit_lo,
                              const double *limit_hi, double limit_weight, const double *move_weight, const double *previous,
                              int has_previous, int n_starts, const double *z0, int max_iter, double tol,
                              const double *draw_weights, double *z, double *cost, double *cost_start, int32_t *status,
                              int32_t *iterations, int32_t *descent_steps, int32_t *best_start, double *members,
                              int32_t *first_saturation, double *cost_draws, double *first_pooled, double *first_rows,
                              const fokl_control_first_trial *first_trial);

int fokl_control_pooled_report(const fokl_ctx *ctx, int64_t *out);


#define FOKL_CONTROL_CVAR_REPORT_LEN 18

int fokl_control_cvar_solve(fokl_ctx *ctx, int n_draws, int n_states, int64_t n_steps, double h, int n_forcing_cols,
                            const double *forcing, int n_norm_forcing, int n_norm, const int32_t *norm_src,
                            const double *norm_lo, const double *norm_span, int n_forcing_factors, int n_factors,
                            const int32_t *fac_norm, const int32_t *fac_kind, const int32_t *fac_row,
                            const int32_t *fac_degree, int n_spline_rows, const double *spline_table, int n_bern_rows,
                            const double *bern_table, int n_entries, const int32_t *entries, const int32_t *entry_begin,
                            const int32_t *entry_count, const int32_t *constant, int n_coef, const double *coef,
                            const double *y0, const double *box, int n_controls, int n_segments, const int32_t *seg_first,
                            const int32_t *norm_control, const double *ctl_lo, const double *ctl_width, const double *ref,
                            const double *track_weight, const double *terminal_weight, const double *limit_lo,
                            const double *limit_hi, double limit_weight, const double *move_weight, const double *previous,
                            int has_previous, int n_starts, const double *z0, int max_iter, double tol,
                            const double *draw_weights, double alpha, double smoothing, double epsilon, double *z,
                            double *cost, double *cost_start, int32_t *status, int32_t *iterations, int32_t *descent_steps,
                            int32_t *best_start, double *members, int32_t *first_saturation, double *cost_draws,
                            double *epsilon_used, double *first_pooled, double *first_rows, double *first_a, double *first_q,
                            double *first_c, const fokl_control_first_trial *first_trial);

int fokl_control_cvar_report(const fokl_ctx *ctx, int64_t *out);


enum { FOKL_REPORT_GRAM = 0, FOKL_REPORT_RESID = 1, FOKL_REPORT_BASIS = 2 };
#define FOKL_GRAM_REPORT_LEN 24
#define FOKL_RESID_REPORT_LEN 10
#define FOKL_BASIS_REPORT_LEN 24
enum {
    FOKL_GRAM_NONE = 0,
    FOKL_GRAM_VALU = 1,
    FOKL_GRAM_TILES = 2,
    FOKL_GRAM_DMA = 3,
    FOKL_GRAM_PANEL = 4,
    FOKL_GRAM_TILES4 = 5
};
enum { FOKL_RESID_NONE = 0, FOKL_RESID_COLUMNS = 1, FOKL_RESID_MATRIX_FREE = 2 };
enum { FOKL_BASIS_NONE = 0, FOKL_BASIS_REG_TABLE = 1, FOKL_BASIS_LDS_TABLE = 2 };

int fokl_fit_report(const fokl_ctx *ctx, int which, int64_t *out, int count);

#ifdef __cplusplus
}
#endif
#endif
```

Measured before the change: 583,000.

## Cut host launch overhead with an argument ring, by-value kernel args and cached queries

Replaces the single pinned argument buffer, which made every launch wait on the previous copy's event, with a ring of argument slots (depth 8 by default) so the host rarely blocks. Small basis-build and residual argument sets are now passed by value as kernel parameters, which removes the host-to-device copy. Occupancy queries and LDS-limit attribute calls are cached per kernel. Launch-count and wall-clock instrumentation is added, which puts a little timing work on the host path.

```diff
diff --git a/fokl_gpy_amd/_capi.py b/fokl_gpy_amd/_capi.py
--- a/fokl_gpy_amd/_capi.py
+++ b/fokl_gpy_amd/_capi.py
@@ -1502,7 +1502,7 @@
 
 
 RUN_STATS = ('terms_physical', 'substages', 'forecasts_used', 'forecasts_early', 'resid_matrix_free', 't_resid',
-             'phase_prepare', 'phase_model', 'phase_statistics', 'phase_tests', 'phase_wrap_up')
+             'phase_prepare', 'phase_model', 'phase_statistics', 'phase_tests', 'phase_wrap_up', 't_launch_calls')
 
 
 def backend_ops(backend, kernel_id):
@@ -2018,6 +2018,12 @@
         v = self._fit_report(1, 9)
         return dict(kernel=RESID_KERNELS[v[0]], columns=v[1], batches=v[2], grid=v[3], row_tiles=v[4], layout=(v[5], v[6]),
                     order_class=v[7], inputs=v[8])
+
+    def launch_report(self):
+        v = self._fit_report(3, 14)
+        return dict(launches=v[0], arg_copies=v[1], result_copies=v[2], by_value=v[3], ring_depth=v[4], ring_slot=v[5],
+                    total=dict(launches=v[6], arg_copies=v[7], result_copies=v[8], by_value=v[9], ring_waits=v[10],
+                               ring_wait_s=1e-9 * v[11], fetch_host_s=1e-9 * v[12], occupancy_queries=v[13]))
 
     def basis_report(self):
         v = self._fit_report(2, 23)
diff --git a/fokl_gpy_amd/csrc/fokl_gram_dev.inc b/fokl_gpy_amd/csrc/fokl_gram_dev.inc
--- a/fokl_gpy_amd/csrc/fokl_gram_dev.inc
+++ b/fokl_gpy_amd/csrc/fokl_gram_dev.inc
@@ -408,7 +408,7 @@
     run.nr_pad = gz * BI;
     run.nc_pad = gy * BJ;
     const int64_t n_chunks = (ctx->n + GM_R - 1) / GM_R;
-    const int per_cu = blocks_per_cu(mfma_fn, GM_THREADS, 0);
+    const int per_cu = blocks_per_cu(ctx, mfma_fn, GM_THREADS, 0);
     const int target = std::max(1, (per_cu * cu_count(ctx)) / (gz * gy));
     rc = size_slabs(ctx, run, (int)std::max<int64_t>(1, std::min<int64_t>(n_chunks, target)), 1, n_chunks);
     if (rc) return rc;
@@ -429,7 +429,7 @@
     int rc = raise_lds_limit(ctx, reinterpret_cast<const void *>(fn), lds);
     if (rc) return rc;
     const int64_t n_chunks = (ctx->n + 31) / 32;
-    const int per_cu = std::min(wgs_cap, blocks_per_cu(fn, G4S_THREADS, lds));
+    const int per_cu = std::min(wgs_cap, blocks_per_cu(ctx, fn, G4S_THREADS, lds));
     const int target = std::max(1, (per_cu * cu_count(ctx)) / (int)pl.groups.size());
     rc = size_slabs(ctx, run, (int)std::max<int64_t>(1, std::min<int64_t>(n_chunks, target)), 1, n_chunks);
     if (rc) return rc;
@@ -450,7 +450,7 @@
     if (pl.ks == 1 && k.dma != 2 && !(k.dma == 1 && c.slot == FOKL_K_GRAM_MFMA)) {
         gram_tiles_fn fn = tiles_kernel(pl.nt, pl.ct << pl.rb_shift, pl.depth, 1);
         const size_t lds = (size_t)pl.ct * 16 * ((32 << pl.rb_shift) + 2) * sizeof(double);
-        return launch_gram_tiles(ctx, c, run, fn, k.wgs, blocks_per_cu(fn, GT_THREADS, lds), cu_count(ctx));
+        return launch_gram_tiles(ctx, c, run, fn, k.wgs, blocks_per_cu(ctx, fn, GT_THREADS, lds), cu_count(ctx));
     }
     if (pl.ks > 1 && (pl.rb_shift != 0 || pl.depth != 1)) {
         const int passes = pl.ct << pl.rb_shift;
diff --git a/fokl_gpy_amd/csrc/fokl_hip.hip b/fokl_gpy_amd/csrc/fokl_hip.hip
--- a/fokl_gpy_amd/csrc/fokl_hip.hip
+++ b/fokl_gpy_amd/csrc/fokl_hip.hip
@@ -10,6 +10,8 @@
 #include <map>
 #include <mutex>
 #include <string>
+#include <tuple>
+#include <chrono>
 #include <utility>
 #include <vector>
 
@@ -40,6 +42,16 @@
     int kernel_id;
     hipEvent_t start, stop;
 };
+
+struct ArgSlot {
+    char *h = nullptr;
+    char *d = nullptr;
+    size_t cap = 0;
+    hipEvent_t free = nullptr;
+    bool used = false;
+};
+constexpr int ARGS_RING_MAX = 16, ARGS_RING_DEFAULT = 8;
+typedef std::tuple<const void *, int, size_t> OccupancyKey;
 
 struct fokl_ctx {
     int device = 0;
@@ -65,18 +77,20 @@
     double **d_slot_ptr = nullptr;
     int table_cap = 0;
 
+    ArgSlot args_ring[ARGS_RING_MAX];
+    int args_depth = ARGS_RING_DEFAULT;
+    int args_at = -1;
     char *d_args = nullptr;
     char *h_args = nullptr;
-    size_t args_cap = 0;
     double *d_slab = nullptr;
     size_t slab_doubles = 0;
     double *d_out = nullptr;
     double *h_out = nullptr;
     size_t out_doubles = 0;
-    hipEvent_t args_free = nullptr;
     bool resid_pending = false;
     double *d_rout = nullptr;
     double *h_rout = nullptr;
+    bool rout_on_device = false;
     double *d_gout = nullptr;
     double *h_gout = nullptr;
     size_t gout_doubles = 0;
@@ -97,6 +111,8 @@
     int64_t gram_report[FOKL_GRAM_REPORT_LEN] = {};
     int64_t resid_report[FOKL_RESID_REPORT_LEN] = {};
     int64_t basis_report[FOKL_BASIS_REPORT_LEN] = {};
+    int64_t launch_report[FOKL_LAUNCH_REPORT_LEN] = {};
+    std::map<OccupancyKey, int> occupancy;
 
     bool timing = false;
     TimingSlot tslot[FOKL_K_COUNT];
@@ -150,6 +166,8 @@
     }
 };
 
+
+constexpr size_t TIMING_POOL_EVENTS = 256;
 
 static hipEvent_t take_event(fokl_ctx *ctx)
 {
@@ -199,19 +217,53 @@
 }
 
 
-static int ensure_args(fokl_ctx *ctx, size_t bytes)
-{
-    if (bytes <= ctx->args_cap) return FOKL_OK;
+static int64_t now_ns()
+{
+    return std::chrono::duration_cast<std::chrono::nanoseconds>(std::chrono::steady_clock::now().time_since_epoch()).count();
+}
+
+enum { LR_LAUNCHES = 0, LR_ARG_COPIES = 1, LR_RESULT_COPIES = 2, LR_BY_VALUE = 3, LR_RING_DEPTH = 4, LR_RING_SLOT = 5,
+       LR_SUM_LAUNCHES = 6, LR_SUM_ARG_COPIES = 7, LR_SUM_RESULT_COPIES = 8, LR_SUM_BY_VALUE = 9, LR_SUM_RING_WAITS = 10,
+       LR_SUM_RING_WAIT_NS = 11, LR_SUM_FETCH_HOST_NS = 12, LR_SUM_OCCUPANCY_QUERIES = 13 };
+static void note_launch(fokl_ctx *ctx, int what, int n = 1)
+{
+    ctx->launch_report[what] += n;
+    ctx->launch_report[what + LR_SUM_LAUNCHES] += n;
+}
+struct LaunchCall {
+    fokl_ctx *ctx;
+    bool ok = false;
+    explicit LaunchCall(fokl_ctx *c) : ctx(c) { clear(); }
+    ~LaunchCall()
+    {
+        if (!ok) clear();
+    }
+    void clear()
+    {
+        std::memset(ctx->launch_report, 0, sizeof(int64_t) * LR_RING_DEPTH);
+        ctx->launch_report[LR_RING_DEPTH] = ctx->args_depth;
+        ctx->launch_report[LR_RING_SLOT] = -1;
+    }
+    int done()
+    {
+        ok = true;
+        return FOKL_OK;
+    }
+};
+
+static int ensure_args(fokl_ctx *ctx, ArgSlot &slot, size_t bytes)
+{
+    if (bytes <= slot.cap) return FOKL_OK;
     size_t cap = std::max<size_t>(bytes * 2, 1 << 16);
     HIP_TRY(ctx, hipStreamSynchronize(ctx->stream));
-    if (ctx->d_args) HIP_TRY(ctx, hipFree(ctx->d_args));
-    if (ctx->h_args) HIP_TRY(ctx, hipHostFree(ctx->h_args));
-    ctx->d_args = nullptr;
-    ctx->h_args = nullptr;
-    ctx->args_cap = 0;
-    HIP_TRY(ctx, hipMalloc((void **)&ctx->d_args, cap));
-    HIP_TRY(ctx, hipHostMalloc((void **)&ctx->h_args, cap, hipHostMallocDefault));
-    ctx->args_cap = cap;
+    if (slot.d) HIP_TRY(ctx, hipFree(slot.d));
+    if (slot.h) HIP_TRY(ctx, hipHostFree(slot.h));
+    slot.d = nullptr;
+    slot.h = nullptr;
+    slot.cap = 0;
+    HIP_TRY(ctx, hipMalloc((void **)&slot.d, cap));
+    HIP_TRY(ctx, hipHostMalloc((void **)&slot.h, cap, hipHostMallocDefault));
+    slot.cap = cap;
     return FOKL_OK;
 }
 
@@ -270,16 +322,29 @@
 
 static int begin_args(fokl_ctx *ctx, size_t bytes)
 {
-    int rc = ensure_args(ctx, bytes);
-    if (rc) return rc;
-    HIP_TRY(ctx, hipEventSynchronize(ctx->args_free));
+    ctx->args_at = (ctx->args_at + 1) % ctx->args_depth;
+    ArgSlot &slot = ctx->args_ring[ctx->args_at];
+    if (slot.used && hipEventQuery(slot.free) != hipSuccess) {
+        const int64_t t0 = now_ns();
+        HIP_TRY(ctx, hipEventSynchronize(slot.free));
+        ctx->launch_report[LR_SUM_RING_WAITS] += 1;
+        ctx->launch_report[LR_SUM_RING_WAIT_NS] += now_ns() - t0;
+    }
+    int rc = ensure_args(ctx, slot, bytes);
+    if (rc) return rc;
+    ctx->h_args = slot.h;
+    ctx->d_args = slot.d;
+    ctx->launch_report[LR_RING_SLOT] = ctx->args_at;
     return FOKL_OK;
 }
 
 static int push_args(fokl_ctx *ctx, size_t bytes)
 {
-    HIP_TRY(ctx, hipMemcpyAsync(ctx->d_args, ctx->h_args, bytes, hipMemcpyHostToDevice, ctx->stream));
-    HIP_TRY(ctx, hipEventRecord(ctx->args_free, ctx->stream));
+    ArgSlot &slot = ctx->args_ring[ctx->args_at];
+    HIP_TRY(ctx, hipMemcpyAsync(slot.d, slot.h, bytes, hipMemcpyHostToDevice, ctx->stream));
+    HIP_TRY(ctx, hipEventRecord(slot.free, ctx->stream));
+    slot.used = true;
+    note_launch(ctx, LR_ARG_COPIES);
     return FOKL_OK;
 }
 
@@ -355,14 +420,26 @@
     const int total_cus = prop.multiProcessorCount;
     ctx->cus = total_cus;
     const hipError_t made = hipStreamCreateWithFlags(&ctx->stream, hipStreamNonBlocking);
-    if (made != hipSuccess ||
-        hipEventCreateWithFlags(&ctx->args_free, hipEventDisableTiming) != hipSuccess ||
+    if (const char *env = std::getenv("FOKL_ARGS_RING")) {
+        const int depth = std::atoi(env);
+        if (depth >= 1 && depth <= ARGS_RING_MAX) ctx->args_depth = depth;
+    }
+    bool ring_made = made == hipSuccess;
+    for (int i = 0; ring_made && i < ctx->args_depth; ++i)
+        ring_made = hipEventCreateWithFlags(&ctx->args_ring[i].free, hipEventDisableTiming) == hipSuccess;
+    if (!ring_made ||
         hipEventCreateWithFlags(&ctx->gram_done, hipEventDisableTiming) != hipSuccess ||
         hipEventCreateWithFlags(&ctx->resid_done, hipEventDisableTiming) != hipSuccess) {
+        for (ArgSlot &slot : ctx->args_ring)
+            if (slot.free) (void)hipEventDestroy(slot.free);
+        if (ctx->gram_done) (void)hipEventDestroy(ctx->gram_done);
+        if (ctx->resid_done) (void)hipEventDestroy(ctx->resid_done);
+        if (ctx->stream) (void)hipStreamDestroy(ctx->stream);
         delete ctx;
         return fail(nullptr, FOKL_ERR_HIP, "fokl_ctx_create: cannot create stream / event");
     }
-    (void)hipEventRecord(ctx->args_free, ctx->stream);
+    ctx->launch_report[LR_RING_DEPTH] = ctx->args_depth;
+    ctx->launch_report[LR_RING_SLOT] = -1;
     *out = ctx;
     return FOKL_OK;
 }
@@ -383,8 +460,11 @@
     if (ctx->d_phis) (void)hipFree(ctx->d_phis);
     if (ctx->d_zero) (void)hipFree(ctx->d_zero);
     if (ctx->d_staged) (void)hipFree(ctx->d_staged);
-    if (ctx->d_args) (void)hipFree(ctx->d_args);
-    if (ctx->h_args) (void)hipHostFree(ctx->h_args);
+    for (ArgSlot &slot : ctx->args_ring) {
+        if (slot.d) (void)hipFree(slot.d);
+        if (slot.h) (void)hipHostFree(slot.h);
+        if (slot.free) (void)hipEventDestroy(slot.free);
+    }
     if (ctx->d_slab) (void)hipFree(ctx->d_slab);
     if (ctx->d_out) (void)hipFree(ctx->d_out);
     if (ctx->h_out) (void)hipHostFree(ctx->h_out);
@@ -393,7 +473,6 @@
     if (ctx->d_rout) (void)hipFree(ctx->d_rout);
     if (ctx->h_rout) (void)hipHostFree(ctx->h_rout);
     if (ctx->d_comm) (void)hipFree(ctx->d_comm);
-    if (ctx->args_free) (void)hipEventDestroy(ctx->args_free);
     if (ctx->gram_done) (void)hipEventDestroy(ctx->gram_done);
     if (ctx->resid_done) (void)hipEventDestroy(ctx->resid_done);
     if (ctx->stream) (void)hipStreamDestroy(ctx->stream);
@@ -601,6 +680,20 @@
 
 static constexpr size_t K1_LDS_BUDGET = 144 * 1024;
 
+static std::mutex lds_limit_mutex;
+static std::map<const void *, size_t> lds_limit_set;
+
+static int raise_lds_limit(fokl_ctx *ctx, const void *fn, size_t lds, size_t limit = 160 * 1024)
+{
+    std::lock_guard<std::mutex> lock(lds_limit_mutex);
+    size_t &have = lds_limit_set[fn];
+    if (have < lds) {
+        HIP_TRY(ctx, hipFuncSetAttribute(fn, hipFuncAttributeMaxDynamicSharedMemorySize, (int)limit));
+        have = limit;
+    }
+    return FOKL_OK;
+}
+
 static int launch_basis(fokl_ctx *ctx, const int32_t *terms, const int32_t *slots, int t_begin, int t_end,
                         const DerivSpec &deriv)
 {
@@ -656,14 +749,16 @@
     const size_t n_ints = (size_t)3 * U + K1_MAX_LDS_SLABS + (T + 1) + n_fac_entries + T;
     const size_t plan_bytes = sizeof(BasisPlan);
     const size_t bytes = plan_bytes + n_ints * sizeof(int);
-    int rc = begin_args(ctx, bytes);
-    if (rc) return rc;
-    BasisPlan *plan = reinterpret_cast<BasisPlan *>(ctx->h_args);
+    const bool by_value = n_ints <= (size_t)K1_VALUE_INTS;
+    BasisArgs value;
+    int rc = by_value ? FOKL_OK : begin_args(ctx, bytes);
+    if (rc) return rc;
+    BasisPlan *plan = by_value ? &value.plan : reinterpret_cast<BasisPlan *>(ctx->h_args);
     plan->n_fac = U;
     plan->n_terms = T;
     plan->n_slabs = NS;
     plan->pad = 0;
-    int *arr = reinterpret_cast<int *>(ctx->h_args + plan_bytes);
+    int *arr = by_value ? value.arr : reinterpret_cast<int *>(ctx->h_args + plan_bytes);
     int *fac_input = arr, *fac_order = arr + U, *fac_slab = arr + 2 * U, *slab_order = arr + 3 * U;
     int *term_off = slab_order + K1_MAX_LDS_SLABS, *term_fac = term_off + (T + 1);
     int *term_slot = term_fac + n_fac_entries;
@@ -687,16 +782,16 @@
         term_slot[j - t_begin] = slots[j];
     }
     term_off[T] = off;
-    rc = push_args(ctx, bytes);
-    if (rc) return rc;
+    if (!by_value) {
+        rc = push_args(ctx, bytes);
+        if (rc) return rc;
+    }
 
     const int64_t tile_rows = (int64_t)threads * K1_ROWS_PER_THREAD;
     const int64_t n_tiles = (ctx->n + tile_rows - 1) / tile_rows;
     int per_cu = (int)std::max<size_t>(1, std::min<size_t>(reg_table ? 5 : 16, (160 * 1024) / std::max<size_t>(lds_bytes, 1)));
     per_cu = std::min(per_cu, launch_knobs().k1_wgs);
     const int grid = (int)std::min<int64_t>(n_tiles, (int64_t)cu_count(ctx) * per_cu);
-    const BasisPlan *d_plan = reinterpret_cast<const BasisPlan *>(ctx->d_args);
-    const int *d_arr = reinterpret_cast<const int *>(ctx->d_args + plan_bytes);
 
     int m_used = 0;
     {
@@ -711,14 +806,28 @@
     TimedRegion timed(ctx, FOKL_K_BASIS, alg_bytes, 0.0);
     typedef void (*basis_fn)(const double *, int64_t, int64_t, const double *, int, const BasisPlan *, const int *,
                              double *const *, DerivSpec);
+    typedef void (*basis_args_fn)(const double *, int64_t, int64_t, const double *, int, const BasisArgs, double *const *,
+                                  DerivSpec);
     basis_fn fn = splines ? (reg_table ? basis_build_reg_kernel<true> : basis_build_kernel<true>)
                           : (reg_table ? basis_build_reg_kernel<false> : basis_build_kernel<false>);
-    if (lds_bytes > 64 * 1024)
-        HIP_TRY(ctx, hipFuncSetAttribute(reinterpret_cast<const void *>(fn), hipFuncAttributeMaxDynamicSharedMemorySize,
-                                         (int)K1_LDS_BUDGET + 4096));
-    hipLaunchKernelGGL(fn, dim3(grid), dim3(threads), lds_bytes, ctx->stream, ctx->d_x, ctx->ld, ctx->n, ctx->d_phis,
-                       ctx->width, d_plan, d_arr, ctx->d_slot_ptr, deriv);
+    basis_args_fn fn_args = splines ? (reg_table ? basis_build_reg_args_kernel<true> : basis_build_args_kernel<true>)
+                                    : (reg_table ? basis_build_reg_args_kernel<false> : basis_build_args_kernel<false>);
+    if (lds_bytes > 64 * 1024) {
+        rc = raise_lds_limit(ctx, by_value ? reinterpret_cast<const void *>(fn_args) : reinterpret_cast<const void *>(fn),
+                             lds_bytes, K1_LDS_BUDGET + 4096);
+        if (rc) return rc;
+    }
+    if (by_value) {
+        hipLaunchKernelGGL(fn_args, dim3(grid), dim3(threads), lds_bytes, ctx->stream, ctx->d_x, ctx->ld, ctx->n, ctx->d_phis,
+                           ctx->width, value, ctx->d_slot_ptr, deriv);
+        note_launch(ctx, LR_BY_VALUE);
+    } else {
+        hipLaunchKernelGGL(fn, dim3(grid), dim3(threads), lds_bytes, ctx->stream, ctx->d_x, ctx->ld, ctx->n, ctx->d_phis,
+                           ctx->width, reinterpret_cast<const BasisPlan *>(ctx->d_args),
+                           reinterpret_cast<const int *>(ctx->d_args + plan_bytes), ctx->d_slot_ptr, deriv);
+    }
     HIP_TRY(ctx, hipGetLastError());
+    note_launch(ctx, LR_LAUNCHES);
     {
         const int64_t rec[7] = {reg_table ? FOKL_BASIS_REG_TABLE : FOKL_BASIS_LDS_TABLE, splines ? 1 : 0, threads, U, NS,
                                 grid, n_tiles};
@@ -760,9 +869,10 @@
 {
     if (!ctx) return fail(nullptr, FOKL_ERR_ARG, "fokl_build_terms: null context");
     std::memset(ctx->basis_report, 0, sizeof ctx->basis_report);
+    LaunchCall call(ctx);
     if (!ctx->have_data) return fail(ctx, FOKL_ERR_STATE, "fokl_build_terms: call fokl_upload first");
     if (T < 0 || (T > 0 && (!terms || !slots))) return fail(ctx, FOKL_ERR_ARG, "fokl_build_terms: null pointer");
-    if (T == 0) return FOKL_OK;
+    if (T == 0) return call.done();
     HIP_TRY(ctx, hipSetDevice(ctx->device));
     int rc = check_slots(ctx, slots, T, "fokl_build_terms");
     if (rc) return rc;
@@ -812,7 +922,7 @@
         }
         begin = end;
     }
-    return FOKL_OK;
+    return call.done();
 }
 
 
@@ -828,11 +938,15 @@
 }
 
 template <typename F>
-static int blocks_per_cu(F fn, int threads, size_t dyn_lds)
-{
+static int blocks_per_cu(fokl_ctx *ctx, F fn, int threads, size_t dyn_lds)
+{
+    const OccupancyKey key(reinterpret_cast<const void *>(fn), threads, dyn_lds);
+    auto at = ctx->occupancy.find(key);
+    if (at != ctx->occupancy.end()) return at->second;
     int nb = 0;
     if (hipOccupancyMaxActiveBlocksPerMultiprocessor(&nb, fn, threads, dyn_lds) != hipSuccess || nb < 1) nb = 1;
-    return std::min(nb, 8);
+    ctx->launch_report[LR_SUM_OCCUPANCY_QUERIES] += 1;
+    return ctx->occupancy[key] = std::min(nb, 8);
 }
 
 
@@ -1081,20 +1195,6 @@
     int64_t rep[FOKL_GRAM_REPORT_LEN] = {};
 };
 
-static std::mutex lds_limit_mutex;
-static std::map<const void *, size_t> lds_limit_set;
-
-static int raise_lds_limit(fokl_ctx *ctx, const void *fn, size_t lds)
-{
-    std::lock_guard<std::mutex> lock(lds_limit_mutex);
-    size_t &have = lds_limit_set[fn];
-    if (have < lds) {
-        HIP_TRY(ctx, hipFuncSetAttribute(fn, hipFuncAttributeMaxDynamicSharedMemorySize, 160 * 1024));
-        have = 160 * 1024;
-    }
-    return FOKL_OK;
-}
-
 static int pinned_row_cut(int wgs_cap, int by_registers, size_t lds, size_t groups, int64_t n_chunks, int cus = 256)
 {
     const int lds_fit = (int)std::max<size_t>(1, (size_t)(160 * 1024) / std::max<size_t>(lds, 1));
@@ -1211,8 +1311,8 @@
         if (!with) return no_instance(ctx, "gram_tiles_dma_kernel with loader wavefronts", pl);
         rc = raise_lds_limit(ctx, reinterpret_cast<const void *>(with), lds);
         if (rc) return rc;
-        const int per_cu = std::min({wgs_cap, blocks_per_cu(fn, GD_THREADS, lds), by_registers});
-        if (blocks_per_cu(with, GD_THREADS + 64 * loaders, lds) >= per_cu)
+        const int per_cu = std::min({wgs_cap, blocks_per_cu(ctx, fn, GD_THREADS, lds), by_registers});
+        if (blocks_per_cu(ctx, with, GD_THREADS + 64 * loaders, lds) >= per_cu)
             fn = with;
         else
             loaders = 0;
@@ -1255,6 +1355,7 @@
                         int allreduce, bool aside)
 {
     std::memset(ctx->gram_report, 0, sizeof ctx->gram_report);
+    LaunchCall launched(ctx);
     if (!ctx->have_data) return fail(ctx, FOKL_ERR_STATE, "fokl_gram: call fokl_upload first");
     if (nr <= 0 || nc <= 0) return fail(ctx, FOKL_ERR_ARG, "fokl_gram: empty block");
     if (path < 0 || path > 3) return fail(ctx, FOKL_ERR_ARG, "fokl_gram: path must be 0, 1, 2 or 3");
@@ -1293,26 +1394,30 @@
     rc = launch_gram(ctx, call, knobs, path, run);
     if (rc) return rc;
     HIP_TRY(ctx, hipGetLastError());
-
+    note_launch(ctx, LR_LAUNCHES, 2);
+
+    const bool sharded = allreduce && ctx->comm;
+    double *r_dst = sharded ? d_dst : h_dst;
     const int total = nr * nc, epb = reduce_elements_per_block(total);
     {
         TimedRegion timed(ctx, FOKL_K_GRAM_REDUCE, 8.0 * ((double)run.slabs + 1.0) * total, 0.0);
         if (run.d_perm)
             hipLaunchKernelGGL(reduce_slabs_sym_kernel, dim3((total + epb - 1) / epb), dim3(RD_THREADS), 0, ctx->stream,
-                               ctx->d_slab, run.slabs, nr, nc, run.nr_pad, run.nc_pad, epb, run.d_perm, d_dst);
+                               ctx->d_slab, run.slabs, nr, nc, run.nr_pad, run.nc_pad, epb, run.d_perm, r_dst);
         else
             hipLaunchKernelGGL(reduce_slabs_kernel, dim3((total + epb - 1) / epb), dim3(RD_THREADS), 0, ctx->stream,
-                               ctx->d_slab, run.slabs, nr, nc, run.nr_pad, run.nc_pad, epb, d_dst);
+                               ctx->d_slab, run.slabs, nr, nc, run.nr_pad, run.nc_pad, epb, r_dst);
     }
     HIP_TRY(ctx, hipGetLastError());
-    if (allreduce && ctx->comm) {
+    if (sharded) {
         rc = comm_allreduce_device(ctx, d_dst, (size_t)nr * nc);
         if (rc) return rc;
-    }
-    HIP_TRY(ctx, hipMemcpyAsync(h_dst, d_dst, (size_t)nr * nc * sizeof(double), hipMemcpyDeviceToHost, ctx->stream));
+        HIP_TRY(ctx, hipMemcpyAsync(h_dst, d_dst, (size_t)nr * nc * sizeof(double), hipMemcpyDeviceToHost, ctx->stream));
+        note_launch(ctx, LR_RESULT_COPIES);
+    }
     run.rep[13] = run.S, run.rep[15] = run.nr_pad, run.rep[16] = run.nc_pad, run.rep[17] = run.slabs, run.rep[18] = epb;
     std::memcpy(ctx->gram_report, run.rep, sizeof run.rep);
-    return FOKL_OK;
+    return launched.done();
 }
 
 extern "C" int fokl_gram(fokl_ctx *ctx, const int32_t *row_slots, int nr, const int32_t *col_slots, int nc,
@@ -1363,10 +1468,26 @@
 }
 
 
+static int finish_resid_pass(fokl_ctx *ctx, int S)
+{
+    ctx->rout_on_device = ctx->comm != nullptr;
+    hipLaunchKernelGGL(reduce_slabs_kernel, dim3(1), dim3(RD_THREADS), 0, ctx->stream, ctx->d_slab, S, 1, 2, 1, 2, 2,
+                       ctx->rout_on_device ? ctx->d_rout : ctx->h_rout);
+    HIP_TRY(ctx, hipGetLastError());
+    note_launch(ctx, LR_LAUNCHES, 2);
+    if (ctx->rout_on_device) {
+        HIP_TRY(ctx, hipMemcpyAsync(ctx->h_rout, ctx->d_rout, 2 * sizeof(double), hipMemcpyDeviceToHost, ctx->stream));
+        note_launch(ctx, LR_RESULT_COPIES);
+    }
+    HIP_TRY(ctx, hipEventRecord(ctx->resid_done, ctx->stream));
+    return FOKL_OK;
+}
+
 extern "C" int fokl_bic_resid_launch(fokl_ctx *ctx, const int32_t *slots, int nc, const double *betahat)
 {
     if (!ctx) return fail(nullptr, FOKL_ERR_ARG, "fokl_bic_resid_launch: null context");
     std::memset(ctx->resid_report, 0, sizeof ctx->resid_report);
+    LaunchCall launched(ctx);
     if (!ctx->have_data) return fail(ctx, FOKL_ERR_STATE, "fokl_bic_resid_launch: call fokl_upload first");
     if (nc <= 0 || !betahat) return fail(ctx, FOKL_ERR_ARG, "fokl_bic_resid_launch: empty model or null pointer");
     if (ctx->resid_pending) return fail(ctx, FOKL_ERR_STATE, "fokl_bic_resid_launch: previous launch not fetched");
@@ -1374,14 +1495,21 @@
     int rc = check_slots(ctx, slots, nc, "fokl_bic_resid_launch");
     if (rc) return rc;
 
+    const bool by_value = nc <= RS_VALUE_COLS;
     const size_t beta_off = ((size_t)nc * sizeof(int) + 7) & ~(size_t)7;
     const size_t arg_bytes = beta_off + (size_t)nc * sizeof(double);
-    rc = begin_args(ctx, arg_bytes);
-    if (rc) return rc;
-    std::memcpy(ctx->h_args, slots, (size_t)nc * sizeof(int));
-    std::memcpy(ctx->h_args + beta_off, betahat, (size_t)nc * sizeof(double));
-    rc = push_args(ctx, arg_bytes);
-    if (rc) return rc;
+    ResidArgs value;
+    if (by_value) {
+        std::memcpy(value.slots, slots, (size_t)nc * sizeof(int));
+        std::memcpy(value.beta, betahat, (size_t)nc * sizeof(double));
+    } else {
+        rc = begin_args(ctx, arg_bytes);
+        if (rc) return rc;
+        std::memcpy(ctx->h_args, slots, (size_t)nc * sizeof(int));
+        std::memcpy(ctx->h_args + beta_off, betahat, (size_t)nc * sizeof(double));
+        rc = push_args(ctx, arg_bytes);
+        if (rc) return rc;
+    }
 
     const int64_t n_row_blocks = (ctx->n + RS_THREADS * 2 - 1) / (RS_THREADS * 2);
     const int S = (int)std::max<int64_t>(1, std::min<int64_t>(n_row_blocks, (int64_t)cu_count(ctx) * 8));
@@ -1392,24 +1520,27 @@
     {
         {
             TimedRegion timed(ctx, FOKL_K_RESID, 8.0 * (double)ctx->n * (double)(nc + 1), 2.0 * (double)ctx->n * nc);
-            hipLaunchKernelGGL(resid_kernel, dim3(S), dim3(RS_THREADS), 0, ctx->stream, ctx->d_slot_ptr,
-                               reinterpret_cast<const int *>(ctx->d_args),
-                               nc, reinterpret_cast<const double *>(ctx->d_args + beta_off),
-                               ctx->slot_ptr[FOKL_SLOT_Y], ctx->n, ctx->d_slab);
+            if (by_value) {
+                hipLaunchKernelGGL(resid_args_kernel, dim3(S), dim3(RS_THREADS), 0, ctx->stream, ctx->d_slot_ptr, value, nc,
+                                   ctx->slot_ptr[FOKL_SLOT_Y], ctx->n, ctx->d_slab);
+                note_launch(ctx, LR_BY_VALUE);
+            } else {
+                hipLaunchKernelGGL(resid_kernel, dim3(S), dim3(RS_THREADS), 0, ctx->stream, ctx->d_slot_ptr,
+                                   reinterpret_cast<const int *>(ctx->d_args),
+                                   nc, reinterpret_cast<const double *>(ctx->d_args + beta_off),
+                                   ctx->slot_ptr[FOKL_SLOT_Y], ctx->n, ctx->d_slab);
+            }
         }
         HIP_TRY(ctx, hipGetLastError());
-        hipLaunchKernelGGL(reduce_slabs_kernel, dim3(1), dim3(RD_THREADS), 0, ctx->stream, ctx->d_slab, S, 1, 2, 1, 2,
-                           2, ctx->d_rout);
-        HIP_TRY(ctx, hipGetLastError());
-    }
-    HIP_TRY(ctx, hipMemcpyAsync(ctx->h_rout, ctx->d_rout, 2 * sizeof(double), hipMemcpyDeviceToHost, ctx->stream));
-    HIP_TRY(ctx, hipEventRecord(ctx->resid_done, ctx->stream));
+    }
+    rc = finish_resid_pass(ctx, S);
+    if (rc) return rc;
     ctx->resid_pending = true;
     {
         const int64_t rep[FOKL_RESID_REPORT_LEN] = {FOKL_RESID_COLUMNS, nc, (nc + RS_BATCH - 1) / RS_BATCH, S, n_row_blocks};
         std::memcpy(ctx->resid_report, rep, sizeof rep);
     }
-    return FOKL_OK;
+    return launched.done();
 }
 
 typedef void (*resid_quad_fn)(const double *, int64_t, int64_t, const double *, int, const ResidQuadTable *, const double *,
@@ -1431,6 +1562,7 @@
 {
     if (!ctx) return fail(nullptr, FOKL_ERR_ARG, "fokl_bic_resid_terms_launch: null context");
     std::memset(ctx->resid_report, 0, sizeof ctx->resid_report);
+    LaunchCall launched(ctx);
     if (!ctx->have_data) return fail(ctx, FOKL_ERR_STATE, "fokl_bic_resid_terms_launch: call fokl_upload first");
     if (n_terms < 0 || !betahat || (n_terms > 0 && !terms))
         return fail(ctx, FOKL_ERR_ARG, "fokl_bic_resid_terms_launch: null pointer");
@@ -1537,36 +1669,39 @@
                                ctx->d_slab);
         }
         HIP_TRY(ctx, hipGetLastError());
-        hipLaunchKernelGGL(reduce_slabs_kernel, dim3(1), dim3(RD_THREADS), 0, ctx->stream, ctx->d_slab, S, 1, 2, 1, 2,
-                           2, ctx->d_rout);
-        HIP_TRY(ctx, hipGetLastError());
-    }
-    HIP_TRY(ctx, hipMemcpyAsync(ctx->h_rout, ctx->d_rout, 2 * sizeof(double), hipMemcpyDeviceToHost, ctx->stream));
-    HIP_TRY(ctx, hipEventRecord(ctx->resid_done, ctx->stream));
+    }
+    rc = finish_resid_pass(ctx, S);
+    if (rc) return rc;
     ctx->resid_pending = true;
     {
         const int64_t rep[FOKL_RESID_REPORT_LEN] = {FOKL_RESID_MATRIX_FREE, n_terms, 0, S, n_row_blocks, GM, KM,
                                                     splines ? 0 : top_order <= 2 ? 2 : top_order <= 4 ? 4 : RT_MAX_ORDER, G};
         std::memcpy(ctx->resid_report, rep, sizeof rep);
     }
-    return FOKL_OK;
+    return launched.done();
 }
 
 extern "C" int fokl_bic_resid_fetch(fokl_ctx *ctx, double *out, int allreduce)
 {
     if (!ctx || !out) return fail(ctx, FOKL_ERR_ARG, "fokl_bic_resid_fetch: null pointer");
     if (!ctx->resid_pending) return fail(ctx, FOKL_ERR_STATE, "fokl_bic_resid_fetch: nothing was launched");
+    const int64_t t_in = now_ns();
     HIP_TRY(ctx, hipSetDevice(ctx->device));
     ctx->resid_pending = false;
     if (allreduce && ctx->comm) {
+        if (!ctx->rout_on_device)
+            HIP_TRY(ctx, hipMemcpyAsync(ctx->d_rout, ctx->h_rout, 2 * sizeof(double), hipMemcpyHostToDevice, ctx->stream));
         int rc = comm_allreduce_device(ctx, ctx->d_rout, 2);
         if (rc) return rc;
         HIP_TRY(ctx, hipMemcpyAsync(ctx->h_rout, ctx->d_rout, 2 * sizeof(double), hipMemcpyDeviceToHost, ctx->stream));
         HIP_TRY(ctx, hipEventRecord(ctx->resid_done, ctx->stream));
     }
+    const int64_t t_wait = now_ns();
     HIP_TRY(ctx, hipEventSynchronize(ctx->resid_done));
+    const int64_t t_there = now_ns();
     out[0] = ctx->h_rout[0];
     out[1] = ctx->h_rout[1];
+    ctx->launch_report[LR_SUM_FETCH_HOST_NS] += (t_wait - t_in) + (now_ns() - t_there);
     return FOKL_OK;
 }
 
@@ -1583,10 +1718,12 @@
 {
     if (!ctx || !out || count < 0) return fail(nullptr, FOKL_ERR_ARG, "fokl_fit_report: null argument");
     const int64_t *src = which == FOKL_REPORT_GRAM ? ctx->gram_report : which == FOKL_REPORT_RESID ? ctx->resid_report
-                         : which == FOKL_REPORT_BASIS ? ctx->basis_report : nullptr;
+                         : which == FOKL_REPORT_BASIS ? ctx->basis_report : which == FOKL_REPORT_LAUNCH ? ctx->launch_report
+                                                                                                        : nullptr;
     const int len = which == FOKL_REPORT_GRAM ? FOKL_GRAM_REPORT_LEN : which == FOKL_REPORT_RESID ? FOKL_RESID_REPORT_LEN
-                                                                                                  : FOKL_BASIS_REPORT_LEN;
-    if (!src) return fail(nullptr, FOKL_ERR_ARG, "fokl_fit_report: which must be FOKL_REPORT_GRAM, _RESID or _BASIS");
+                    : which == FOKL_REPORT_BASIS ? FOKL_BASIS_REPORT_LEN : FOKL_LAUNCH_REPORT_LEN;
+    if (!src)
+        return fail(nullptr, FOKL_ERR_ARG, "fokl_fit_report: which must be FOKL_REPORT_GRAM, _RESID, _BASIS or _LAUNCH");
     std::memcpy(out, src, (size_t)std::min(count, len) * sizeof(int64_t));
     return FOKL_OK;
 }
@@ -1627,6 +1764,14 @@
 {
     if (!ctx) return fail(nullptr, FOKL_ERR_ARG, "fokl_timing_enable: null context");
     ctx->timing = on != 0;
+    if (ctx->timing) {
+        HIP_TRY(ctx, hipSetDevice(ctx->device));
+        while (ctx->event_pool.size() + 2 * ctx->pending.size() < TIMING_POOL_EVENTS) {
+            hipEvent_t e = nullptr;
+            HIP_TRY(ctx, hipEventCreate(&e));
+            ctx->event_pool.push_back(e);
+        }
+    }
     return FOKL_OK;
 }
 
diff --git a/fokl_gpy_amd/csrc/fokl_kernels.hip.h b/fokl_gpy_amd/csrc/fokl_kernels.hip.h
--- a/fokl_gpy_amd/csrc/fokl_kernels.hip.h
+++ b/fokl_gpy_amd/csrc/fokl_kernels.hip.h
@@ -156,15 +156,20 @@
     }
 }
 
+constexpr int K1_VALUE_INTS = 896;
+struct BasisArgs {
+    BasisPlan plan;
+    int arr[K1_VALUE_INTS];
+};
+
 template <bool SPLINES>
-__global__ __launch_bounds__(K1_THREADS) void basis_build_kernel(
+__device__ __forceinline__ void basis_build_body(
     const double *__restrict__ xT, int64_t ld, int64_t n, const double *__restrict__ phis, int width,
-    const BasisPlan *__restrict__ plan, const int *__restrict__ arr, double *const *__restrict__ slot_ptr,
-    DerivSpec deriv)
+    const int U, const int T, const int NS, const int *__restrict__ arr, double *const *__restrict__ slot_ptr,
+    const DerivSpec &deriv)
 {
     __builtin_amdgcn_s_setprio(3);
     extern __shared__ __attribute__((aligned(16))) double lds[];
-    const int U = plan->n_fac, T = plan->n_terms, NS = plan->n_slabs;
     const int *fac_input = arr;
     const int *fac_order = arr + U;
     const int *fac_slab = arr + 2 * U;
@@ -243,17 +248,34 @@
     }
 }
 
-constexpr int K1_REG_FACTORS = 16;
-
 template <bool SPLINES>
-__global__ __launch_bounds__(K1_THREADS) void basis_build_reg_kernel(
+__global__ __launch_bounds__(K1_THREADS) void basis_build_kernel(
     const double *__restrict__ xT, int64_t ld, int64_t n, const double *__restrict__ phis, int width,
     const BasisPlan *__restrict__ plan, const int *__restrict__ arr, double *const *__restrict__ slot_ptr,
     DerivSpec deriv)
 {
+    basis_build_body<SPLINES>(xT, ld, n, phis, width, plan->n_fac, plan->n_terms, plan->n_slabs, arr, slot_ptr, deriv);
+}
+
+template <bool SPLINES>
+__global__ __launch_bounds__(K1_THREADS) void basis_build_args_kernel(
+    const double *__restrict__ xT, int64_t ld, int64_t n, const double *__restrict__ phis, int width,
+    const BasisArgs args, double *const *__restrict__ slot_ptr, DerivSpec deriv)
+{
+    basis_build_body<SPLINES>(xT, ld, n, phis, width, args.plan.n_fac, args.plan.n_terms, args.plan.n_slabs, args.arr,
+                              slot_ptr, deriv);
+}
+
+constexpr int K1_REG_FACTORS = 16;
+
+template <bool SPLINES>
+__device__ __forceinline__ void basis_build_reg_body(
+    const double *__restrict__ xT, int64_t ld, int64_t n, const double *__restrict__ phis, int width,
+    const int U, const int T, const int NS, const int *__restrict__ arr, double *const *__restrict__ slot_ptr,
+    const DerivSpec &deriv)
+{
     __builtin_amdgcn_s_setprio(3);
     extern __shared__ __attribute__((aligned(16))) double lds[];
-    const int U = plan->n_fac, T = plan->n_terms, NS = plan->n_slabs;
     const int *fac_input = arr;
     const int *fac_order = arr + U;
     const int *fac_slab = arr + 2 * U;
@@ -327,6 +349,24 @@
             }
         }
     }
+}
+
+template <bool SPLINES>
+__global__ __launch_bounds__(K1_THREADS) void basis_build_reg_kernel(
+    const double *__restrict__ xT, int64_t ld, int64_t n, const double *__restrict__ phis, int width,
+    const BasisPlan *__restrict__ plan, const int *__restrict__ arr, double *const *__restrict__ slot_ptr,
+    DerivSpec deriv)
+{
+    basis_build_reg_body<SPLINES>(xT, ld, n, phis, width, plan->n_fac, plan->n_terms, plan->n_slabs, arr, slot_ptr, deriv);
+}
+
+template <bool SPLINES>
+__global__ __launch_bounds__(K1_THREADS) void basis_build_reg_args_kernel(
+    const double *__restrict__ xT, int64_t ld, int64_t n, const double *__restrict__ phis, int width,
+    const BasisArgs args, double *const *__restrict__ slot_ptr, DerivSpec deriv)
+{
+    basis_build_reg_body<SPLINES>(xT, ld, n, phis, width, args.plan.n_fac, args.plan.n_terms, args.plan.n_slabs, args.arr,
+                                  slot_ptr, deriv);
 }
 
 
@@ -1037,11 +1077,9 @@
     double beta;
 };
 
-__global__ __launch_bounds__(RS_THREADS) void resid_kernel(double *const *__restrict__ slot_ptr,
-                                                           const int *__restrict__ slots, int nc,
-                                                           const double *__restrict__ beta,
-                                                           const double *__restrict__ y, int64_t n,
-                                                           double *__restrict__ slab)
+__device__ __forceinline__ void resid_body(double *const *__restrict__ slot_ptr, const int *__restrict__ slots, int nc,
+                                           const double *__restrict__ beta, const double *__restrict__ y, int64_t n,
+                                           double *__restrict__ slab)
 {
     __builtin_amdgcn_s_setprio(3);
     __shared__ __attribute__((aligned(16))) ResidCol cols[RS_BATCH];
@@ -1099,6 +1137,28 @@
     }
 }
 
+__global__ __launch_bounds__(RS_THREADS) void resid_kernel(double *const *__restrict__ slot_ptr,
+                                                           const int *__restrict__ slots, int nc,
+                                                           const double *__restrict__ beta,
+                                                           const double *__restrict__ y, int64_t n,
+                                                           double *__restrict__ slab)
+{
+    resid_body(slot_ptr, slots, nc, beta, y, n, slab);
+}
+
+constexpr int RS_VALUE_COLS = RS_BATCH;
+struct ResidArgs {
+    double beta[RS_VALUE_COLS];
+    int slots[RS_VALUE_COLS];
+};
+
+__global__ __launch_bounds__(RS_THREADS) void resid_args_kernel(double *const *__restrict__ slot_ptr, const ResidArgs args,
+                                                                int nc, const double *__restrict__ y, int64_t n,
+                                                                double *__restrict__ slab)
+{
+    resid_body(slot_ptr, args.slots, nc, args.beta, y, n, slab);
+}
+
 
 
 constexpr int RT_MAX_ORDER = 8;
diff --git a/fokl_gpy_amd/csrc/fokl_run.cpp b/fokl_gpy_amd/csrc/fokl_run.cpp
--- a/fokl_gpy_amd/csrc/fokl_run.cpp
+++ b/fokl_gpy_amd/csrc/fokl_run.cpp
@@ -204,9 +204,15 @@
 
 enum RunStat {
     R_TERMS_PHYSICAL, R_SUBSTAGES, R_FORECASTS_USED, R_FORECASTS_EARLY, R_RESID_MATRIX_FREE, R_T_RESID, R_PHASE_PREPARE,
-    R_PHASE_MODEL, R_PHASE_STATISTICS, R_PHASE_TESTS, R_PHASE_WRAP_UP, R_COUNT
+    R_PHASE_MODEL, R_PHASE_STATISTICS, R_PHASE_TESTS, R_PHASE_WRAP_UP, R_T_LAUNCH_CALLS, R_COUNT
 };
 static_assert(R_COUNT <= FOKL_RUN_STATS, "fokl_run_stats: grow FOKL_RUN_STATS");
+
+struct LaunchClock {
+    double *sum, t0;
+    explicit LaunchClock(double *stats) : sum(stats + R_T_LAUNCH_CALLS), t0(now_s()) {}
+    ~LaunchClock() { *sum += now_s() - t0; }
+};
 
 int matrix_free_pay_from(const fokl_backend_ops &ops, const std::vector<int32_t> &terms, int rows, int m)
 {
@@ -321,7 +327,11 @@
         a->T = (int)(a->vecs.size() / (size_t)m);
         int rc = r->pool.take(a->T, &a->slots);
         if (rc != FOKL_OK) return rc;
-        if ((rc = ops.build_terms(ops.ctx, a->vecs.data(), a->T, a->slots.data())) != FOKL_OK) return rc;
+        {
+            LaunchClock clock(r->stats);
+            rc = ops.build_terms(ops.ctx, a->vecs.data(), a->T, a->slots.data());
+        }
+        if (rc != FOKL_OK) return rc;
         r->stats[R_TERMS_PHYSICAL] += a->T;
         a->built = true;
         return FOKL_OK;
@@ -333,7 +343,11 @@
         std::vector<int32_t> cols(active);
         cols.insert(cols.end(), a->slots.begin(), a->slots.end());
         cols.push_back(FOKL_SLOT_Y);
-        const int rc = ops.gram_launch(ops.ctx, a->slots.data(), a->T, cols.data(), (int)cols.size(), 0);
+        int rc;
+        {
+            LaunchClock clock(r->stats);
+            rc = ops.gram_launch(ops.ctx, a->slots.data(), a->T, cols.data(), (int)cols.size(), 0);
+        }
         if (rc != FOKL_OK) return rc;
         a->pending = true;
         a->valid = true;
@@ -543,7 +557,11 @@
             vecs = arrangements(indvec);
             const int T = (int)(vecs.size() / (size_t)m);
             if ((rc = R->pool.take(T, &new_slots)) != FOKL_OK) return rc;
-            if ((rc = ops.build_terms(ops.ctx, vecs.data(), T, new_slots.data())) != FOKL_OK) return rc;
+            {
+                LaunchClock clock(R->stats);
+                rc = ops.build_terms(ops.ctx, vecs.data(), T, new_slots.data());
+            }
+            if (rc != FOKL_OK) return rc;
             R->stats[R_TERMS_PHYSICAL] += T;
             std::vector<int32_t> cols{FOKL_SLOT_ONES};
             cols.insert(cols.end(), model_slots.begin(), model_slots.end());
@@ -603,9 +621,11 @@
         }
         const double *betahat = buffer + 2 * (size_t)A;
         if (!terms_arr.empty() && A >= terms_pay_from) {
+            LaunchClock clock(R->stats);
             rc = ops.bic_resid_terms_launch(ops.ctx, terms_arr.data() + m, A - 1, betahat);
             R->stats[R_RESID_MATRIX_FREE] += 1;
         } else {
+            LaunchClock clock(R->stats);
             rc = ops.bic_resid_launch(ops.ctx, active_slots.data(), A, betahat);
         }
         if (rc == FOKL_OK && ahead.built && !ahead.valid) rc = launch_ahead_gram(active_slots, &ahead);
diff --git a/fokl_gpy_amd/engine.py b/fokl_gpy_amd/engine.py
--- a/fokl_gpy_amd/engine.py
+++ b/fokl_gpy_amd/engine.py
@@ -1090,6 +1090,7 @@
             self.stats[key] += int(st[key])
         self.stats['forecasts_early'] = self.stats.get('forecasts_early', 0) + int(st['forecasts_early'])
         self.stats['t_resid'] += st['t_resid']
+        self.stats['t_launch_calls'] = self.stats.get('t_launch_calls', 0.0) + st['t_launch_calls']
         self.stats['substage_loop'] = 'native'
         phase = self.stats.setdefault('phases', dict(prepare=0.0, model=0.0, statistics=0.0, tests=0.0, wrap_up=0.0))
         for key in phase:
diff --git a/include/fokl_hip_internal.h b/include/fokl_hip_internal.h
--- a/include/fokl_hip_internal.h
+++ b/include/fokl_hip_internal.h
@@ -544,7 +544,8 @@
 int fokl_control_cvar_report(const fokl_ctx *ctx, int64_t *out);
 
 
-enum { FOKL_REPORT_GRAM = 0, FOKL_REPORT_RESID = 1, FOKL_REPORT_BASIS = 2 };
+enum { FOKL_REPORT_GRAM = 0, FOKL_REPORT_RESID = 1, FOKL_REPORT_BASIS = 2, FOKL_REPORT_LAUNCH = 3 };
+#define FOKL_LAUNCH_REPORT_LEN 16
 #define FOKL_GRAM_REPORT_LEN 24
 #define FOKL_RESID_REPORT_LEN 10
 #define FOKL_BASIS_REPORT_LEN 24
```

New measurement: 540,900. 0.928x the previous value.
